# fetty31/fast_LIMO

Measured on AMD Instinct MI355X. Metric: scans/sec (64k-pt scan, 1M-pt map) + kNN HBM GB/s vs roofline; ATE vs CPU ref, higher is better.
Workload: dtype f32; 1 GPU; BASELINE.json configs[1]: 65536-pt Velodyne-like scan (64 rings x 1024 azimuths), 1000000-pt box-world map, k=5, MAX_NUM_ITERS=3, GPU deskew + iterated ESKF update per step; parallelism=replicas x1 (independent scan streams, no collective), steps_bit_reproducible=True, chains_run=0, chains_handed_back_early=0, chains_declined=2597

## Files before the change

fast_limo_amd/_lib.py:

```python
from __future__ import annotations

import ctypes as C
import os
import numpy as np

_PKG = os.path.dirname(os.path.abspath(__file__))
ROOT = os.path.dirname(_PKG)

f32p = np.ctypeslib.ndpointer(dtype=np.float32, flags="C_CONTIGUOUS")
f64p = np.ctypeslib.ndpointer(dtype=np.float64, flags="C_CONTIGUOUS")
i32p = np.ctypeslib.ndpointer(dtype=np.int32, flags="C_CONTIGUOUS")


class FlimoError(RuntimeError):
    pass


class MapCfg(C.Structure):
    _fields_ = [("min_extent", C.c_float), ("bucket_size", C.c_int), ("downsample", C.c_int),
                ("cell_size", C.c_float)]


class MatchCfg(C.Structure):
    _fields_ = [("NUM_MATCH_POINTS", C.c_int), ("MAX_NUM_MATCHES", C.c_int), ("MAX_NUM_PC2MATCH", C.c_int),
                ("MAX_DIST_PLANE", C.c_double), ("PLANE_THRESHOLD", C.c_double), ("estimate_extrinsics", C.c_int)]


class Frame(C.Structure):
    _fields_ = [("p", C.c_float * 3), ("q", C.c_float * 4), ("v", C.c_float * 3), ("g", C.c_float * 3),
                ("w", C.c_float * 3), ("a", C.c_float * 3), ("bg", C.c_float * 3), ("ba", C.c_float * 3),
                ("time", C.c_double)]


CHAIN_MAX_PASSES = 12


class FilterCfg(C.Structure):
    _fields_ = [("crop_active", C.c_int), ("crop_min", C.c_float * 3), ("crop_max", C.c_float * 3), ("dist_active", C.c_int),
                ("min_dist", C.c_float), ("rate_active", C.c_int), ("rate_value", C.c_int), ("time_kind", C.c_int),
                ("end_of_sweep", C.c_int), ("sweep_ref_time", C.c_double), ("fov_active", C.c_int), ("fov_angle", C.c_float)]


class ChainPass(C.Structure):
    _fields_ = [("M", C.c_int), ("stragglers", C.c_int), ("ties", C.c_int), ("HTH", C.c_double * 144), ("HTh", C.c_double * 12),
                ("dx", C.c_double * 23), ("x_after", C.c_double * 26)]


class ChainIO(C.Structure):
    _fields_ = [("x26", C.c_double * 26), ("P", C.c_double * 529), ("limits", C.c_double * 23), ("R", C.c_double), ("D", C.c_double),
                ("max_iter", C.c_int), ("want_log", C.c_int),
                ("status", C.c_int), ("reason", C.c_int), ("passes", C.c_int), ("it_next", C.c_int), ("t", C.c_int),
                ("x26_out", C.c_double * 26), ("meas_valid", C.c_int), ("meas_M", C.c_int), ("meas_HTH", C.c_double * 144),
                ("meas_HTh", C.c_double * 12), ("log", ChainPass * CHAIN_MAX_PASSES)]


MATCH_REC_DTYPE = np.dtype([
    ("H", np.float32, 12), ("h", np.float32), ("valid", np.float32), ("n", np.float32, 4),
    ("p_global", np.float32, 3), ("sqd", np.float32, 5), ("nbr", np.int32, 5), ("n_nbr", np.int32)])

FRAME_DTYPE = np.dtype([
    ("p", np.float32, 3), ("q", np.float32, 4), ("v", np.float32, 3), ("g", np.float32, 3), ("w", np.float32, 3),
    ("a", np.float32, 3), ("bg", np.float32, 3), ("ba", np.float32, 3), ("_pad", np.float32), ("time", np.float64)])

HIP_SYMBOLS = [
    "flimo_ctx_create", "flimo_ctx_destroy", "flimo_last_error", "flimo_version",
    "flimo_map_config", "flimo_map_add", "flimo_map_clear", "flimo_map_crop_box", "flimo_map_crop_stats", "flimo_map_size", "flimo_map_last_time",
    "flimo_map_points", "flimo_knn", "flimo_scan_set", "flimo_scan_size", "flimo_scan_get",
    "flimo_scan_voxel_filter", "flimo_raw_scan_set", "flimo_raw_scan_filter_set", "flimo_raw_scan_filter_order_set", "flimo_raw_scan_order", "flimo_deskew_resident", "flimo_deskew_resident_offset", "flimo_deskew",
    "flimo_match_reduce", "flimo_match_fetch", "flimo_match_fetch_H",
    "flimo_scan_to_world", "flimo_scan_clouds", "flimo_scan_debug_clouds", "flimo_upload_stage", "flimo_match_reduce_overlap", "flimo_map_add_scan",
    "flimo_set_timing", "flimo_set_timing_stride", "flimo_set_timing_deferred", "flimo_pass_count", "flimo_fused_pass_count", "flimo_tie_stats", "flimo_map_index_bytes", "flimo_fine_stats", "flimo_map_grid_selfcheck", "flimo_set_debug_records", "flimo_last_kernel_ms",
    "flimo_last_candidates_per_query", "flimo_last_widen_count", "flimo_last_stragglers", "flimo_stragglers_by_pass", "flimo_timing_totals", "flimo_timing_split", "flimo_set_path_switches", "flimo_set_wait_timeout_ms", "flimo_insert_rule_replay", "flimo_plane_fit5_host", "flimo_plane_eval5_host", "flimo_calculate_H_host",
    "flimo_update_chain", "flimo_chain_stats", "flimo_set_update_mode", "flimo_update_mode", "flimo_scan_adopt", "flimo_set_pass_pipeline", "flimo_pass_pipeline_end", "flimo_pass_pipeline_last", "flimo_pass_pipeline_stats",
]

_hip = None


def hip_lib_path() -> str:
    return os.environ.get("FLIMO_HIP_LIB") or os.path.join(_PKG, "libflimo_hip.so")


def load_hip():
    global _hip
    if _hip is not None:
        return _hip
    path = hip_lib_path()
    if not os.path.exists(path):
        raise FlimoError(f"{path} not found: run `python -c 'import __graft_entry__ as g; g.build()'` first")
    L = C.CDLL(path)
    vp = C.c_void_p
    L.flimo_ctx_create.restype = C.c_int
    L.flimo_ctx_create.argtypes = [C.c_int, C.POINTER(vp)]
    L.flimo_ctx_destroy.restype = None
    L.flimo_ctx_destroy.argtypes = [vp]
    L.flimo_last_error.restype = C.c_char_p
    L.flimo_last_error.argtypes = [vp]
    L.flimo_version.restype = C.c_char_p
    L.flimo_map_config.argtypes = [vp, C.POINTER(MapCfg)]
    L.flimo_map_add.argtypes = [vp, f32p, C.c_size_t, C.c_size_t, C.c_double]
    L.flimo_map_clear.argtypes = [vp]
    L.flimo_map_crop_box.argtypes = [vp, C.c_void_p, C.c_void_p, C.POINTER(C.c_size_t)]
    L.flimo_map_crop_stats.argtypes = [vp, C.POINTER(C.c_uint64)]
    L.flimo_map_size.restype = C.c_size_t
    L.flimo_map_size.argtypes = [vp]
    L.flimo_map_last_time.restype = C.c_double
    L.flimo_map_last_time.argtypes = [vp]
    L.flimo_map_points.argtypes = [vp, C.c_void_p, C.c_size_t, C.POINTER(C.c_size_t)]
    L.flimo_knn.argtypes = [vp, f32p, C.c_size_t, C.c_int, i32p, f32p, i32p]
    L.flimo_scan_set.argtypes = [vp, f32p, C.c_size_t, C.c_size_t]
    L.flimo_scan_size.restype = C.c_size_t
    L.flimo_scan_size.argtypes = [vp]
    L.flimo_scan_get.argtypes = [vp, C.c_void_p, C.c_size_t, C.POINTER(C.c_size_t)]
    L.flimo_scan_voxel_filter.argtypes = [vp, C.c_float, C.POINTER(C.c_size_t)]
    L.flimo_raw_scan_set.argtypes = [vp, f32p, C.c_size_t, C.c_size_t, f64p]
    L.flimo_deskew_resident.argtypes = [vp, C.c_void_p, C.c_size_t, f32p, f64p]
    L.flimo_deskew.argtypes = [vp, f32p, C.c_size_t, C.c_size_t, f64p, C.c_void_p, C.c_size_t, f32p, f64p]
    L.flimo_match_reduce.argtypes = [vp, f64p, C.POINTER(MatchCfg), f64p, f64p, C.POINTER(C.c_int)]
    L.flimo_match_fetch.argtypes = [vp, C.c_void_p, C.c_size_t, C.POINTER(C.c_size_t)]
    L.flimo_match_fetch_H.argtypes = [vp, C.c_void_p, C.c_void_p, C.c_size_t, C.POINTER(C.c_size_t)]
    L.flimo_scan_to_world.argtypes = [vp, f64p, C.c_void_p, C.c_size_t]
    L.flimo_scan_clouds.argtypes = [vp, f64p, C.POINTER(C.c_void_p), C.POINTER(C.c_void_p), C.POINTER(C.c_size_t)]
    L.flimo_scan_debug_clouds.argtypes = [vp, f64p, C.POINTER(C.c_void_p), C.POINTER(C.c_void_p), C.POINTER(C.c_size_t)]
    L.flimo_upload_stage.argtypes = [vp, C.c_size_t, C.POINTER(C.c_void_p)]
    L.flimo_map_add_scan.argtypes = [vp, f64p, C.c_double]
    L.flimo_set_timing.argtypes = [vp, C.c_int]
    L.flimo_set_wait_timeout_ms.argtypes = [vp, C.c_int]
    L.flimo_set_timing_stride.argtypes = [vp, C.c_int]
    L.flimo_set_timing_deferred.argtypes = [vp, C.c_int]
    L.flimo_pass_count.restype = C.c_ulonglong
    L.flimo_pass_count.argtypes = [vp]
    L.flimo_tie_stats.argtypes = [vp, C.POINTER(C.c_ulonglong)]
    L.flimo_fine_stats.argtypes = [vp, C.POINTER(C.c_ulonglong)]
    L.flimo_map_index_bytes.argtypes = [vp, C.POINTER(C.c_uint64)]
    L.flimo_fused_pass_count.restype = C.c_ulonglong
    L.flimo_fused_pass_count.argtypes = [vp]
    L.flimo_map_grid_selfcheck.restype = C.c_int
    L.flimo_map_grid_selfcheck.argtypes = [vp, C.POINTER(C.c_uint64), C.POINTER(C.c_uint64)]
    L.flimo_set_debug_records.argtypes = [vp, C.c_int]
    L.flimo_last_kernel_ms.argtypes = [vp, C.POINTER(C.c_float), C.POINTER(C.c_float), C.POINTER(C.c_float)]
    L.flimo_timing_totals.argtypes = [vp, C.POINTER(C.c_double), C.POINTER(C.c_double), C.POINTER(C.c_double),
                                      C.POINTER(C.c_longlong), C.POINTER(C.c_longlong), C.c_int]
    L.flimo_timing_split.argtypes = [vp, f64p, C.c_int]
    L.flimo_set_path_switches.argtypes = [vp, C.c_int, C.c_int]
    L.flimo_insert_rule_replay.argtypes = [C.c_float, C.c_int, f32p, C.c_void_p, C.c_size_t, C.c_void_p, C.POINTER(C.c_size_t)]
    L.flimo_calculate_H_host.argtypes = [f64p, f32p, f32p, f32p, C.c_size_t, C.c_int, f64p, f64p]
    L.flimo_update_chain.argtypes = [vp, C.POINTER(MatchCfg), C.POINTER(ChainIO)]
    L.flimo_chain_stats.argtypes = [vp, f64p, C.c_int]
    L.flimo_set_update_mode.argtypes = [vp, C.c_int]
    L.flimo_scan_adopt.argtypes = [vp, vp]
    L.flimo_raw_scan_filter_order_set.argtypes = [vp, C.c_void_p, C.c_size_t, C.POINTER(FilterCfg), C.c_int, C.POINTER(C.c_size_t),
                                                  C.POINTER(C.c_double), C.POINTER(C.c_int), C.POINTER(C.c_int)]
    L.flimo_raw_scan_order.argtypes = [vp, C.c_void_p, C.c_size_t, C.POINTER(C.c_size_t)]
    L.flimo_deskew_resident_offset.argtypes = [vp, C.c_void_p, C.c_size_t, np.ctypeslib.ndpointer(np.float32, flags="C_CONTIGUOUS"),
                                               np.ctypeslib.ndpointer(np.float64, flags="C_CONTIGUOUS"), C.c_double]
    L.flimo_set_pass_pipeline.argtypes = [vp, C.c_int]
# ... 245 lines not shown
    def set_debug_records(self, on=True):
        self._chk(self._L.flimo_set_debug_records(self._h, int(on)))

    def last_kernel_ms(self):
        a = C.c_float(0)
        b = C.c_float(0)
        d = C.c_float(0)
        self._chk(self._L.flimo_last_kernel_ms(self._h, C.byref(a), C.byref(b), C.byref(d)))
        return a.value, b.value, d.value

    def timing_totals(self, reset=False):
        a = C.c_double(0); b = C.c_double(0); d = C.c_double(0); n = C.c_longlong(0); q = C.c_longlong(0)
        self._chk(self._L.flimo_timing_totals(self._h, C.byref(a), C.byref(b), C.byref(d), C.byref(n), C.byref(q), int(reset)))
        return dict(knn_ms=a.value, widen_ms=b.value, fit_ms=d.value, passes=n.value, queries=q.value)

    def set_path_switches(self, tail=-1, fuse=-1):
        self._chk(self._L.flimo_set_path_switches(self._h, int(tail), int(fuse)))

    def timing_split(self, reset=False):
        o = np.zeros(6)
        self._chk(self._L.flimo_timing_split(self._h, o, int(reset)))
        return dict(fused_ms=o[0], fused_n=int(o[1]), knn_ms=o[2], widen_ms=o[3], fit_ms=o[4], separate_n=int(o[5]))

    def update_chain(self, cfg: "MatchCfg", x26, P, limits, R=0.001, D=5.0, max_iter=3, want_log=True):
        io = ChainIO()
        io.x26[:] = list(np.asarray(x26, dtype=np.float64))
        io.P[:] = list(np.asarray(P, dtype=np.float64).reshape(-1))
        io.limits[:] = list(np.asarray(limits, dtype=np.float64))
        io.R, io.D, io.max_iter, io.want_log = float(R), float(D), int(max_iter), int(bool(want_log))
        self._chk(self._L.flimo_update_chain(self._h, C.byref(cfg), C.byref(io)))
        n_log = min(CHAIN_MAX_PASSES, io.passes + (1 if io.status == 2 else 0))
        log = [dict(M=io.log[i].M, stragglers=io.log[i].stragglers, ties=io.log[i].ties,
                    HTH=np.array(io.log[i].HTH).reshape(12, 12), HTh=np.array(io.log[i].HTh), dx=np.array(io.log[i].dx),
                    x_after=np.array(io.log[i].x_after)) for i in range(n_log)]
        meas = dict(M=io.meas_M, HTH=np.array(io.meas_HTH).reshape(12, 12), HTh=np.array(io.meas_HTh)) if io.meas_valid else None
        return dict(status=io.status, reason=io.reason, passes=io.passes, it_next=io.it_next, t=io.t, x=np.array(io.x26_out),
                    meas=meas, log=log)

    def set_update_mode(self, mode: int):
        self._chk(self._L.flimo_set_update_mode(self._h, int(mode)))

    def update_mode(self):
        ch = C.c_int(0); rtt = C.c_double(0)
        self._chk(self._L.flimo_update_mode(self._h, C.byref(ch), C.byref(rtt)))
        return dict(chained=bool(ch.value), launch_rtt_us=rtt.value)

    def set_pass_pipeline(self, on: bool):
        self._chk(self._L.flimo_set_pass_pipeline(self._h, int(on)))

    def pass_pipeline_end(self):
        self._chk(self._L.flimo_pass_pipeline_end(self._h))

    def pass_pipeline_last(self):
        self._chk(self._L.flimo_pass_pipeline_last(self._h))

    def pass_pipeline_stats(self):
        o = (C.c_ulonglong * 4)()
        self._chk(self._L.flimo_pass_pipeline_stats(self._h, o))
        return dict(published=int(o[0]), cancelled=int(o[1]), aged=int(o[2]), left=int(o[3]))

    def chain_stats(self, reset=False):
        o = np.zeros(5)
        self._chk(self._L.flimo_chain_stats(self._h, o, int(reset)))
        return dict(algebra_ms=o[0], algebra_n=int(o[1]), chains=int(o[2]), handed_back=int(o[3]), declined=int(o[4]))

    def last_widen_count(self) -> int:
        return int(self._L.flimo_last_widen_count(self._h))

    def set_wait_timeout_ms(self, ms: int):
        self._chk(self._L.flimo_set_wait_timeout_ms(self._h, int(ms)))

    def last_stragglers(self) -> int:
        return int(self._L.flimo_last_stragglers(self._h))

    def stragglers_by_pass(self):
        o = (C.c_int * 4)()
        self._chk(self._L.flimo_stragglers_by_pass(self._h, o))
        return [int(v) for v in o]

    def last_candidates_per_query(self) -> float:
        return float(self._L.flimo_last_candidates_per_query(self._h))


def default_match_cfg(**kw) -> MatchCfg:
    c = MatchCfg(5, 2000, 10000, 2.0, 5.0e-2, 1)
    for k, v in kw.items():
        if not hasattr(c, k):
            raise AttributeError(k)
        setattr(c, k, v)
    return c


def insert_rule_replay(batches, min_extent=0.2, downsample=True):
    L = load_hip()
    sizes = np.array([b.shape[0] for b in batches], dtype=np.uint64)
    xyz = np.ascontiguousarray(np.concatenate([np.asarray(b, dtype=np.float32).reshape(-1, 3) for b in batches]))
    keep = np.zeros(xyz.shape[0], dtype=np.uint8)
    stored = C.c_size_t(0)
    rc = L.flimo_insert_rule_replay(float(min_extent), int(downsample), xyz.reshape(-1), sizes.ctypes.data, len(batches),
                                    keep.ctypes.data, C.byref(stored))
    if rc != 0:
        raise FlimoError(f"flimo_insert_rule_replay failed ({rc})")
    out, off = [], 0
    for b in batches:
        out.append(keep[off:off + b.shape[0]].astype(bool))
        off += b.shape[0]
    return out, int(stored.value)
```

fast_limo_amd/csrc/hip/flimo_capi.hip:

```cpp
#include <hip/hip_runtime.h>
#include <stdarg.h>
#include <stdio.h>
#include <string.h>
#include <math.h>
#include <string>
#include <chrono>
#include <thread>
#include <array>
#include <vector>
#include <algorithm>
#include <immintrin.h>
#include "../../../include/flimo_c.h"
#include "../../../include/flimo_dev.h"
#include "flimo_types.h"
#include "flimo_kernels.h"
#include "flimo_math.h"
#include "flimo_pose.h"
#include "flimo_chain.h"
#include "flimo_ieskf.h"
#include "flimo_insert.h"
#include "flimo_gbook.h"

#pragma clang fp contract(off)

// ... 93 lines not shown
  float4* d_dbg_clouds = nullptr;
  size_t dbg_clouds_cap = 0, dbg_clouds_dcap = 0;
  void (*overlap_fn)(void*) = nullptr;
  void* overlap_arg = nullptr;
  size_t clouds_cap = 0;
  size_t stage_cap = 0;
  hipEvent_t ev[6] = {nullptr, nullptr, nullptr, nullptr, nullptr, nullptr};
  static constexpr int EV_RING = 64;
  hipEvent_t ev_ring[EV_RING][6];
  unsigned char ev_kind[EV_RING];
  int ev_pending = 0;
  bool ev_ring_made = false, timing_deferred = false;
  float last_knn_ms = 0.f, last_widen_ms = 0.f, last_fit_ms = 0.f;
  int* h_wl_count = nullptr;
  int last_widen_count = 0;
  double tot_knn_ms = 0, tot_widen_ms = 0, tot_fit_ms = 0;
  long long tot_passes = 0, tot_queries = 0;
  double split_fused_ms = 0, split_knn_ms = 0, split_widen_ms = 0, split_fit_ms = 0;
  long long split_fused_n = 0, split_sep_n = 0;
  flimo_match_cfg last_cfg{};
  PoseMats last_P{};
  MatchParams last_mp{};
  int last_n_all = 0;
  bool recs_valid = false, dbg_valid = false;
  PrevPass prev{};
  bool prune = true;
  unsigned probe_min = 96;
  int stragglers_hist[4] = {1 << 30, 0, 0, 0};
  int pass_in_scan = 0;
  int last_stragglers = -1;
  bool fine_on = true;
  unsigned fine_threshold = 64;
  int fine_div = 4;
  unsigned fine_min_points = 32768;
  bool fine_valid = false;
  bool crowd_box_valid = false;
  GridView fine{};
  int fine_qlo[3] = {0, 0, 0}, fine_qhi[3] = {-1, -1, -1};
  float4 *d_fine_tmp = nullptr, *d_fine_pts = nullptr;
  size_t fine_pts_cap = 0;
  IndexTables fine_idx;
  uint32_t* d_fine_count = nullptr;
  void* d_crowd_list = nullptr;
  uint32_t* d_crowd_count = nullptr;
  uint32_t* d_crowd_bits = nullptr;
  size_t crowd_bits_cap = 0;
  uint32_t crowd_listed = 0;
  std::vector<std::array<int, 3>> crowd_cells;
  float fine_center[3] = {0.f, 0.f, 0.f};
  bool have_fine_center = false;
  float fine_radius = 24.f;
  uint64_t fine_builds = 0, fine_passes = 0;
  int xslabs = 2;
  int* d_tie_list = nullptr;
  unsigned int* d_tie_count = nullptr;
  size_t tie_cap = 0;
  bool ties = true;
  unsigned long long tie_redos = 0, tie_queries = 0;
  unsigned long long* d_tie_settled = nullptr;
  void* d_nbrk = nullptr;
  size_t nbrk_cap = 0;
  int wait_timeout_ms = 2000;
  hipEvent_t adopt_ev = nullptr;
  hipEvent_t timeout_ev = nullptr;
  bool timeout_pending = false;
  ChainState* d_chain = nullptr;
  void* d_chain_gran = nullptr;
  ChainPrior* h_chain_prior = nullptr;
  ChainPrior* d_chain_prior = nullptr;
  double* h_chain_res = nullptr;
  void* d_chain_res = nullptr;
  double* h_chain_log = nullptr;
  void* d_chain_log = nullptr;
  unsigned long long chain_tag = 0x4000000000000000ull;
  struct Prelaunch {
    bool active = false;
    unsigned long long seq = 0;
    size_t nq = 0;
    int n_all = 0, pos = 0;
    flimo_match_cfg cfg{};
    uint64_t grid_version = 0;
    unsigned int end_code = 0;
    double t_launch = 0.0;
  } pre;
  bool pipeline = false;
  bool pipeline_env = false;
  ChainHead* d_pipe_head = nullptr;
  unsigned int pipe_tag = 0;
  bool pipe_last_hint = false;
  unsigned long long pipe_published = 0, pipe_cancelled = 0;
  unsigned long long pipe_aged = 0, pipe_left = 0;
  bool row_slack = true;
  bool test_tight_array = false;
  int test_publish_delay_ms = 0;
  PrevPass prev_before{};
  int update_mode = 0;
  double launch_rtt_us = 0.0;
  bool host_update = false;
  hipEvent_t chain_ev[CH_MAX_PASSES][8];
  bool chain_ev_made = false;
  double chain_alg_ms = 0;
  long long chain_alg_n = 0, chains_run = 0, chains_back = 0, chains_declined = 0;
  int fov_check = 0, fov_check_bad = 0;
  bool tail = true;
};

constexpr size_t FRAMES_FG_SLOT = 8192;
static int timing_drain(flimo_ctx* c);
static inline void ctx_enter(flimo_ctx* c);
static int fail(flimo_ctx* c, int code, const char* fmt, ...) {
  char buf[512];
  va_list ap;
  va_start(ap, fmt);
  vsnprintf(buf, sizeof(buf), fmt, ap);
  va_end(ap);
  if (c) c->err = buf;
  return code;
}
#define HIPCHK(c, call)                                                                          \
  do {                                                                                           \
    hipError_t e_ = (call);                                                                      \
    if (e_ != hipSuccess) return fail(c, FLIMO_ERR_HIP, "%s failed: %s", #call, hipGetErrorString(e_)); \
  } while (0)

static int ensure_pinned(flimo_ctx* c, void*& buf, size_t& cap, size_t bytes) {
  if (bytes <= cap) return FLIMO_OK;
  if (buf) (void)hipHostFree(buf);
  buf = nullptr;
  cap = 0;
  const size_t ncap = bytes + bytes / 4 + 4096;
  HIPCHK(c, hipHostMalloc(&buf, ncap, hipHostMallocDefault));
  cap = ncap;
  return FLIMO_OK;
}
static int ensure_stage(flimo_ctx* c, size_t bytes) { return ensure_pinned(c, c->h_stage, c->stage_cap, bytes); }

template <typename T>
static int ensure_dev(flimo_ctx* c, T*& p, size_t& cap, size_t need, bool keep, size_t keep_n) {
  if (need <= cap) return FLIMO_OK;
  size_t ncap = need + need / 4 + 1024;
  T* np = nullptr;
  HIPCHK(c, hipMalloc(&np, ncap * sizeof(T)));
  if (keep && p && keep_n) {
    HIPCHK(c, hipMemcpyAsync(np, p, keep_n * sizeof(T), hipMemcpyDeviceToDevice, c->stream));
    HIPCHK(c, hipStreamSynchronize(c->stream));
  }
  if (p) (void)hipFree(p);
  p = np;
  cap = ncap;
  return FLIMO_OK;
}


static void load_dev_switches(flimo_ctx* c) {
  auto env_int = [](const char* name, int& out) { const char* e = getenv(name); if (!e) return false; out = atoi(e); return true; };
  int v = 0;
  if (env_int("FLIMO_FUSE", v)) c->fuse = v != 0;
  if (env_int("FLIMO_TAIL", v)) c->tail = v != 0;
  if (env_int("FLIMO_PRUNE", v)) c->prune = v != 0;
  if (env_int("FLIMO_PROBE", v) && v >= 0) c->probe_min = (unsigned)v;
  if (env_int("FLIMO_TIES", v)) c->ties = v != 0;
  if (env_int("FLIMO_FINE", v)) c->fine_on = v != 0;
  if (env_int("FLIMO_FINE_THRESHOLD", v) && v > 0) c->fine_threshold = (unsigned)v;
  if (env_int("FLIMO_FINE_MIN_POINTS", v) && v >= 0) c->fine_min_points = (unsigned)v;
  if (env_int("FLIMO_FULL_REBUILD", v)) c->full_rebuild = v != 0;
  if (env_int("FLIMO_HOST_UPDATE", v)) c->update_mode = v != 0 ? 1 : 2;
  if (env_int("FLIMO_PIPELINE", v)) { c->pipeline = v != 0; c->pipeline_env = true; }
  if (env_int("FLIMO_TEST_PUBLISH_DELAY_MS", v) && v > 0) c->test_publish_delay_ms = v;
  if (env_int("FLIMO_TEST_TIGHT_ARRAY", v)) c->test_tight_array = v != 0;
  if (env_int("FLIMO_ROW_SLACK", v)) c->row_slack = v != 0;
  if (env_int("FLIMO_TAIL_MAX", v) && v > 0) c->tail_max_env = v;
}

static bool host_store_probe(flimo_ctx* c, ChainHead* head) {
  volatile unsigned long long* tagp = reinterpret_cast<volatile unsigned long long*>(c->h_chain_res) + 1;
  for (unsigned int round = 0; round < 2; round++) {
    const unsigned int pattern = 0x5a17c0deu ^ (round * 0x01010101u);
    __atomic_store_n(&head->epoch, pattern, __ATOMIC_RELEASE);
    _mm_sfence();
    const unsigned long long tag = 0x7200000000000000ull + round;
    launch_word_probe(c->stream, &head->epoch, c->d_chain_res, tag);
    if (hipStreamSynchronize(c->stream) != hipSuccess) { (void)hipGetLastError(); return false; }
    if (*tagp != tag) return false;
    const double seen = c->h_chain_res[0];
    if ((unsigned int)llround(seen) != pattern) return false;
  }
  __atomic_store_n(&head->epoch, 0u, __ATOMIC_RELEASE);
  _mm_sfence();
  memset(c->h_chain_res, 0, 2 * sizeof(double));
  return true;
}

extern "C" const char* flimo_version(void) { return "fast_limo_amd 0.1.0 (gfx950)"; }

extern "C" const char* flimo_last_error(const flimo_ctx* ctx) { return ctx ? ctx->err.c_str() : "null context"; }

extern "C" int flimo_ctx_create(int device, flimo_ctx** out) {
  if (!out) return FLIMO_ERR_INVALID;
  *out = nullptr;
  int ndev = 0;
  if (hipGetDeviceCount(&ndev) != hipSuccess || ndev <= 0) return FLIMO_ERR_NO_DEVICE;
  if (device < 0 || device >= ndev) return FLIMO_ERR_INVALID;
  if (hipSetDevice(device) != hipSuccess) return FLIMO_ERR_NO_DEVICE;
  hipDeviceProp_t prop;
  if (hipGetDeviceProperties(&prop, device) != hipSuccess) return FLIMO_ERR_NO_DEVICE;
  if (strncmp(prop.gcnArchName, "gfx950", 6) != 0) return FLIMO_ERR_NO_DEVICE;
  flimo_ctx* c = new flimo_ctx();
  c->device = device;
  if (hipStreamCreateWithFlags(&c->stream, hipStreamNonBlocking) != hipSuccess) { delete c; return FLIMO_ERR_HIP; }
  for (int i = 0; i < 6; i++) (void)hipEventCreate(&c->ev[i]);
  bool ok = hipMalloc(&c->d_partials, (size_t)c->reduce_waves * 256 * sizeof(double)) == hipSuccess &&
            hipMalloc(&c->d_out256, FIT_GROUPS * FIT_SLOT * sizeof(double)) == hipSuccess &&
            hipHostMalloc((void**)&c->h_out256, FIT_GROUPS * FIT_SLOT * sizeof(double), hipHostMallocMapped) == hipSuccess &&
            hipHostGetDevicePointer((void**)&c->d_out256_host, c->h_out256, 0) == hipSuccess &&
            hipHostMalloc((void**)&c->h_granules, FIT_GROUPS * FIT_LIVE_PAD * 2 * sizeof(double), hipHostMallocMapped) == hipSuccess &&
            hipHostGetDevicePointer((void**)&c->d_granules_host, c->h_granules, 0) == hipSuccess &&
            hipMalloc(&c->d_ticket, (FIT_GROUPS + 2) * sizeof(unsigned int)) == hipSuccess &&
            hipMemset(c->d_ticket, 0, (FIT_GROUPS + 2) * sizeof(unsigned int)) == hipSuccess &&
            hipMalloc(&c->d_cand, sizeof(unsigned long long)) == hipSuccess &&
            hipMalloc(&c->d_tie_count, 2 * sizeof(unsigned int)) == hipSuccess &&
            hipMemset(c->d_tie_count, 0, 2 * sizeof(unsigned int)) == hipSuccess &&
            hipMalloc((void**)&c->d_chain, chain_state_size()) == hipSuccess &&
            hipMemset(c->d_chain, 0, chain_state_size()) == hipSuccess &&
            hipMalloc(&c->d_chain_gran, FIT_GROUPS * FIT_LIVE_PAD * 2 * sizeof(double)) == hipSuccess &&
            hipMemset(c->d_chain_gran, 0, FIT_GROUPS * FIT_LIVE_PAD * 2 * sizeof(double)) == hipSuccess &&
            hipHostMalloc((void**)&c->h_chain_prior, sizeof(ChainPrior), hipHostMallocMapped) == hipSuccess &&
            hipHostGetDevicePointer((void**)&c->d_chain_prior, c->h_chain_prior, 0) == hipSuccess &&
            hipHostMalloc((void**)&c->h_chain_res, (size_t)CH_RES * 2 * sizeof(double), hipHostMallocMapped) == hipSuccess &&
            hipHostGetDevicePointer(&c->d_chain_res, c->h_chain_res, 0) == hipSuccess &&
            hipHostMalloc((void**)&c->h_chain_log, (size_t)CH_MAX_PASSES * CH_LOGN * 2 * sizeof(double), hipHostMallocMapped) == hipSuccess &&
            hipHostGetDevicePointer(&c->d_chain_log, c->h_chain_log, 0) == hipSuccess &&
            hipMalloc((void**)&c->d_tie_settled, sizeof(unsigned long long)) == hipSuccess &&
            hipMemset(c->d_tie_settled, 0, sizeof(unsigned long long)) == hipSuccess &&
            hipMalloc(&c->d_wl_count, sizeof(int)) == hipSuccess &&
            hipMemset(c->d_wl_count, 0, sizeof(int)) == hipSuccess &&
            hipHostMalloc((void**)&c->h_wl_count, sizeof(int), hipHostMallocDefault) == hipSuccess &&
            hipHostMalloc((void**)&c->h_cand, sizeof(unsigned long long), hipHostMallocDefault) == hipSuccess;
  if (!ok) { flimo_ctx_destroy(c); return FLIMO_ERR_HIP; }
  memset(c->h_chain_res, 0, (size_t)CH_RES * 2 * sizeof(double));
  memset(c->h_chain_log, 0, (size_t)CH_MAX_PASSES * CH_LOGN * 2 * sizeof(double));
  memset(c->h_out256, 0, FIT_GROUPS * FIT_SLOT * sizeof(double));
  memset(c->h_granules, 0, FIT_GROUPS * FIT_LIVE_PAD * 2 * sizeof(double));
  launch_mfma_layout(c->stream, c->d_out256);
  if (hipMemcpyAsync(c->h_out256, c->d_out256, 256 * sizeof(double), hipMemcpyDeviceToHost, c->stream) != hipSuccess ||
      hipStreamSynchronize(c->stream) != hipSuccess) { flimo_ctx_destroy(c); return FLIMO_ERR_HIP; }
  bool seen[256] = {false};
  for (int r = 0; r < 256; r++) {
    const double v = c->h_out256[r];
    const int code = (int)llround(v);
    if (code < 0 || code > 255 || fabs(v - code) > 1e-9 || seen[code]) { flimo_ctx_destroy(c); return FLIMO_ERR_HIP; }
    seen[code] = true;
    c->mfma_idx[code / 16][code % 16] = r;
  }
  {
    int k = 0;
    for (int i = 0; i < 12; i++) for (int j = i; j < 12; j++) c->live_idx[k++] = (unsigned char)c->mfma_idx[i][j];
    for (int i = 0; i < 12; i++) c->live_idx[k++] = (unsigned char)c->mfma_idx[i][12];
    c->live_idx[k++] = (unsigned char)c->mfma_idx[13][13];
    for (; k < FIT_LIVE_PAD; k++) c->live_idx[k] = 0;
  }
  c->book = insert_book_create();
  load_dev_switches(c);
  {
    void* p = nullptr;
    int large_bar = 0;
    (void)hipDeviceGetAttribute(&large_bar, hipDeviceAttributeIsLargeBar, device);
    if (getenv("FLIMO_NO_BAR") != nullptr) large_bar = 0;
    if (large_bar && hipExtMallocWithFlags(&p, sizeof(ChainHead), hipDeviceMallocFinegrained) == hipSuccess && p &&
        hipMemset(p, 0, sizeof(ChainHead)) == hipSuccess && hipDeviceSynchronize() == hipSuccess && host_store_probe(c, static_cast<ChainHead*>(p))) {
      c->d_pipe_head = static_cast<ChainHead*>(p);
      void* q = nullptr;
      if (hipExtMallocWithFlags(&q, 2 * FRAMES_FG_SLOT, hipDeviceMallocFinegrained) == hipSuccess && q)
        c->d_frames_fg = static_cast<char*>(q);
      else (void)hipGetLastError();
    } else {
      if (p) (void)hipFree(p);
      (void)hipGetLastError();
      c->d_pipe_head = nullptr;
    }
  }
  {
    std::vector<double> rt;
    volatile unsigned long long* tagp = reinterpret_cast<volatile unsigned long long*>(c->h_chain_res) + 1;
    for (int i = 0; i < 40; i++) {
      const unsigned long long tag = 0x7100000000000000ull + (unsigned long long)i;
      const auto t0 = std::chrono::steady_clock::now();
      launch_rtt_probe(c->stream, c->d_chain_res, tag);
      unsigned long long spins = 0;
      while (*tagp != tag && ++spins < 200000000ull) _mm_pause();
      const double us = std::chrono::duration<double, std::micro>(std::chrono::steady_clock::now() - t0).count();
      if (i >= 8) rt.push_back(us);
    }
    (void)hipStreamSynchronize(c->stream);
    std::sort(rt.begin(), rt.end());
    c->launch_rtt_us = rt[rt.size() / 4];
    memset(c->h_chain_res, 0, 2 * sizeof(double));
    c->host_update = c->update_mode != 2;
  }
  *out = c;
  return FLIMO_OK;
}

extern "C" void flimo_ctx_destroy(flimo_ctx* c) {
  if (!c) return;
  ctx_enter(c);
  if (c->stream) (void)hipStreamSynchronize(c->stream);
  (void)hipFree(c->d_map_raw); (void)hipFree(c->d_map_sorted); index_free(c->idx); index_free(c->fine_idx);
  (void)hipFree(c->d_scan_sorted); (void)hipFree(c->d_nbr); (void)hipFree(c->d_wl); (void)hipFree(c->d_wl_count);
  (void)hipFree(c->d_fit_partials); (void)hipFree(c->d_raw_sorted); (void)hipFree(c->d_t_sorted);
  (void)hipFree(c->d_scan); (void)hipFree(c->d_scan_raw); (void)hipFree(c->d_scan_world); (void)hipFree(c->d_scan_t);
  (void)hipFree(c->d_frames); (void)hipFree(c->d_recs); (void)hipFree(c->d_dbg); (void)hipFree(c->d_dbg_clouds);
  (void)hipFree(c->d_fine_tmp); (void)hipFree(c->d_fine_pts); 
  (void)hipFree(c->d_fine_count); (void)hipFree(c->d_crowd_list); (void)hipFree(c->d_crowd_count); (void)hipFree(c->d_crowd_bits);
  (void)hipFree(c->d_tkey[0]); (void)hipFree(c->d_tkey[1]); (void)hipFree(c->d_tperm); (void)hipFree(c->d_t_tmp);
  (void)hipFree(c->d_raw32); (void)hipFree(c->d_filt_ext); (void)hipFree(c->d_nbrk); (void)hipFree(c->d_tie_list); (void)hipFree(c->d_tie_count);
  if (c->h_filt_ext) (void)hipHostFree(c->h_filt_ext);
  (void)hipFree(c->d_partials); (void)hipFree(c->d_out256); (void)hipFree(c->d_cand); (void)hipFree(c->d_ticket);
  if (c->h_out256) (void)hipHostFree(c->h_out256);
  if (c->h_granules) (void)hipHostFree(c->h_granules);
  (void)hipFree(c->d_fit2_partials);
  if (c->h_cand) (void)hipHostFree(c->h_cand);
  (void)hipFree(c->d_chain); (void)hipFree(c->d_chain_gran); (void)hipFree(c->d_tie_settled);
  if (c->h_chain_prior) (void)hipHostFree(c->h_chain_prior);
  if (c->h_chain_res) (void)hipHostFree(c->h_chain_res);
  if (c->h_chain_log) (void)hipHostFree(c->h_chain_log);
  if (c->chain_ev_made) for (int i = 0; i < CH_MAX_PASSES; i++) for (int k = 0; k < 8; k++) (void)hipEventDestroy(c->chain_ev[i][k]);
  if (c->h_stage) (void)hipHostFree(c->h_stage);
  if (c->h_dbg_clouds) (void)hipHostFree(c->h_dbg_clouds);
  if (c->h_clouds) (void)hipHostFree(c->h_clouds);
  for (int k = 0; k < 2; k++) if (c->h_frames[k]) (void)hipHostFree(c->h_frames[k]);
  map_scratch_free(c->scratch);
  for (int i = 0; i < 6; i++) if (c->ev[i]) (void)hipEventDestroy(c->ev[i]);
  if (c->ev_ring_made) for (int r = 0; r < flimo_ctx::EV_RING; r++) for (int i = 0; i < 6; i++) (void)hipEventDestroy(c->ev_ring[r][i]);
  if (c->timeout_ev) (void)hipEventDestroy(c->timeout_ev);
  if (c->adopt_ev) (void)hipEventDestroy(c->adopt_ev);
  if (c->h_wl_count) (void)hipHostFree(c->h_wl_count);
  if (c->d_pipe_head) (void)hipFree(c->d_pipe_head);
  if (c->d_frames_fg) (void)hipFree(c->d_frames_fg);
  if (c->stream) (void)hipStreamDestroy(c->stream);
  if (c->book) insert_book_destroy(c->book);
  c->gbook.release();
  (void)hipFree(c->d_batch);
  delete c;
}

extern "C" int flimo_map_config(flimo_ctx* c, const flimo_map_cfg* cfg) {
  if (!c || !cfg) return FLIMO_ERR_INVALID;
  if (!(cfg->min_extent > 0.f)) return fail(c, FLIMO_ERR_INVALID, "min_extent must be > 0");
  const float cell_before = c->map_cfg.cell_size;
  c->map_cfg = *cfg;
  if (!(c->map_cfg.cell_size > 0.f)) c->map_cfg.cell_size = 0.5f;
  if (c->map_cfg.cell_size != cell_before) { c->force_full = true; c->have_gbox = false; c->have_origin = false; }
  insert_book_config(c->book, cfg->min_extent, cfg->downsample != 0);
// ... 1007 lines not shown
  out[5] = c->d_map_sorted ? (uint64_t)c->sorted_cap * sizeof(float4) : 0ull;
  out[1] = c->grid_valid ? tables(c->grid, c->idx) : 0ull;
  out[2] = c->fine_valid ? (uint64_t)c->fine.n_pts * sizeof(float4) + tables(c->fine, c->fine_idx) : 0ull;
  out[3] = c->grid_valid ? c->idx.tiles_used : 0ull;
  out[4] = c->index_overflows;
  return FLIMO_OK;
}
extern "C" int flimo_tie_stats(flimo_ctx* c, unsigned long long out[2]) {
  if (!c || !out) return FLIMO_ERR_INVALID;
  out[0] = c->tie_redos; out[1] = c->tie_queries;
  unsigned long long dev = 0;
  ctx_enter(c);
  if (c->d_tie_settled && hipMemcpy(&dev, c->d_tie_settled, sizeof(dev), hipMemcpyDeviceToHost) == hipSuccess) out[1] += dev;
  return FLIMO_OK;
}
extern "C" int flimo_set_timing_stride(flimo_ctx* c, int every) { if (!c || every < 1) return FLIMO_ERR_INVALID; c->timing_stride = every; return FLIMO_OK; }
extern "C" int flimo_set_debug_records(flimo_ctx* c, int on) { if (!c) return FLIMO_ERR_INVALID; c->debug_recs = on != 0; return FLIMO_OK; }
extern "C" int flimo_last_kernel_ms(const flimo_ctx* c, float* knn_ms, float* widen_ms, float* fit_ms) {
  if (!c) return FLIMO_ERR_INVALID;
  if (knn_ms) *knn_ms = c->last_knn_ms;
  if (widen_ms) *widen_ms = c->last_widen_ms;
  if (fit_ms) *fit_ms = c->last_fit_ms;
  return FLIMO_OK;
}
extern "C" int flimo_last_widen_count(const flimo_ctx* c) { return c ? c->last_widen_count : 0; }
extern "C" int flimo_last_stragglers(const flimo_ctx* c) { return c ? c->last_stragglers : -1; }
extern "C" int flimo_stragglers_by_pass(const flimo_ctx* c, int out[4]) {
  if (!c || !out) return FLIMO_ERR_INVALID;
  for (int i = 0; i < 4; i++) out[i] = c->stragglers_hist[i];
  return FLIMO_OK;
}
extern "C" int flimo_timing_totals(flimo_ctx* c, double* knn_ms, double* widen_ms, double* fit_ms, long long* passes,
                                   long long* queries, int reset) {
  if (!c) return FLIMO_ERR_INVALID;
  if (c->ev_pending) { ctx_enter(c); const int rc = timing_drain(c); if (rc) return rc; }
  if (knn_ms) *knn_ms = c->tot_knn_ms;
  if (widen_ms) *widen_ms = c->tot_widen_ms;
  if (fit_ms) *fit_ms = c->tot_fit_ms;
  if (passes) *passes = c->tot_passes;
  if (queries) *queries = c->tot_queries;
  if (reset) { c->tot_knn_ms = c->tot_widen_ms = c->tot_fit_ms = 0.0; c->tot_passes = 0; c->tot_queries = 0; }
  return FLIMO_OK;
}
extern "C" int flimo_set_path_switches(flimo_ctx* c, int tail, int fuse) {
  if (!c) return FLIMO_ERR_INVALID;
  if (tail >= 0) c->tail = tail != 0;
  if (fuse >= 0) c->fuse = fuse != 0;
  return FLIMO_OK;
}
extern "C" int flimo_timing_split(flimo_ctx* c, double out[6], int reset) {
  if (!c || !out) return FLIMO_ERR_INVALID;
  if (c->ev_pending) { ctx_enter(c); const int rc = timing_drain(c); if (rc) return rc; }
  out[0] = c->split_fused_ms; out[1] = (double)c->split_fused_n;
  out[2] = c->split_knn_ms; out[3] = c->split_widen_ms; out[4] = c->split_fit_ms; out[5] = (double)c->split_sep_n;
  if (reset) { c->split_fused_ms = c->split_knn_ms = c->split_widen_ms = c->split_fit_ms = 0.0; c->split_fused_n = c->split_sep_n = 0; }
  return FLIMO_OK;
}
extern "C" double flimo_last_candidates_per_query(const flimo_ctx* c) { return c ? c->last_cand_per_query : 0.0; }

static int gate_rings(const flimo_ctx* c, double max_dist_plane) {
  const double cell = c->grid.cell;
  const int maxdim = std::max(c->grid.nx, std::max(c->grid.ny, c->grid.nz));
  const double margin = 1.0e-3 + 4.0e-7 * maxdim;
  const double need = sqrt(std::max(max_dist_plane, 0.0)) * (1.0 + 1e-5) / cell + margin;
  int r = (int)ceil(need);
  return std::max(r, 1);
}

static int abandon_wait(flimo_ctx* c, const char* what, unsigned long long id) {
  if (!c->timeout_ev) (void)hipEventCreateWithFlags(&c->timeout_ev, hipEventDisableTiming);
  if (c->timeout_ev && hipEventRecord(c->timeout_ev, c->stream) == hipSuccess) c->timeout_pending = true;
  c->prev.valid = 0;
  return fail(c, FLIMO_ERR_TIMEOUT, "%s %llu did not publish its result within %d ms (kernels still running)", what, id, c->wait_timeout_ms);
}
static inline bool same_match_cfg(const flimo_match_cfg& a, const flimo_match_cfg& b) {
  return a.NUM_MATCH_POINTS == b.NUM_MATCH_POINTS && a.MAX_NUM_MATCHES == b.MAX_NUM_MATCHES && a.MAX_NUM_PC2MATCH == b.MAX_NUM_PC2MATCH &&
         a.MAX_DIST_PLANE == b.MAX_DIST_PLANE && a.PLANE_THRESHOLD == b.PLANE_THRESHOLD && a.estimate_extrinsics == b.estimate_extrinsics;
}
static inline double wall_s() { return std::chrono::duration<double>(std::chrono::steady_clock::now().time_since_epoch()).count(); }
static inline void cancel_prelaunch(flimo_ctx* c) {
  if (!c->pre.active) return;
  c->pre.active = false;
  c->pipe_cancelled++;
  __atomic_store_n(&c->d_pipe_head->epoch, c->pre.end_code, __ATOMIC_RELEASE);
  _mm_sfence();
}
static inline void ctx_enter(flimo_ctx* c) {
  (void)hipSetDevice(c->device);
  cancel_prelaunch(c);
}
static inline void publish_prelaunch(flimo_ctx* c, const PoseMats& P, const float prev_RT[16], unsigned long long seq) {
  ChainHead h;
  memset(&h, 0, sizeof(h));
  h.pose = P;
  memcpy(h.prev_RT, prev_RT, sizeof(h.prev_RT));
  h.status = 0;
  const size_t words8 = offsetof(ChainHead, status) / 8;
  static_assert(offsetof(ChainHead, status) % 8 == 0 && offsetof(ChainHead, epoch) == offsetof(ChainHead, status) + 4, "ChainHead layout");
  volatile unsigned long long* dst = reinterpret_cast<volatile unsigned long long*>(c->d_pipe_head);
  const unsigned long long* src = reinterpret_cast<const unsigned long long*>(&h);
  for (size_t i = 0; i < words8; i++) dst[i] = src[i];
  __atomic_store_n(&c->d_pipe_head->status, 0, __ATOMIC_RELAXED);
  _mm_sfence();
  __atomic_store_n(&c->d_pipe_head->epoch, ch_epoch_of(seq), __ATOMIC_RELEASE);
  _mm_sfence();
  c->pre.active = false;
  c->pipe_published++;
}

static inline bool auto_host_update(const flimo_ctx*) { return true; }

static int check_abandoned(flimo_ctx* c) {
  if (!c->timeout_pending) return FLIMO_OK;
  hipError_t q = hipEventQuery(c->timeout_ev);
  if (q == hipErrorNotReady) return fail(c, FLIMO_ERR_TIMEOUT, "the launches of an earlier pass whose wait ran out are still running");
  c->timeout_pending = false;
  if (q != hipSuccess) return fail(c, FLIMO_ERR_HIP, "an abandoned pass failed: %s", hipGetErrorString(q));
  return FLIMO_OK;
}
static bool tags_complete(const flimo_ctx* c, unsigned long long want) {
  const volatile unsigned long long* t0 = reinterpret_cast<const volatile unsigned long long*>(c->h_granules);
  if (t0[2 * FIT_LIVE + 1] != want || t0[2 * (FIT_LIVE + 1) + 1] != want) return false;
  for (int g = 0; g < FIT_GROUPS; g++) {
    const volatile unsigned long long* tags = reinterpret_cast<const volatile unsigned long long*>(c->h_granules + (size_t)g * FIT_LIVE_PAD * 2);
    for (int k = 0; k < FIT_LIVE; k++)
      if (tags[2 * k + 1] != want) return false;
  }
  return true;
}
constexpr int FLIMO_PASS_LEFT = 1000;
static int wait_tags(flimo_ctx* c, unsigned long long want, int left_ms = -1) {
  const volatile unsigned long long* t0 = reinterpret_cast<const volatile unsigned long long*>(c->h_granules);
  unsigned long long spins = 0;
  double deadline = 0.0;
  auto now_s = [] { return std::chrono::duration<double>(std::chrono::steady_clock::now().time_since_epoch()).count(); };
  if (c->wait_timeout_ms == 0) return abandon_wait(c, "pass", want);
  const int bound_ms = left_ms >= 0 ? std::min(left_ms, c->wait_timeout_ms) : c->wait_timeout_ms;
  for (;;) {
    if (t0[2 * (FIT_LIVE + 1) + 1] == want && tags_complete(c, want)) return FLIMO_OK;
    _mm_pause();
    if ((++spins & 0x3fffull) != 0) continue;
    if (left_ms >= 0 && c->d_pipe_head &&
        __atomic_load_n(&c->d_pipe_head->decision, __ATOMIC_ACQUIRE) == ((ch_epoch_of(want) & 0x3fffffffu) | 0x80000000u)) return FLIMO_PASS_LEFT;
    const double t = now_s();
    if (deadline == 0.0) { deadline = t + 1e-3 * (double)bound_ms; continue; }
    if (t < deadline) continue;
    const hipError_t q = hipStreamQuery(c->stream);
    if (q == hipErrorNotReady && left_ms >= 0 && bound_ms < c->wait_timeout_ms) { left_ms = -1; deadline = t + 1e-3 * (double)(c->wait_timeout_ms - bound_ms); continue; }
    if (q == hipErrorNotReady) return abandon_wait(c, "pass", want);
    if (q != hipSuccess) return fail(c, FLIMO_ERR_HIP, "pass %llu failed: %s", want, hipGetErrorString(q));
    if (tags_complete(c, want)) return FLIMO_OK;
    if (left_ms >= 0) return FLIMO_PASS_LEFT;
    (void)hipMemsetAsync(c->d_ticket, 0, (FIT_GROUPS + 2) * sizeof(unsigned int), c->stream);
    (void)hipMemsetAsync(c->d_wl_count, 0, sizeof(int), c->stream);
    (void)hipMemsetAsync(c->d_tie_count, 0, 2 * sizeof(unsigned int), c->stream);
    (void)hipStreamSynchronize(c->stream);
    c->prev.valid = 0;
    return fail(c, FLIMO_ERR_HIP, "pass %llu completed without publishing its result (reduction tickets re-armed)", want);
  }
}

extern "C" int flimo_set_wait_timeout_ms(flimo_ctx* c, int ms) {
  if (!c || ms < 0) return FLIMO_ERR_INVALID;
  c->wait_timeout_ms = ms;
  return FLIMO_OK;
}

extern "C" int flimo_match_reduce(flimo_ctx* c, const double x26[26], const flimo_match_cfg* cfg, double HTH[144], double HTh[12], int* M);
extern "C" int flimo_match_reduce_overlap(flimo_ctx* c, const double x26[26], const flimo_match_cfg* cfg, double HTH[144], double HTh[12],
                                          int* M, void (*while_in_flight)(void*), void* arg) {
  if (!c) return FLIMO_ERR_INVALID;
  c->overlap_fn = while_in_flight;
  c->overlap_arg = arg;
  const int rc = flimo_match_reduce(c, x26, cfg, HTH, HTh, M);
  c->overlap_fn = nullptr;
  return rc;
}

static inline void run_overlap(flimo_ctx* c) {
  if (!c->overlap_fn) return;
  void (*fn)(void*) = c->overlap_fn;
  c->overlap_fn = nullptr;
  fn(c->overlap_arg);
}

struct PassPlan {
  const flimo_match_cfg* cfg = nullptr;
  PoseMats P;
  MatchParams mp;
  size_t nq = 0;
  int n_all = 0;
  bool general_k = false;
  bool use_pre = false, was_pre = false;
  bool last_of_update = false;
  uint64_t grid_version = 0;
  const DeskewArgs* dkp = nullptr;
  bool cap_binds = false, want_recs = false, want_count = false, fused_cap = false, use_fit2 = false;
  int tlev = 0;
  hipEvent_t* ev = nullptr;
  int tail_max = 0;
  bool tail = false, fused = false, after_fine = false, widen_timed = false;
  unsigned long long seq = 0;
  bool ties_on = false, inline_ties = false;
  TieList tl{};
  BookView book{};
  const BookView* bookp = nullptr;
  double tp0 = 0, tpa = 0, tpb = 0, tpc = 0, tp1 = 0;
};
static const bool g_prof_pass = getenv("FLIMO_PROF_PASS") != nullptr;
static inline double now_us() { return std::chrono::duration<double, std::micro>(std::chrono::steady_clock::now().time_since_epoch()).count(); }

constexpr int PASS_NOTHING = 2000;
static int pass_plan(flimo_ctx* c, const double x26[26], const flimo_match_cfg* cfg, PassPlan& pl) {
  pl.cfg = cfg;
  pl.general_k = cfg->NUM_MATCH_POINTS != 5;
  pl.last_of_update = c->pipe_last_hint;
  c->pipe_last_hint = false;
  struct PreGuard { flimo_ctx* c; bool decided = false; ~PreGuard() { if (!decided) cancel_prelaunch(c); } } pre_guard{c};
  { const int rca = check_abandoned(c); if (rca) return rca; }
  c->last_nq = 0;
  c->last_cfg = *cfg;
  c->recs_valid = c->dbg_valid = false;
  if (!c->grid_valid && c->map_n > 0) { int rc0 = rebuild_grid(c); if (rc0) return rc0; }
  if (!c->grid_valid || c->map_n == 0) return PASS_NOTHING;
  size_t nq = c->scan_n;
  if (cfg->MAX_NUM_PC2MATCH >= 0 && nq > (size_t)cfg->MAX_NUM_PC2MATCH) nq = (size_t)cfg->MAX_NUM_PC2MATCH;
  if (nq == 0) return PASS_NOTHING;
  pl.nq = nq;
  (void)hipSetDevice(c->device);
  pl.grid_version = c->grid_builds * 0x100000000ull + c->grid_merges;
  bool use_pre = c->pre.active && !pl.general_k && c->prev.valid && c->pre.nq == nq && c->pre.seq == c->pass_seq + 1 &&
                 same_match_cfg(c->pre.cfg, *cfg) && c->pre.grid_version == pl.grid_version && !c->deskew_pending &&
                 !(nq < c->sorted_n || (c->sorted_n < c->scan_n && nq > c->sorted_n)) && c->pre.n_all == (int)c->sorted_n &&
                 !c->debug_recs && !(cfg->MAX_NUM_MATCHES >= 0 && (size_t)cfg->MAX_NUM_MATCHES < nq);
  if (use_pre && !(wall_s() - c->pre.t_launch < 0.25e-3 * (double)CH_POLL_MS)) { use_pre = false; c->pipe_aged++; }
  if (!use_pre) cancel_prelaunch(c);
  pre_guard.decided = true;
  int rc = ensure_recs(c, nq);
  if (rc) { cancel_prelaunch(c); return rc; }

  pl.tp0 = g_prof_pass ? now_us() : 0.0;
  pose_from_x26(x26, pl.P);
  MatchParams& mp = pl.mp;
  mp.max_dist_plane_d = cfg->MAX_DIST_PLANE;
  mp.plane_threshold = (float)cfg->PLANE_THRESHOLD;
  mp.estimate_extrinsics = cfg->estimate_extrinsics ? 1 : 0;
  mp.n_queries = (int)nq;
  mp.max_ring = gate_rings(c, cfg->MAX_DIST_PLANE);

  if (nq < c->sorted_n || (c->sorted_n < c->scan_n && nq > c->sorted_n)) {
    const size_t want = nq;
    { const int rcf = flush_deskew(c); if (rcf) return rcf; }
    HIPCHK(c, sort_scan(c->stream, c->d_scan, want, c->d_scan_sorted, c->scratch));
    c->sorted_n = want;
    c->prev.valid = 0;
  }
  pl.n_all = (int)c->sorted_n;
  const bool ride = c->deskew_pending && !pl.general_k && c->deskew_n == (size_t)pl.n_all &&
                    !(c->fine_valid && mp.max_ring >= 1);
  if (!ride) { const int rcf = flush_deskew(c); if (rcf) return rcf; }
  pl.dkp = ride ? &c->deskew_args : nullptr;
  c->deskew_pending = false;
  pl.cap_binds = cfg->MAX_NUM_MATCHES >= 0 && (size_t)cfg->MAX_NUM_MATCHES < nq;
  if (pl.general_k) return FLIMO_OK;
  pl.want_recs = c->debug_recs || pl.cap_binds;
  if (c->debug_recs) HIPCHK(c, hipMemsetAsync(c->d_cand, 0, sizeof(unsigned long long), c->stream));
  pl.want_count = c->debug_recs;
  pl.tpa = g_prof_pass ? now_us() : 0.0;
  pl.tlev = (c->timing == 1 && c->timing_stride > 1 && ((c->pass_seq + 1) % (unsigned long long)c->timing_stride) != 0) ? 0 : c->timing;
  pl.ev = (c->timing_deferred && c->ev_ring_made) ? c->ev_ring[c->ev_pending] : c->ev;
  const bool first_pass = !c->prev.valid;
  c->pass_in_scan = first_pass ? 0 : std::min(c->pass_in_scan + 1, 3);
  pl.tail_max = c->tail_max_env > 0 ? c->tail_max_env : std::max(1024, pl.n_all / 64);
  const bool tail_here = first_pass ? (c->stragglers_hist[0] <= pl.tail_max)
                                    : (c->stragglers_hist[c->pass_in_scan] <= pl.tail_max);
  pl.tail = c->tail && tail_here && mp.max_ring >= 2 && mp.max_ring <= 3;
  c->prev.probe_min = c->probe_min;
  pl.fused = pl.tail && c->fuse && !pl.want_recs;
  pl.seq = ++c->pass_seq;
  pl.ties_on = c->ties && c->gbook.active;
  pl.tl = TieList{};
  pl.tl.count_next = c->d_tie_count + ((pl.seq + 1) & 1);
  pl.inline_ties = pl.ties_on && !pl.want_recs;
  if (pl.ties_on && !pl.inline_ties) { pl.tl.list = c->d_tie_list; pl.tl.count = c->d_tie_count + (pl.seq & 1); pl.tl.cap = (unsigned)c->tie_cap; }
  pl.book = BookView{c->gbook.node_c, c->gbook.node_child, c->gbook.node_cnt, c->gbook.root, c->d_tie_settled};
  pl.bookp = pl.inline_ties ? &pl.book : nullptr;
  pl.after_fine = c->fine_valid && mp.max_ring >= 1;
  if (use_pre && !(pl.fused && !pl.after_fine && pl.tlev == 0)) {
    cancel_prelaunch(c);
    use_pre = false;
  }
  if (use_pre) {
    const int test_delay_ms = c->test_publish_delay_ms;
    if (wall_s() - c->pre.t_launch >= 0.25e-3 * (double)CH_POLL_MS) { cancel_prelaunch(c); use_pre = false; c->pipe_aged++; }
    else if (test_delay_ms > 0) std::this_thread::sleep_for(std::chrono::milliseconds(test_delay_ms));
  }
  pl.use_pre = pl.was_pre = use_pre;
  pl.widen_timed = !pl.tail && pl.tlev == 1 && mp.max_ring >= 2;
  pl.fused_cap = pl.cap_binds && !c->debug_recs;
  pl.use_fit2 = !pl.want_recs;
  return FLIMO_OK;
}

static int pass_general_k(flimo_ctx* c, const PassPlan& pl, double HTH[144], double HTh[12], int* M) {
  const flimo_match_cfg* cfg = pl.cfg;
  const int n_all = pl.n_all;
  const size_t nq = pl.nq;
  if ((size_t)n_all > c->nbrk_cap) {
    (void)hipFree(c->d_nbrk);
    c->d_nbrk = nullptr; c->nbrk_cap = 0;
    const size_t cap = (size_t)n_all + (size_t)n_all / 4 + 1024;
    HIPCHK(c, hipMalloc(&c->d_nbrk, cap * nbrk_rec_size()));
    c->nbrk_cap = cap;
  }
  c->prev.valid = 0;
  const BookView bookk{c->gbook.node_c, c->gbook.node_child, c->gbook.node_cnt, c->gbook.root, nullptr};
  if (!launch_match_k(c->stream, cfg->NUM_MATCH_POINTS, c->grid, c->d_scan_sorted, n_all, pl.P, pl.mp, c->d_nbrk, c->d_recs, c->d_dbg,
                      (c->ties && c->gbook.active) ? &bookk : nullptr))
    return fail(c, FLIMO_ERR_UNSUPPORTED, "NUM_MATCH_POINTS out of range");
  if (pl.cap_binds) launch_cap(c->stream, c->d_recs, (int)nq, cfg->MAX_NUM_MATCHES);
  launch_reduce(c->stream, c->d_recs, (int)nq, c->reduce_waves, c->d_partials, c->d_out256_host);
  HIPCHK(c, hipMemsetAsync(c->d_tie_count, 0, 2 * sizeof(unsigned int), c->stream));
  HIPCHK(c, hipGetLastError());
  run_overlap(c);
  HIPCHK(c, hipStreamSynchronize(c->stream));
  ++c->pass_seq;
  for (int i = 0; i < 12; i++) {
    for (int j = 0; j < 12; j++) HTH[i * 12 + j] = c->h_out256[c->mfma_idx[i][j]];
    HTh[i] = c->h_out256[c->mfma_idx[i][12]];
  }
  *M = (int)llround(c->h_out256[c->mfma_idx[13][13]]);
  c->last_nq = (int)nq;
  c->last_P = pl.P; c->last_mp = pl.mp; c->last_n_all = n_all;
  c->recs_valid = true; c->dbg_valid = true;
  c->last_stragglers = -1;
  c->async_deskews = 0;
  return FLIMO_OK;
}

static int pass_launch(flimo_ctx* c, PassPlan& pl) {
  const flimo_match_cfg* cfg = pl.cfg;
  const PoseMats& P = pl.P;
  const MatchParams& mp = pl.mp;
  const int n_all = pl.n_all;
  const size_t nq = pl.nq;
  const unsigned long long seq = pl.seq;
  const int tlev = pl.tlev;
  if (pl.use_pre) {
    publish_prelaunch(c, P, c->prev.RT, seq);
    c->fused_passes++;
  } else if (pl.after_fine) {
    launch_knn5_fine(c->stream, c->fine, c->d_scan_sorted, n_all, P, c->d_nbr, c->prev, c->fine_qlo, c->fine_qhi, &pl.tl, seq);
    c->fine_passes++;
  }
  if (pl.use_pre) {
  } else if (pl.fused) {
    launch_match_fused(c->stream, c->grid, c->d_scan_sorted, n_all, P, mp, c->d_nbr, c->d_wl, c->d_wl_count, nullptr, c->prev,
                       c->live_idx, c->d_fit2_partials, c->d_granules_host, c->d_ticket, seq, tlev == 1 ? pl.ev[0] : nullptr,
                       tlev == 1 ? pl.ev[1] : nullptr, &pl.tl, pl.after_fine ? 1 : 0, pl.dkp, nullptr, nullptr, pl.bookp);
    c->fused_passes++;
  } else
  launch_knn5(c->stream, 2, c->grid, c->d_scan_sorted, n_all, P, mp.max_ring, c->d_nbr, c->d_wl,
              c->d_wl_count, c->debug_recs ? c->d_cand : nullptr, c->prev, pl.tail ? 1 : 0, tlev == 1 ? pl.ev[0] : nullptr,
              tlev == 1 ? pl.ev[1] : nullptr, nullptr, &pl.tl, pl.after_fine ? 1 : 0, seq, pl.dkp);
  c->prev_before = c->prev;
  if (c->prune) { memcpy(c->prev.RT, P.RT, sizeof(c->prev.RT)); c->prev.valid = 1; }
  pl.tpb = g_prof_pass ? now_us() : 0.0;
  if (!pl.tail)
    launch_widen(c->stream, c->grid, c->d_scan_sorted, P, mp.max_ring, c->d_nbr, c->d_wl, c->d_wl_count,
                 c->debug_recs ? c->d_cand : nullptr, pl.widen_timed ? pl.ev[4] : nullptr, pl.widen_timed ? pl.ev[5] : nullptr, &pl.tl);
  pl.tpc = g_prof_pass ? now_us() : 0.0;
  if (pl.want_count) HIPCHK(c, hipMemcpyAsync(c->h_wl_count, c->d_wl_count, sizeof(int), hipMemcpyDeviceToHost, c->stream));
  if (pl.fused) {
  } else if (pl.use_fit2)
    launch_fit2(c->stream, c->grid, c->d_scan_sorted, n_all, c->d_nbr, P, mp, c->live_idx, c->d_fit2_partials, c->d_granules_host,
                c->d_ticket, c->d_wl_count, seq, tlev == 1 ? pl.ev[2] : nullptr, tlev == 1 ? pl.ev[3] : nullptr, &pl.tl, nullptr, nullptr, pl.bookp);
  else {
    HIPCHK(c, hipGetLastError());
    if (pl.ties_on) { launch_tie(c->stream, c->grid, pl.book, c->d_scan_sorted, P, c->d_nbr, pl.tl); HIPCHK(c, hipGetLastError()); }
    launch_fit(c->stream, c->grid, c->d_scan_sorted, n_all, c->d_nbr, P, mp, pl.fused_cap ? nullptr : c->d_fit_partials,
               pl.want_recs ? c->d_recs : nullptr, c->debug_recs ? c->d_dbg : nullptr, pl.cap_binds ? c->d_out256 : c->d_out256_host,
               c->d_ticket, c->d_wl_count, seq);
    HIPCHK(c, hipGetLastError());
    HIPCHK(c, hipMemsetAsync(c->d_tie_count, 0, 2 * sizeof(unsigned int), c->stream));
  }
  if (pl.fused_cap) {
    launch_capreduce(c->stream, c->d_recs, (int)nq, cfg->MAX_NUM_MATCHES, c->d_out256_host, c->d_wl_count, seq);
  } else if (pl.cap_binds) {
    launch_cap(c->stream, c->d_recs, (int)nq, cfg->MAX_NUM_MATCHES);
    launch_reduce(c->stream, c->d_recs, (int)nq, c->reduce_waves, c->d_partials, c->d_out256_host);
  }
  HIPCHK(c, hipGetLastError());
  pl.tp1 = g_prof_pass ? now_us() : 0.0;
  if (c->debug_recs) HIPCHK(c, hipMemcpyAsync(c->h_cand, c->d_cand, sizeof(unsigned long long), hipMemcpyDeviceToHost, c->stream));
  if (c->pipeline && !pl.last_of_update && c->d_pipe_head && c->prune && pl.use_fit2 && !pl.want_count && c->tail && c->fuse &&
      mp.max_ring >= 2 && mp.max_ring <= 3 && !c->fine_valid && pl.inline_ties == pl.ties_on) {
    const unsigned long long nseq = seq + 1;
    const int ntlev = (c->timing == 1 && c->timing_stride > 1 && (nseq % (unsigned long long)c->timing_stride) != 0) ? 0 : c->timing;
    const int npos = std::min(c->pass_in_scan + 1, 3);
    if (ntlev == 0 && c->stragglers_hist[npos] <= pl.tail_max) {
      TieList tln{};
      tln.count_next = c->d_tie_count + ((nseq + 1) & 1);
      ChainCtl pc{};
      pc.end_code = 0x80000000u | (++c->pipe_tag & 0x7fffffffu);
      PrevPass pv = c->prev;
      pv.valid = 1;
      launch_match_fused(c->stream, c->grid, c->d_scan_sorted, n_all, P, mp, c->d_nbr, c->d_wl, c->d_wl_count, nullptr, pv,
                         c->live_idx, c->d_fit2_partials, c->d_granules_host, c->d_ticket, nseq, nullptr, nullptr, &tln, 0, nullptr,
                         c->d_pipe_head, &pc, pl.bookp, ch_epoch_of(nseq));
      HIPCHK(c, hipGetLastError());
      c->pre.active = true; c->pre.seq = nseq; c->pre.nq = nq; c->pre.n_all = n_all; c->pre.pos = npos; c->pre.cfg = *cfg;
      c->pre.grid_version = pl.grid_version; c->pre.end_code = pc.end_code; c->pre.t_launch = wall_s();
    }
  }
  return FLIMO_OK;
}

static int timing_read(flimo_ctx* c, hipEvent_t* ev, int kind) {
  const bool fused = kind & 1, use_fit2 = kind & 2, widen_timed = kind & 4;
  if (hipEventElapsedTime(&c->last_knn_ms, ev[0], ev[1]) != hipSuccess) {
    HIPCHK(c, hipEventSynchronize(ev[1]));
    (void)hipEventElapsedTime(&c->last_knn_ms, ev[0], ev[1]);
  }
  c->tot_knn_ms += c->last_knn_ms;
  if (fused) {
    c->last_fit_ms = 0.f; c->last_widen_ms = 0.f;
    c->split_fused_ms += c->last_knn_ms; c->split_fused_n++;
  } else if (use_fit2) {
    c->last_widen_ms = 0.f;
    if (widen_timed) {
      if (hipEventElapsedTime(&c->last_widen_ms, ev[4], ev[5]) != hipSuccess) c->last_widen_ms = 0.f;
      c->tot_widen_ms += c->last_widen_ms;
    }
    if (hipEventElapsedTime(&c->last_fit_ms, ev[2], ev[3]) != hipSuccess) {
      HIPCHK(c, hipEventSynchronize(ev[3]));
      (void)hipEventElapsedTime(&c->last_fit_ms, ev[2], ev[3]);
    }
    c->tot_fit_ms += c->last_fit_ms;
    c->split_knn_ms += c->last_knn_ms; c->split_widen_ms += c->last_widen_ms; c->split_fit_ms += c->last_fit_ms; c->split_sep_n++;
  }
  return FLIMO_OK;
}
static int timing_drain(flimo_ctx* c) {
  const int n = c->ev_pending;
  c->ev_pending = 0;
  for (int i = 0; i < n; i++) { const int rc = timing_read(c, c->ev_ring[i], c->ev_kind[i]); if (rc) return rc; }
  return FLIMO_OK;
}

static int pass_collect(flimo_ctx* c, PassPlan& pl, double HTH[144], double HTh[12], int* M) {
  const PoseMats& P = pl.P;
  const MatchParams& mp = pl.mp;
  const int n_all = pl.n_all;
  const size_t nq = pl.nq;
  const unsigned long long seq = pl.seq;
  const int tlev = pl.tlev;
  double acc[256];
  if (pl.use_fit2) {
    auto wait_granules = [&](unsigned long long want, int left_ms = -1) -> int {
      const int rcw = wait_tags(c, want, left_ms);
      if (rcw) return rcw;
      __atomic_thread_fence(__ATOMIC_ACQUIRE);
      return FLIMO_OK;
    };
    run_overlap(c);
    {
      int rcw = wait_granules(seq, pl.was_pre ? CH_POLL_MS + 25 : -1);
      if (rcw == FLIMO_PASS_LEFT) {
        cancel_prelaunch(c);
        c->pipe_left++;
        launch_match_fused(c->stream, c->grid, c->d_scan_sorted, n_all, P, mp, c->d_nbr, c->d_wl, c->d_wl_count, nullptr, c->prev_before,
                           c->live_idx, c->d_fit2_partials, c->d_granules_host, c->d_ticket, seq, nullptr, nullptr, &pl.tl, 0, nullptr, nullptr,
                           nullptr, pl.bookp);
        HIPCHK(c, hipGetLastError());
        rcw = wait_granules(seq);
      }
      if (rcw) return rcw;
    }
    c->last_stragglers = (int)llround(c->h_granules[2 * FIT_LIVE]);
    c->stragglers_hist[c->pass_in_scan] = c->last_stragglers;
    const long n_ties = (long)llround(c->h_granules[2 * (FIT_LIVE + 1)]);
    if (n_ties > 0 && pl.ties_on) {
      c->tie_redos++; c->tie_queries += (unsigned long long)n_ties;
      launch_tie(c->stream, c->grid, pl.book, c->d_scan_sorted, P, c->d_nbr, pl.tl);
      const unsigned long long seq2 = ++c->pass_seq;
      TieList tl2{};
      tl2.count_next = c->d_tie_count + ((seq2 + 1) & 1);
      launch_fit2(c->stream, c->grid, c->d_scan_sorted, n_all, c->d_nbr, P, mp, c->live_idx, c->d_fit2_partials, c->d_granules_host,
                  c->d_ticket, c->d_wl_count, seq2, nullptr, nullptr, &tl2);
      HIPCHK(c, hipGetLastError());
      const int rcw = wait_granules(seq2);
      if (rcw) return rcw;
    }
    double live[FIT_LIVE];
    for (int k = 0; k < FIT_LIVE; k++) {
// ... 34 lines not shown
      const int rc = timing_read(c, c->ev, kind);
      if (rc) return rc;
    }
    c->tot_passes++; c->tot_queries += n_all;
  }
  if (g_prof_pass) {
    static double acc_launch = 0, acc_wait = 0, a0 = 0, a1 = 0, a2 = 0, a3 = 0; static long cnt = 0;
    const double tp2 = now_us();
    acc_launch += pl.tp1 - pl.tp0; acc_wait += tp2 - pl.tp1;
    a0 += pl.tpa - pl.tp0; a1 += pl.tpb - pl.tpa; a2 += pl.tpc - pl.tpb; a3 += pl.tp1 - pl.tpc;
    if (++cnt % 200 == 0) {
      fprintf(stderr, "[flimo pass] host: pose+launches %.2f us (prep %.2f, knn launch %.2f, widen launch %.2f, fit launch %.2f), wait for result %.2f us (mean of 200)\n",
              acc_launch / 200, a0 / 200, a1 / 200, a2 / 200, a3 / 200, acc_wait / 200);
      acc_launch = acc_wait = a0 = a1 = a2 = a3 = 0;
    }
  }
  c->async_deskews = 0;
  if (pl.want_count) c->last_widen_count = *c->h_wl_count;
  if (c->debug_recs) c->last_cand_per_query = (double)(*c->h_cand) / (double)nq;
  if (!pl.use_fit2) {
    c->last_stragglers = -1;
    const int slots = pl.cap_binds ? 1 : FIT_GROUPS;
    for (int t = 0; t < 256; t++) {
      double r = c->h_out256[t];
      for (int g = 1; g < slots; g++) r += c->h_out256[(size_t)g * FIT_SLOT + t];
      acc[t] = r;
    }
  }
  for (int i = 0; i < 12; i++) {
    for (int j = 0; j < 12; j++) HTH[i * 12 + j] = acc[c->mfma_idx[i][j]];
    HTh[i] = acc[c->mfma_idx[i][12]];
  }
  *M = (int)llround(acc[c->mfma_idx[13][13]]);
  c->last_nq = (int)nq;
  c->last_P = P; c->last_mp = mp; c->last_n_all = n_all;
  c->recs_valid = pl.want_recs && !pl.fused_cap;
  c->dbg_valid = c->debug_recs;
  return FLIMO_OK;
}

extern "C" int flimo_match_reduce(flimo_ctx* c, const double x26[26], const flimo_match_cfg* cfg, double HTH[144],
                                  double HTh[12], int* M) {
  if (!c || !x26 || !cfg || !HTH || !HTh || !M) return FLIMO_ERR_INVALID;
  if (cfg->NUM_MATCH_POINTS < 3 || cfg->NUM_MATCH_POINTS > 8)
    return fail(c, FLIMO_ERR_UNSUPPORTED, "NUM_MATCH_POINTS must be in 3..8 (a plane needs 3 points; the neighbour records hold 8)");
  for (int i = 0; i < 144; i++) HTH[i] = 0.0;
  for (int i = 0; i < 12; i++) HTh[i] = 0.0;
  *M = 0;
  PassPlan pl;
  int rc = pass_plan(c, x26, cfg, pl);
  if (rc == PASS_NOTHING) return FLIMO_OK;
  if (rc) return rc;
  if (pl.general_k) return pass_general_k(c, pl, HTH, HTh, M);
  if ((rc = pass_launch(c, pl)) != FLIMO_OK) return rc;
  return pass_collect(c, pl, HTH, HTh, M);
}

extern "C" int flimo_set_update_mode(flimo_ctx* c, int mode) {
  if (!c || mode < 0 || mode > 2) return FLIMO_ERR_INVALID;
  c->update_mode = mode;
  c->host_update = mode == 1 || (mode == 0 && auto_host_update(c));
  return FLIMO_OK;
}
extern "C" int flimo_set_pass_pipeline(flimo_ctx* c, int on) {
  if (!c) return FLIMO_ERR_INVALID;
  cancel_prelaunch(c);
  if (!c->pipeline_env) c->pipeline = on != 0;
  if (c->update_mode == 0) c->host_update = auto_host_update(c);
  return FLIMO_OK;
}
extern "C" int flimo_pass_pipeline_end(flimo_ctx* c) {
  if (!c) return FLIMO_ERR_INVALID;
  cancel_prelaunch(c);
  return FLIMO_OK;
}
extern "C" int flimo_pass_pipeline_last(flimo_ctx* c) {
  if (!c) return FLIMO_ERR_INVALID;
  c->pipe_last_hint = true;
  return FLIMO_OK;
}
extern "C" int flimo_pass_pipeline_stats(const flimo_ctx* c, unsigned long long out[4]) {
  if (!c || !out) return FLIMO_ERR_INVALID;
  out[0] = c->pipe_published; out[1] = c->pipe_cancelled; out[2] = c->pipe_aged; out[3] = c->pipe_left;
  return FLIMO_OK;
}
extern "C" int flimo_update_mode(const flimo_ctx* c, int* chained, double* launch_rtt_us) {
  if (!c) return FLIMO_ERR_INVALID;
  if (chained) *chained = c->host_update ? 0 : 1;
  if (launch_rtt_us) *launch_rtt_us = c->launch_rtt_us;
  return FLIMO_OK;
}
extern "C" int flimo_chain_stats(flimo_ctx* c, double out[5], int reset) {
  if (!c || !out) return FLIMO_ERR_INVALID;
  out[0] = c->chain_alg_ms; out[1] = (double)c->chain_alg_n; out[2] = (double)c->chains_run; out[3] = (double)c->chains_back;
  out[4] = (double)c->chains_declined;
  if (reset) { c->chain_alg_ms = 0; c->chain_alg_n = 0; c->chains_run = c->chains_back = c->chains_declined = 0; }
  return FLIMO_OK;
}

extern "C" int flimo_update_chain(flimo_ctx* c, const flimo_match_cfg* cfg, flimo_chain_io* io) {
  if (!c || !cfg || !io) return FLIMO_ERR_INVALID;
  io->status = FLIMO_CHAIN_DECLINED; io->reason = 0; io->passes = 0; io->it_next = -1; io->t = 0; io->meas_valid = 0; io->meas_M = 0;
  auto decline = [&]() { c->chains_declined++; return FLIMO_OK; };
  { const int rca = check_abandoned(c); if (rca) return rca; }
  if (c->host_update) return decline();
  if (cfg->NUM_MATCH_POINTS != 5) return decline();
  const int n_pass = io->max_iter + 1;
  if (io->max_iter < 0 || n_pass > CH_MAX_PASSES) return decline();
  if (c->debug_recs || !c->tail || !c->fuse) return decline();
  if (!c->grid_valid && c->map_n > 0) { int rc0 = rebuild_grid(c); if (rc0) return rc0; }
  if (!c->grid_valid || c->map_n == 0) return decline();
  size_t nq = c->scan_n;
  if (cfg->MAX_NUM_PC2MATCH >= 0 && nq > (size_t)cfg->MAX_NUM_PC2MATCH) nq = (size_t)cfg->MAX_NUM_PC2MATCH;
  if (nq == 0) return decline();
  if (cfg->MAX_NUM_MATCHES >= 0 && (size_t)cfg->MAX_NUM_MATCHES < nq) return decline();
  ctx_enter(c);
  { int rc = ensure_recs(c, nq); if (rc) return rc; }
  MatchParams mp;
  mp.max_dist_plane_d = cfg->MAX_DIST_PLANE;
  mp.plane_threshold = (float)cfg->PLANE_THRESHOLD;
  mp.estimate_extrinsics = cfg->estimate_extrinsics ? 1 : 0;
  mp.n_queries = (int)nq;
  mp.max_ring = gate_rings(c, cfg->MAX_DIST_PLANE);
  if (mp.max_ring < 2 || mp.max_ring > 3) return decline();
  c->last_nq = 0;
  c->last_cfg = *cfg;
  c->recs_valid = c->dbg_valid = false;
  if (nq < c->sorted_n || (c->sorted_n < c->scan_n && nq > c->sorted_n)) {
    { const int rcf = flush_deskew(c); if (rcf) return rcf; }
    HIPCHK(c, sort_scan(c->stream, c->d_scan, nq, c->d_scan_sorted, c->scratch));
    c->sorted_n = nq;
    c->prev.valid = 0;
  }
  const int n_all = (int)c->sorted_n;
  const bool after_fine = c->fine_valid && mp.max_ring >= 1;
  const bool ride = c->deskew_pending && c->deskew_n == (size_t)n_all && !after_fine;
  if (!ride) { const int rcf = flush_deskew(c); if (rcf) return rcf; }
  const DeskewArgs* dkp = ride ? &c->deskew_args : nullptr;
  c->deskew_pending = false;

  PoseMats P0;
  pose_from_x26(io->x26, P0);
  ChainPrior& pr = *c->h_chain_prior;
  memcpy(pr.x, io->x26, sizeof(pr.x));
  memcpy(pr.P, io->P, sizeof(pr.P));
  memcpy(pr.limit, io->limits, sizeof(pr.limit));
  pr.R = io->R; pr.D = io->D; pr.max_iter = io->max_iter; pr.pad = 0;
  ik_pre_serial(io->x26, io->x26, io->P, io->R, pr.dxn, pr.AG, pr.AG + 144);
  __atomic_thread_fence(__ATOMIC_RELEASE);

  const unsigned long long tag = ++c->chain_tag;
  const unsigned long long seq0 = c->pass_seq;
  const bool ties_on = c->ties && c->gbook.active;
  const BookView book{c->gbook.node_c, c->gbook.node_child, c->gbook.node_cnt, c->gbook.root, c->d_tie_settled};
  const BookView* bookp = ties_on ? &book : nullptr;
  const ChainHead* head = reinterpret_cast<const ChainHead*>(c->d_chain);
  const int tail_max = std::max(1024, n_all / 64);
  struct Plan { int pos; bool fused, combined, timed; };
  Plan plan[CH_MAX_PASSES];
  int pos = c->pass_in_scan;
  bool prev_valid = c->prev.valid != 0;
  c->prev.probe_min = c->probe_min;
  ChainCtl ctl{};
  ctl.S = c->d_chain;
  ctl.gran = reinterpret_cast<double2*>(c->d_chain_gran);
  ctl.res = reinterpret_cast<double2*>(c->d_chain_res);
  ctl.log = io->want_log ? reinterpret_cast<double2*>(c->d_chain_log) : nullptr;
  ctl.tag = tag;
  ctl.end_code = 0x80000000u | (unsigned int)(tag & 0x7fffffffull);
  for (int i = 0; i < n_pass; i++) {
    const unsigned long long seq = seq0 + 1 + (unsigned long long)i;
    const bool first_pass = !prev_valid;
    pos = first_pass ? 0 : std::min(pos + 1, 3);
    const bool tail_here = first_pass ? (c->stragglers_hist[0] <= tail_max)
                                      : (c->stragglers_hist[pos] <= tail_max);
    const bool fused = tail_here;
    const bool combined = false;
    const bool timed = c->timing == 1 && (c->timing_stride <= 1 || (seq % (unsigned long long)c->timing_stride) == 0);
    plan[i] = Plan{pos, fused, combined, timed};
    hipEvent_t* ev = timed ? c->chain_ev[i] : nullptr;
    const ChainHead* ch = i == 0 ? nullptr : head;
    ctl.prior = i == 0 ? c->d_chain_prior : nullptr;
    PrevPass pv = c->prev;
    pv.valid = prev_valid ? 1 : 0;
    TieList tl{};
    tl.count_next = c->d_tie_count + ((seq + 1) & 1);
    unsigned int wait_epoch = 0u;
    if (after_fine) {
      launch_knn5_fine(c->stream, c->fine, c->d_scan_sorted, n_all, P0, c->d_nbr, pv, c->fine_qlo, c->fine_qhi, &tl, seq, ch, wait_epoch, ctl.end_code);
      wait_epoch = 0u;
      c->fine_passes++;
    }
    const DeskewArgs* dk = i == 0 ? dkp : nullptr;
    if (fused) {
      launch_match_fused(c->stream, c->grid, c->d_scan_sorted, n_all, P0, mp, c->d_nbr, c->d_wl, c->d_wl_count, nullptr, pv, c->live_idx,
                         c->d_fit2_partials, c->d_chain_gran, c->d_ticket, seq, ev ? ev[0] : nullptr, ev ? ev[1] : nullptr, &tl,
                         after_fine ? 1 : 0, dk, ch, &ctl, bookp, wait_epoch);
    } else {
      launch_knn5(c->stream, 2, c->grid, c->d_scan_sorted, n_all, P0, mp.max_ring, c->d_nbr, c->d_wl, c->d_wl_count, nullptr, pv, 0,
                  ev ? ev[0] : nullptr, ev ? ev[1] : nullptr, nullptr, &tl, after_fine ? 1 : 0, seq, dk, ch, wait_epoch, ctl.end_code);
      {
        launch_widen(c->stream, c->grid, c->d_scan_sorted, P0, mp.max_ring, c->d_nbr, c->d_wl, c->d_wl_count, nullptr, ev ? ev[6] : nullptr, ev ? ev[7] : nullptr, &tl, ch);
        launch_fit2(c->stream, c->grid, c->d_scan_sorted, n_all, c->d_nbr, P0, mp, c->live_idx, c->d_fit2_partials, c->d_chain_gran,
                    c->d_ticket, c->d_wl_count, seq, ev ? ev[2] : nullptr, ev ? ev[3] : nullptr, &tl, ch, &ctl, bookp);
      }
    }
    launch_ieskf(c->stream, ctl, seq, i == 0 ? P0.RT : nullptr, ev ? ev[4] : nullptr, ev ? ev[5] : nullptr);
    prev_valid = c->prune;
  }
  HIPCHK(c, hipGetLastError());
  c->chains_run++;

  const volatile unsigned long long* rt = reinterpret_cast<const volatile unsigned long long*>(c->h_chain_res);
  auto tag_at = [&](int slot) { return rt[2 * slot + 1] == tag; };
  auto val_at = [&](int slot) { return c->h_chain_res[2 * slot]; };
  auto complete = [&]() {
    for (int k = 0; k < CH_RES; k++) if (!tag_at(k)) return false;
    return true;
  };
  {
    if (c->wait_timeout_ms == 0) { c->pass_seq = seq0 + (unsigned long long)n_pass; return abandon_wait(c, "update chain", tag - 0x4000000000000000ull); }
    unsigned long long spins = 0;
    double deadline = 0.0;
    auto now_s = [] { return std::chrono::duration<double>(std::chrono::steady_clock::now().time_since_epoch()).count(); };
    for (;;) {
      if (tag_at(CH_STATUS) && complete()) break;
      _mm_pause();
      if ((++spins & 0x3fffull) != 0) continue;
      const double t = now_s();
      if (deadline == 0.0) { deadline = t + 1e-3 * (double)c->wait_timeout_ms; continue; }
      if (t < deadline) continue;
      const hipError_t q = hipStreamQuery(c->stream);
      c->prev.valid = 0;
      if (q == hipErrorNotReady) { c->pass_seq = seq0 + (unsigned long long)n_pass; return abandon_wait(c, "update chain", tag - 0x4000000000000000ull); }
      if (q != hipSuccess) return fail(c, FLIMO_ERR_HIP, "the update chain failed: %s", hipGetErrorString(q));
      if (complete()) break;
      (void)hipMemsetAsync(c->d_ticket, 0, (FIT_GROUPS + 2) * sizeof(unsigned int), c->stream);
      (void)hipMemsetAsync(c->d_wl_count, 0, sizeof(int), c->stream);
      (void)hipMemsetAsync(c->d_tie_count, 0, 2 * sizeof(unsigned int), c->stream);
      (void)hipStreamSynchronize(c->stream);
      return fail(c, FLIMO_ERR_HIP, "the update chain completed without publishing its result (reduction tickets re-armed)");
    }
    __atomic_thread_fence(__ATOMIC_ACQUIRE);
  }
  io->status = (int)llround(val_at(CH_STATUS));
  io->reason = (int)llround(val_at(CH_BAIL));
  io->passes = (int)llround(val_at(CH_PASSES));
  io->it_next = (int)llround(val_at(CH_IT));
  io->t = (int)llround(val_at(CH_T));
  for (int k = 0; k < 26; k++) io->x26_out[k] = val_at(CH_X + k);
  if (io->reason == CH_R_FINAL || io->reason == CH_R_DEGENERATE) {
    io->meas_valid = 1;
    int k = 0;
    for (int i = 0; i < 12; i++) for (int j = i; j < 12; j++) { const double v = val_at(CH_SUMS + k++); io->meas_HTH[i * 12 + j] = v; io->meas_HTH[j * 12 + i] = v; }
    for (int i = 0; i < 12; i++) io->meas_HTh[i] = val_at(CH_SUMS + k++);
    io->meas_M = (int)llround(val_at(CH_SUMS + k));
  }
  const int executed = std::min(n_pass, io->passes + 1);
  for (int i = 0; i < executed; i++) {
    flimo_chain_pass& L = io->log[i];
    L.M = (int)llround(val_at(CH_PASSINFO + 3 * i)); L.stragglers = (int)llround(val_at(CH_PASSINFO + 3 * i + 1));
    L.ties = (int)llround(val_at(CH_PASSINFO + 3 * i + 2));
    c->stragglers_hist[plan[i].pos] = L.stragglers;
    c->last_stragglers = L.stragglers;
    c->pass_in_scan = plan[i].pos;
    if (plan[i].fused) c->fused_passes++;
    if (io->want_log && i < io->passes) {
      const volatile unsigned long long* lt = reinterpret_cast<const volatile unsigned long long*>(c->h_chain_log) + (size_t)i * CH_LOGN * 2;
      const double* lv = c->h_chain_log + (size_t)i * CH_LOGN * 2;
      unsigned long long spins = 0;
      for (int k = 0; k < CH_LOGN; k++) {
        while (lt[2 * k + 1] != tag) { _mm_pause(); if (++spins > 400000000ull) return fail(c, FLIMO_ERR_HIP, "the update chain's log did not arrive"); }
      }
      __atomic_thread_fence(__ATOMIC_ACQUIRE);
      for (int k = 0; k < 144; k++) L.HTH[k] = lv[2 * k];
      for (int k = 0; k < 12; k++) L.HTh[k] = lv[2 * (144 + k)];
      for (int k = 0; k < 23; k++) L.dx[k] = lv[2 * (156 + k)];
      for (int k = 0; k < 26; k++) L.x_after[k] = lv[2 * (179 + k)];
    }
  }
  if (io->reason != CH_R_FINAL) c->chains_back++;
  c->pass_seq = seq0 + (unsigned long long)executed;
  if (io->reason == CH_R_FAILED) {
// ... 216 lines not shown
```

fast_limo_amd/csrc/hip/flimo_chain.h:

```cpp
#pragma once
#include <hip/hip_runtime.h>
#include "flimo_types.h"

namespace flimo {

constexpr int CH_MAX_PASSES = 12;

struct ChainHead {
  PoseMats pose;
  float prev_RT[16];
  int status;
  unsigned int epoch;
  unsigned int decision;
  int pad;
};
static_assert(sizeof(ChainHead) % 4 == 0 && sizeof(ChainHead) / 4 <= 128, "a pass workgroup reads the head with one load per thread");

struct ChainPrior {
  double x[26];
  double P[529];
  double limit[23];
  double R, D;
  int max_iter;
  int pad;
  double dxn[23];
  double AG[276];
};

struct ChainState {
  ChainHead head;
  double x[26];
  double x_prop[26];
  double P_prop[529];
  double limit[23];
  double R, D;
  int max_iter;
  int it;
  int t;
  int passes;
  double info[3 * CH_MAX_PASSES];
  double pre_dxn[23];
  double pre_AG[276];
};

struct ChainCtl {
  ChainState* S;
  const ChainPrior* prior;
  double2* gran;
  double2* res;
  double2* log;
  unsigned long long tag;
  unsigned int end_code;
};

constexpr int CH_STATUS = 0, CH_BAIL = 1, CH_PASSES = 2, CH_IT = 3, CH_T = 4;
constexpr int CH_X = 5;
constexpr int CH_PASSINFO = CH_X + 26;
constexpr int CH_SUMS = CH_PASSINFO + 3 * CH_MAX_PASSES;
constexpr int CH_RES = CH_SUMS + 91;
constexpr int CH_R_FEW = 1, CH_R_TIES = 2, CH_R_DEGENERATE = 3, CH_R_FAILED = 4, CH_R_FINAL = 5;
constexpr int CH_LOGN = 144 + 12 + 23 + 26;

size_t chain_state_size();
void launch_ieskf(hipStream_t st, const ChainCtl& ch, unsigned long long seq, const float* used_RT_host_or_null,
                  hipEvent_t e0 = nullptr, hipEvent_t e1 = nullptr);
void launch_ieskf_extra(hipStream_t st, const ChainCtl& ch, hipEvent_t e0 = nullptr, hipEvent_t e1 = nullptr);
__host__ __device__ inline unsigned int ch_epoch_of(unsigned long long seq) { return (unsigned int)(seq & 0x3fffffffull) | 0x40000000u; }
constexpr int CH_POLL_MS = 50;

}
```

fast_limo_amd/csrc/hip/flimo_kernels.h:

```cpp
#pragma once
#include <hip/hip_runtime.h>
#include "flimo_types.h"

namespace flimo {
struct FuseArgs;
struct TieList;
struct BookView;
struct ChainCtl;
struct ChainHead;
struct DeskewArgs {
  const float4* raw; const double* t; const void* frames; int nf; const float* mats; double t_offset;
  float4* out_sorted; float4* out_orig; int on;
  int stage_words;
};

void launch_knn5(hipStream_t st, int lanes_per_query, const GridView& G, const float4* scan_sorted, int n,
                 const PoseMats& P, int max_ring, void* nbr, int* wl, int* wl_count, unsigned long long* cand,
                 const PrevPass& prev, int tail, hipEvent_t e0 = nullptr, hipEvent_t e1 = nullptr, const struct FuseArgs* fuse = nullptr,
                 const TieList* ties = nullptr, int after_fine = 0, unsigned long long seq = 0ull, const DeskewArgs* deskew = nullptr,
                 const ChainHead* chain = nullptr, unsigned int wait_epoch = 0u, unsigned int end_code = 0u);
void launch_knn5_fine(hipStream_t st, const GridView& Gf, const float4* scan_sorted, int n, const PoseMats& P, void* nbr,
                      const PrevPass& prev, const int qlo[3], const int qhi[3], const TieList* ties, unsigned long long seq,
                      const ChainHead* chain = nullptr, unsigned int wait_epoch = 0u, unsigned int end_code = 0u);
void launch_widen(hipStream_t st, const GridView& G, const float4* scan_sorted, const PoseMats& P, int max_ring, void* nbr,
                  int* wl, int* wl_count, unsigned long long* cand, hipEvent_t e0 = nullptr, hipEvent_t e1 = nullptr,
                  const TieList* ties = nullptr, const ChainHead* chain = nullptr);
int fit_blocks(int n);
void set_xcd_stripe(int stripe);
constexpr int FIT_GROUPS = 8;
constexpr int FIT_SLOT = 264;
void launch_fit(hipStream_t st, const GridView& G, const float4* scan_sorted, int n, const void* nbr, const PoseMats& P,
                const MatchParams& mp, double* partials, Rec16* recs, RecDbg* dbg, double* out256, unsigned int* ticket,
                int* wl_count, unsigned long long seq);
constexpr int FIT_LIVE = 91;
constexpr int FIT_LIVE_PAD = 96;
int fit2_blocks(int n);
void launch_fit2(hipStream_t st, const GridView& G, const float4* scan_sorted, int n, const void* nbr, const PoseMats& P,
                 const MatchParams& mp, const unsigned char* live_idx, double* partials, void* out_granules, unsigned int* ticket,
                 int* wl_count, unsigned long long seq, hipEvent_t e0 = nullptr, hipEvent_t e1 = nullptr, const TieList* ties = nullptr,
                 const ChainHead* chain = nullptr, const ChainCtl* ctl = nullptr, const BookView* book = nullptr);
constexpr int FUSED_SPREAD_SLOTS = 32768;
int fused_spread(int n);
int fused_blocks(int n);
void launch_match_fused(hipStream_t st, const GridView& G, const float4* scan_sorted, int n, const PoseMats& P, const MatchParams& mp,
                        void* nbr, int* wl, int* wl_count, unsigned long long* cand, const PrevPass& prev,
                        const unsigned char* live_idx, double* partials, void* out_granules, unsigned int* ticket,
                        unsigned long long seq, hipEvent_t e0 = nullptr, hipEvent_t e1 = nullptr, const TieList* ties = nullptr,
                        int after_fine = 0, const DeskewArgs* deskew = nullptr, const ChainHead* chain = nullptr,
                        const ChainCtl* ctl = nullptr, const BookView* book = nullptr, unsigned int wait_epoch = 0u);
struct BookView { const float4* node_c; const int* node_child; const int* node_cnt; int root; unsigned long long* settled; };
struct TieList { int* list; unsigned int* count; unsigned int cap; unsigned int* count_next; };
void launch_tie(hipStream_t st, const GridView& G, const BookView& B, const float4* scan_sorted, const PoseMats& P, void* nbr,
                const TieList& tl);
void launch_knn_tie(hipStream_t st, const GridView& G, const BookView& B, const float* qxyz, int nq, int k, int32_t* idx, float* sqd,
                    const int32_t* cnt);
size_t nbrk_rec_size();
bool launch_match_k(hipStream_t st, int k, const GridView& G, const float4* scan_sorted, int n, const PoseMats& P,
                    const MatchParams& mp, void* nbrk, Rec16* recs, RecDbg* dbg, const BookView* book = nullptr);
size_t nbr_rec_size();
size_t wl_entry_size();
void launch_knn(hipStream_t st, const GridView& G, const float* qxyz, int nq, int k, int max_ring, int32_t* idx,
                float* sqd, int32_t* cnt);
void launch_cap(hipStream_t st, Rec16* recs, int n, int cap);
void launch_capreduce(hipStream_t st, const Rec16* recs, int n, int cap, double* out256, int* wl_count, unsigned long long seq);
void launch_reduce(hipStream_t st, const Rec16* recs, int n, int nwaves, double* partials, double* out256);
void launch_mfma_layout(hipStream_t st, double* raw256);
void launch_word_probe(hipStream_t st, const unsigned int* src, void* out_granule, unsigned long long tag);
void launch_rtt_probe(hipStream_t st, void* out_granule, unsigned long long tag);
void launch_deskew(hipStream_t st, const float4* in, const double* t, int n, const void* frames, int nf,
                   const float* mats32, float4* out_sorted, float4* out_orig, double t_offset = 0.0);
void launch_transform(hipStream_t st, const float4* in, int n, const PoseMats& P, float4* out);
bool launch_deskew_debug(hipStream_t st, const DeskewArgs& dk, int n, const PoseMats& P, float4* out_world, float4* out_final);
size_t dev_frame_size();

struct MapBuildScratch {
  void* cub_tmp = nullptr;
  size_t cub_tmp_bytes = 0;
  uint32_t* keys_in = nullptr;
  uint32_t* keys_out = nullptr;
  uint32_t* vals_in = nullptr;
  uint32_t* vals_out = nullptr;
  size_t cap_pts = 0;
  unsigned long long *ck_in = nullptr, *ck_out = nullptr;
  size_t ck_cap = 0;
  float* bbox = nullptr;
  uint32_t* mail_host = nullptr;
  uint32_t* mail_dev = nullptr;
  uint32_t mail_seq = 0;
  unsigned long long* filt_desc = nullptr;
  size_t filt_tiles_cap = 0;
  unsigned int filt_epoch = 0, filt_ticket_base = 0;
  unsigned long long* filt_mail_host = nullptr;
  unsigned long long* filt_mail_dev = nullptr;
  unsigned long long* crop_desc = nullptr;
  size_t crop_tiles_cap = 0;
};
enum MailSlot { MAIL_BOOK = 0 , MAIL_BOOK_END = 8 , MAIL_CROWD = 12, MAIL_BOXCOUNT = 13, MAIL_BBOX = 16 , MAIL_VOXEL = 24 , MAIL_TILES = 28 , MAIL_ROWS = 32 , MAIL_CROP = 36 ,
                MAIL_TAG = 62 , MAIL_WORDS = 64 };
struct MailPart { const void* src; int n; int dst; };
hipError_t mail_words(hipStream_t st, MapBuildScratch& S, const MailPart* parts, int nparts, bool rearm_bbox = false, void* zero = nullptr,
                      int zero_n = 0);
hipError_t ensure_mail(MapBuildScratch& S);
hipError_t mail_wait(hipStream_t st, MapBuildScratch& S);
hipError_t map_crop_compact(hipStream_t st, const float4* in, size_t n, const float lo[3], const float hi[3], float4* out, int blocks,
                            MapBuildScratch& S, size_t* kept, float bb[6]);

hipError_t map_bbox(hipStream_t st, const float4* pts, size_t n, MapBuildScratch& S, float bbox_host[6]);
hipError_t sort_scan(hipStream_t st, const float4* in, size_t n, float4* out, MapBuildScratch& S,
                     const double* t_in = nullptr, double* t_out = nullptr);
hipError_t index_scan(hipStream_t st, const float4* in, size_t n, float4* out, const double* t_in, double* t_out);
struct IndexTables {
  uint2* tiles = nullptr; size_t tiles_cap_entries = 0;
  uint32_t cap_tiles = 0, tiles_used = 0;
  TileShape shape{5, 5, 3, 0, 0, 0};
  uint16_t* dir = nullptr;
  uint32_t* need = nullptr;
  uint32_t* counters = nullptr;
  uint32_t* ovf = nullptr; size_t ovf_cap = 0;
  uint32_t* xstart = nullptr; size_t xstart_cap = 0;
  uint32_t* rowcap = nullptr; size_t rowcap_cap = 0;
  uint32_t* rowoff = nullptr; size_t rowoff_cap = 0;
  uint32_t* xstart_alt = nullptr; size_t xstart_alt_cap = 0;
  uint32_t* rowcap_alt = nullptr; size_t rowcap_alt_cap = 0;
  uint16_t* dir_alt = nullptr;
  uint32_t* tail = nullptr;
};
void index_free(IndexTables& T);
hipError_t map_build_grid(hipStream_t st, const float4* pts_in, size_t n, float4* pts_out, size_t out_cap, bool slack, IndexTables& T, size_t pts_cap,
                          const GridView& geo, MapBuildScratch& S);
hipError_t index_regrid(hipStream_t st, IndexTables& T, const GridView& O, GridView& N);
hipError_t index_grow_pool(hipStream_t st, IndexTables& T, uint32_t cap_tiles_new);
void index_view(const IndexTables& T, GridView& G);
// ... 26 lines not shown
```

fast_limo_amd/csrc/hip/flimo_kernels.hip:

```cpp
#include <hip/hip_runtime.h>
#include <hip/hip_ext.h>
#include <float.h>
#include <limits.h>
#include <stdlib.h>
#include <algorithm>
#include "flimo_types.h"
#include "flimo_math.h"
#include "flimo_kernels.h"
#include "flimo_chain.h"
#include "flimo_ieskf.h"

#pragma clang fp contract(off)

namespace flimo {

FLIMO_DEV bool pair_less(float d0, int i0, float d1, int i1) { return (d0 < d1) || (d0 == d1 && i0 < i1); }

template <int K>
FLIMO_DEV void topk_insert(float (&bd)[K], int (&bi)[K], float d, int id) {
  if (!pair_less(d, id, bd[K - 1], bi[K - 1])) return;
  bd[K - 1] = d;
  bi[K - 1] = id;
#pragma unroll
  for (int s = K - 1; s > 0; s--) {
// ... 110 lines not shown
  const float rx = fminf(fmaxf(fx - flx, 0.f), 1.f), ry = fminf(fmaxf(fy - fly, 0.f), 1.f),
              rz = fminf(fmaxf(fz - flz, 0.f), 1.f);

  const int maxdim = grid_maxdim(G);
  const float margin = 1.0e-3f + 4.0e-7f * (float)maxdim;
  const float cell2 = G.cell * G.cell;
  const float edge = fminf(fminf(fminf(rx, 1.f - rx), fminf(ry, 1.f - ry)), fminf(rz, 1.f - rz));

  int r0;
  {
    const int ox_ = cx < 0 ? -cx : (cx >= G.nx ? cx - G.nx + 1 : 0);
    const int oy_ = cy < 0 ? -cy : (cy >= G.ny ? cy - G.ny + 1 : 0);
    const int oz_ = cz < 0 ? -cz : (cz >= G.nz ? cz - G.nz + 1 : 0);
    r0 = max(1, max(ox_, max(oy_, oz_)));
  }
  if (r0 > max_ring) return;

  int r_prev = -1;
  int r = r0;
  float bound = FLT_MAX;
  for (;;) {
    if (r == 1) {
      uint32_t lo[9], hi[9];
      const int x0 = max(cx - 1, 0), x1 = min(cx + 1, G.nx - 1);
#pragma unroll
      for (int t = 0; t < 9; t++) {
        const int dy = (t % 3 == 0) ? 0 : ((t % 3 == 1) ? -1 : 1);
        const int dz = (t / 3 == 0) ? 0 : ((t / 3 == 1) ? -1 : 1);
        const int yy = cy + dy, zz = cz + dz;
        const bool in = (yy >= 0) && (yy < G.ny) && (zz >= 0) && (zz < G.nz) && (x0 <= x1);
        lo[t] = 0u; hi[t] = 0u;
        if (in) grid_row_range(G, G.dir, yy, zz, x0 * G.xs, (x1 + 1) * G.xs, lo[t], hi[t]);
      }
#pragma unroll
      for (int t = 0; t < 9; t++) {
        const int dy = (t % 3 == 0) ? 0 : ((t % 3 == 1) ? -1 : 1);
        const int dz = (t / 3 == 0) ? 0 : ((t / 3 == 1) ? -1 : 1);
        const float a = fmaxf(slab_dist(dy, ry) - margin, 0.f), b = fmaxf(slab_dist(dz, rz) - margin, 0.f);
        if ((a * a + b * b) * cell2 >= R.bd[K - 1]) continue;
        scan_range<L, K>(G.pts, lo[t], hi[t], sub, gx, gy, gz, R.bd, R.bi, R.cand);
      }
    } else {
      const int dz0 = max(-r, -cz), dz1 = min(r, G.nz - 1 - cz);
      const int dy0 = max(-r, -cy), dy1 = min(r, G.ny - 1 - cy);
      for (int dz = dz0; dz <= dz1; dz++)
        for (int dy = dy0; dy <= dy1; dy++)
          visit_row<L, K>(G, cx, cy, cz, dy, dz, r_prev, r, rx, ry, rz, margin, cell2, bound, sub, gx, gy, gz, R);
    }
    if (L > 1) merge_group<L, K>(R.bd, R.bi);
    const float rg = ((float)r + edge - margin) * G.cell;
    const bool have5 = R.bi[K - 1] != INT_MAX;
    const bool covers = (cx - r <= 0) && (cx + r >= G.nx - 1) && (cy - r <= 0) && (cy + r >= G.ny - 1) &&
                        (cz - r <= 0) && (cz + r >= G.nz - 1);
    if (covers || (have5 && R.bd[K - 1] <= rg * rg * (1.f - 1.0e-6f))) { R.exact = true; break; }
    if (r >= max_ring) break;
    int rn = 2 * r;
    if (have5) {
      bound = R.bd[K - 1];
      const float need = fl_sqrt(R.bd[K - 1]) * G.inv_cell * (1.f + 4.0e-6f) - edge + margin;
      rn = max(r + 1, (int)ceilf(fminf(need, 1.0e9f)));
    }
    rn = min(rn, max_ring);
    if (L > 1 && sub != 0) {
#pragma unroll
      for (int s = 0; s < K; s++) { R.bd[s] = FLT_MAX; R.bi[s] = INT_MAX; }
    }
    r_prev = r;
    r = rn;
  }
}

typedef unsigned long long u64;
#define KEY_EMPTY 0xffffffffffffffffull

#ifdef FLIMO_TRACE
__device__ unsigned long long g_trace[2][16384 * 8];
#if FLIMO_TRACE == 2
__shared__ unsigned long long s_trace_lds[2][8];
#define TRACE(k, slot)                                                                                  \
  do {                                                                                                  \
    asm volatile("s_waitcnt vmcnt(0) lgkmcnt(0)" ::: "memory");                                         \
    if (threadIdx.x == 0) s_trace_lds[k][slot] = wall_clock64();                                        \
  } while (0)
#define TRACE_FLUSH()                                                                                   \
  do {                                                                                                  \
    if (threadIdx.x == 0 && blockIdx.x < 16384)                                                         \
      for (int k_ = 0; k_ < 2; k_++) for (int s_ = 0; s_ < 8; s_++) g_trace[k_][blockIdx.x * 8 + s_] = s_trace_lds[k_][s_]; \
  } while (0)
#else
#define TRACE(k, slot)                                                                                  \
  do {                                                                                                  \
    asm volatile("s_waitcnt vmcnt(0) lgkmcnt(0)" ::: "memory");                                         \
    if (threadIdx.x == 0 && blockIdx.x < 16384) g_trace[k][blockIdx.x * 8 + (slot)] = wall_clock64();  \
  } while (0)
#define TRACE_FLUSH() do {} while (0)
#endif
extern "C" int flimo_trace_read(int k, unsigned long long* out, size_t n) {
  return (int)hipMemcpyFromSymbol(out, HIP_SYMBOL(g_trace), n * sizeof(unsigned long long), (size_t)k * 16384 * 8 * sizeof(unsigned long long),
                                  hipMemcpyDeviceToHost);
}
#else
#define TRACE(k, slot) do {} while (0)
#define TRACE_FLUSH() do {} while (0)
#endif

FLIMO_DEV u64 make_key(float d, uint32_t idx) { return ((u64)__float_as_uint(d) << 32) | (u64)idx; }

FLIMO_DEV void key5_insert(u64 (&k)[5], u64 key) {
  if (key >= k[4]) return;
  k[4] = key;
#pragma unroll
  for (int s = 4; s > 0; s--) {
    const u64 a = k[s - 1], b = k[s];
    const bool sw = b < a;
    k[s - 1] = sw ? b : a;
    k[s] = sw ? a : b;
  }
}

__constant__ int c_stripe = 8;
void set_xcd_stripe(int stripe) { (void)hipMemcpyToSymbol(HIP_SYMBOL(c_stripe), &stripe, sizeof(int)); }

__device__ __forceinline__ int xcd_chunk(int b, int nb) {
  const int x = b & 7, k = b >> 3, per = nb >> 3;
  const int S = c_stripe;
  if (S <= 0 || S >= per) return x * per + k;
  const int full = (per / S) * S;
  if (k >= full) return 8 * full + x * (per - full) + (k - full);
  return ((k / S) * 8 + x) * S + (k % S);
}

struct NbrRec {
  int32_t idx[5];
  int32_t flag;
  int32_t d5_bits;
  int32_t d5_valid;
};

struct U3 { uint32_t a, b, c; };
struct __attribute__((aligned(8))) Seg2 { uint32_t x0, y0, x1, y1; };
__device__ __forceinline__ double key_min(double a, double b) { double r; asm("v_min_f64 %0, %1, %2" : "=v"(r) : "v"(a), "v"(b)); return r; }
__device__ __forceinline__ double key_max(double a, double b) { double r; asm("v_max_f64 %0, %1, %2" : "=v"(r) : "v"(a), "v"(b)); return r; }
__device__ __forceinline__ double key_make(float d, uint32_t id) { return __hiloint2double((int)__float_as_uint(d), (int)id); }
__device__ __forceinline__ void best5_insert(double (&k)[5], double x) {
  double t = x;
#pragma unroll
  for (int i = 0; i < 4; i++) {
    const double lo = key_min(k[i], t);
    t = key_max(k[i], t);
    k[i] = lo;
  }
  k[4] = key_min(k[4], t);
}
__device__ __forceinline__ void best6_insert(double (&k)[6], double x) {
  double t = x;
#pragma unroll
  for (int i = 0; i < 5; i++) {
    const double lo = key_min(k[i], t);
    t = key_max(k[i], t);
    k[i] = lo;
  }
  k[5] = key_min(k[5], t);
}
#define KEY_NONE 0x7f800000ffffffffull

template <int CTRL>
__device__ __forceinline__ double key_dpp(double x) {
  const int lo = __double2loint(x), hi = __double2hiint(x);
  const int l2 = __builtin_amdgcn_update_dpp(lo, lo, CTRL, 0xf, 0xf, false);
  const int h2 = __builtin_amdgcn_update_dpp(hi, hi, CTRL, 0xf, 0xf, false);
  return __hiloint2double(h2, l2);
}
__device__ __forceinline__ double key_group_min(double md, int Gl, int lane) {
  md = key_min(md, key_dpp<0xB1>(md));
  if (Gl >= 4) md = key_min(md, key_dpp<0x4E>(md));
  if (Gl >= 8) md = key_min(md, key_dpp<0x141>(md));
  if (Gl >= 16) md = key_min(md, key_dpp<0x140>(md));
  if (Gl >= 32) {
    const int lo = __double2loint(md), hi = __double2hiint(md);
    const double r0 = __hiloint2double(__builtin_amdgcn_readlane(hi, 0), __builtin_amdgcn_readlane(lo, 0));
    const double r1 = __hiloint2double(__builtin_amdgcn_readlane(hi, 16), __builtin_amdgcn_readlane(lo, 16));
    const double r2 = __hiloint2double(__builtin_amdgcn_readlane(hi, 32), __builtin_amdgcn_readlane(lo, 32));
    const double r3 = __hiloint2double(__builtin_amdgcn_readlane(hi, 48), __builtin_amdgcn_readlane(lo, 48));
    const double a = key_min(r0, r1), b = key_min(r2, r3);
    md = (Gl >= 64) ? key_min(a, b) : (lane < 32 ? a : b);
  }
// ... 823 lines not shown
    for (int o = 1; o < L; o <<= 1) c += __shfl_xor(c, o, 64);
    if (sub == 0 && in_range) atomicAdd(cand_total, (unsigned long long)c);
  }
  if constexpr (FINE) {
    const bool inside = qcx >= fa.qlo[0] && qcx <= fa.qhi[0] && qcy >= fa.qlo[1] && qcy <= fa.qhi[1] && qcz >= fa.qlo[2] && qcz <= fa.qhi[2];
    if (in_range && sub == 0 && flag == 1 && inside) {
      int4 a, b;
      a.x = (int)(uint32_t)best[0]; a.y = (int)(uint32_t)best[1]; a.z = (int)(uint32_t)best[2]; a.w = (int)(uint32_t)best[3];
      b.x = (int)(uint32_t)best[4]; b.y = 4; b.z = (int)(uint32_t)(best[4] >> 32);
      b.w = (int)(1u | (tie ? 2u : 0u) | ((uint32_t)(fa.seq & 0xffffffull) << 8));
      int4* o = reinterpret_cast<int4*>(&nbr[p]);
      o[0] = a;
      o[1] = b;
      if (tie && tl.list) { const unsigned slot = atomicAdd(tl.count, 1u); if (slot < tl.cap) tl.list[slot] = p; }
    }
    return;
  }
  TRACE(0, 4);
  const bool pend_tail = tail && in_range && flag == 2;
  if (in_range && sub == 0 && !pend_tail) {
    int4 a, b;
    a.x = (int)(uint32_t)best[0]; a.y = (int)(uint32_t)best[1]; a.z = (int)(uint32_t)best[2]; a.w = (int)(uint32_t)best[3];
    b.x = (int)(uint32_t)best[4]; b.y = min(flag, 2); b.z = (int)(uint32_t)(best[4] >> 32); b.w = ((flag == 1) ? 1 : 0) | (tie ? 2 : 0);
    if (tie && !tie_listed && tl.list) { const unsigned slot = atomicAdd(tl.count, 1u); if (slot < tl.cap) tl.list[slot] = p; }
    int4* o = reinterpret_cast<int4*>(&nbr[p]);
    o[0] = a;
    o[1] = b;
    if (flag >= 2) {
      const int slot = atomicAdd(wl_count, 1);
      int4* e = reinterpret_cast<int4*>(wl) + 2 * (size_t)slot;
      e[0] = make_int4(p, __float_as_int(gx), __float_as_int(gy), __float_as_int(gz));
      e[1] = make_int4((int)(uint32_t)(best[4] >> 32), 2, __float_as_int(b2), 0);
    }
  }
  WaveLds& W = s_w[threadIdx.x >> 6];
  if (tail) knn5_tail(G, dir, max_ring, nbr, pend_tail && sub == 0, p, gx, gy, gz, (uint32_t)(best[4] >> 32), b2, W, wl_count, cand_total, FUSE, tl);
  TRACE(0, 5);
  if constexpr (FUSE) {
    const int lane = threadIdx.x & 63;
    float v[16];
#pragma unroll
    for (int i = 0; i < 16; i++) v[i] = 0.f;
    wave_lds_sync();
    int ids[5] = {(int)(uint32_t)best[0], (int)(uint32_t)best[1], (int)(uint32_t)best[2], (int)(uint32_t)best[3], (int)(uint32_t)best[4]};
    int fl = flag;
    bool tied = tie;
    uint32_t d5b = (uint32_t)(best[4] >> 32);
    if (sub == 0 && in_range && pend_tail) {
      const int4* rr = reinterpret_cast<const int4*>(W.res[lane]);
      const int4 a = rr[0], b = rr[1];
      ids[0] = a.x; ids[1] = a.y; ids[2] = a.z; ids[3] = a.w; ids[4] = b.x;
      fl = b.y;
      tied = (b.w & 2) != 0;
      d5b = (uint32_t)b.z;
    }
    if (fa.book.node_c)
      tie_repair_wave(G, fa.book, nbr, sub == 0 && in_range && fl == 1 && tied, p, gx, gy, gz, d5b, ids, *reinterpret_cast<TieLds*>(W.tile));
    TRACE(1, 1);
    if (sub == 0 && in_range) {
      if (fl == 1 && __float_as_uint(sp.w) < (uint32_t)fa.mp.n_queries) fit_row(G, P, fa.mp, ids, gx, gy, gz, v);
    }
    TRACE(1, 3);
    wave_lds_sync();
    fit_reduce_publish<64 / L>(v, sub == 0, lane / L, W.tile, s_w[0].acc, s_w[1].acc, s_w[2].acc, s_w[3].acc, &s_last, fa.idx,
                               fa.partials, fa.granules, fa.ticket, wl_count, fa.seq, tl, (int)blockIdx.x, nb);
  }
  TRACE_FLUSH();
}

template <int L, int SLOTS, bool FUSE, bool FINE = false>
__global__ __launch_bounds__(256) KNN_WPE void knn5_kernel(GridView G, const float4* __restrict__ scan_sorted, int n,
                                                   PoseMats P, int max_ring, NbrRec* __restrict__ nbr,
                                                   int* __restrict__ wl, int* __restrict__ wl_count,
                                                   unsigned long long* __restrict__ cand_total, PrevPass prev, int tail,
                                                   FuseArgs fa) {
  __shared__ __align__(16) uint16_t s_dir[GRID_DIR_MAX];
  const DirRegs dr = grid_dir_fetch(G);
  __shared__ PoseMats s_pose;
  static_assert(sizeof(PoseMats) % 4 == 0 && sizeof(PoseMats) / 4 <= 256, "one word per thread");
  if (threadIdx.x < sizeof(PoseMats) / 4)
    reinterpret_cast<uint32_t*>(&s_pose)[threadIdx.x] = reinterpret_cast<const uint32_t*>(&P)[threadIdx.x];
  knn5_pass<L, SLOTS, FUSE, FINE>(G, s_dir, &dr, scan_sorted, n, s_pose, max_ring, nbr, wl, wl_count, cand_total, prev.RT, prev.valid, prev.probe_min, tail, fa);
}
__device__ __forceinline__ const ChainHead* chain_enter(const ChainHead* __restrict__ H, unsigned int wait_epoch, unsigned int end_code) {
  constexpr int NW = (int)(sizeof(ChainHead) / 4);
  __shared__ unsigned int s_head[NW];
  __shared__ int s_go;
  if (wait_epoch != 0u) {
    if (threadIdx.x == 0) {
      const unsigned long long t0 = wall_clock64();
      int go = 0;
      unsigned int* dec = const_cast<unsigned int*>(&H->decision);
      const unsigned int v_go = wait_epoch, v_pend = wait_epoch | 0x80000000u, v_no = (wait_epoch & 0x3fffffffu) | 0x80000000u;
      for (int look = 0;; look++) {
        const unsigned int d = __hip_atomic_load(dec, __ATOMIC_RELAXED, __HIP_MEMORY_SCOPE_SYSTEM);
        const unsigned int e = __hip_atomic_load(&H->epoch, __ATOMIC_RELAXED, __HIP_MEMORY_SCOPE_SYSTEM);
        if (d == v_no) break;
        if (d == v_pend) { __builtin_amdgcn_s_sleep(8); continue; }
        if (e == wait_epoch || d == v_go) { go = 1; break; }
        if (e == end_code) break;
        const unsigned long long waited = wall_clock64() - t0;
        if (blockIdx.x == 0 && waited > (unsigned long long)CH_POLL_MS * 100000ull) {
          __hip_atomic_store(dec, v_pend, __ATOMIC_RELAXED, __HIP_MEMORY_SCOPE_SYSTEM);
          asm volatile("s_waitcnt vmcnt(0)" ::: "memory");
          for (int nap = 0; nap < 4; nap++) __builtin_amdgcn_s_sleep(127);
          const unsigned int e2 = __hip_atomic_load(&H->epoch, __ATOMIC_RELAXED, __HIP_MEMORY_SCOPE_SYSTEM);
          go = e2 == wait_epoch ? 1 : 0;
          __hip_atomic_store(dec, go ? v_go : v_no, __ATOMIC_RELAXED, __HIP_MEMORY_SCOPE_SYSTEM);
          break;
        }
        if (waited > 4ull * (unsigned long long)CH_POLL_MS * 100000ull) break;
        if (look == 0) __builtin_amdgcn_s_sleep(48);
        else __builtin_amdgcn_s_sleep(8);
      }
      s_go = go;
    }
    __syncthreads();
    if (!s_go) return nullptr;
    if ((int)threadIdx.x < NW)
      s_head[threadIdx.x] = __hip_atomic_load(reinterpret_cast<const unsigned int*>(H) + threadIdx.x, __ATOMIC_RELAXED, __HIP_MEMORY_SCOPE_SYSTEM);
  } else {
    if ((int)threadIdx.x < NW) s_head[threadIdx.x] = reinterpret_cast<const unsigned int*>(H)[threadIdx.x];
  }
  __syncthreads();
  const ChainHead* Lh = reinterpret_cast<const ChainHead*>(s_head);
  return Lh->status != 0 ? nullptr : Lh;
}
template <int L, int SLOTS, bool FUSE, bool FINE = false>
__global__ __launch_bounds__(256) KNN_WPE void knn5_chain_kernel(GridView G, const float4* __restrict__ scan_sorted, int n,
                                                   const ChainHead* __restrict__ H, int max_ring, NbrRec* __restrict__ nbr,
                                                   int* __restrict__ wl, int* __restrict__ wl_count,
                                                   unsigned long long* __restrict__ cand_total, int prev_valid, unsigned probe_min, int tail,
                                                   FuseArgs fa, unsigned int wait_epoch) {
  __shared__ __align__(16) uint16_t s_dir[GRID_DIR_MAX];
  {
    const DirRegs dr = grid_dir_fetch(G);
    grid_dir_store(s_dir, dr);
  }
  const ChainHead* Lh = chain_enter(H, wait_epoch, fa.ch.end_code);
  if (!Lh) return;
  knn5_pass<L, SLOTS, FUSE, FINE>(G, s_dir, nullptr, scan_sorted, n, Lh->pose, max_ring, nbr, wl, wl_count, cand_total, Lh->prev_RT, prev_valid, probe_min, tail, fa);
}

__device__ __forceinline__ void widen_body(const GridView& G, int max_ring, NbrRec* __restrict__ nbr,
                                           const int* __restrict__ wl, const int* __restrict__ wl_count,
                                           unsigned long long* __restrict__ cand_total, int first_ring, const TieList& tl,
                                           int blk, int nblk, uint32_t (*s_off)[65], uint32_t (*s_lo)[64]) {
  const int lane = threadIdx.x & 63, wave = threadIdx.x >> 6;
  const int maxdim = grid_maxdim(G);
  const float margin = 1.0e-3f + 4.0e-7f * (float)maxdim;
  int w = blk * 4 + wave;
  const int4* entries = reinterpret_cast<const int4*>(wl);
  int4 e0 = entries[2 * (size_t)w], e1 = entries[2 * (size_t)w + 1];
  const int count = *wl_count;
  for (; w < count; w += nblk * 4) {
    if (w != blk * 4 + wave) { e0 = entries[2 * (size_t)w]; e1 = entries[2 * (size_t)w + 1]; }
    const int p = e0.x;
    const float gx = __int_as_float(e0.y), gy = __int_as_float(e0.z), gz = __int_as_float(e0.w);
    const int hint_bits = e1.x;
    const float fx = (gx - G.ox) * G.inv_cell, fy = (gy - G.oy) * G.inv_cell, fz = (gz - G.oz) * G.inv_cell;
    const float flx = floorf(fminf(fmaxf(fx, -1.0e9f), 1.0e9f)), fly = floorf(fminf(fmaxf(fy, -1.0e9f), 1.0e9f)),
                flz = floorf(fminf(fmaxf(fz, -1.0e9f), 1.0e9f));
    const int cx = (int)flx - G.six, cy = (int)fly - G.siy, cz = (int)flz - G.siz;
    const float rx = fminf(fmaxf(fx - flx, 0.f), 1.f), ry = fminf(fmaxf(fy - fly, 0.f), 1.f),
                rz = fminf(fmaxf(fz - flz, 0.f), 1.f);
    const float edge = fminf(fminf(fminf(rx, 1.f - rx), fminf(ry, 1.f - ry)), fminf(rz, 1.f - rz));
    u64 best[5] = {KEY_NONE, KEY_NONE, KEY_NONE, KEY_NONE, KEY_NONE};
    u64 sixth = KEY_NONE;
    int flag = 0;
    int cand = 0;
    int r = first_ring;
    float bnd2 = __int_as_float(e1.z);
    if (!(bnd2 >= 0.f)) bnd2 = INFINITY;
    {
      const float hint = __int_as_float(hint_bits);
      if (hint >= 0.f && hint < INFINITY) {
        const float need = fl_sqrt(hint) * G.inv_cell * (1.f + 4.0e-6f) - edge + margin;
        r = max(2, (int)ceilf(fminf(need, 1.0e9f)));
        const float rc = (fl_sqrt(hint) * (1.f + 1.0e-5f) + 1.0e-6f) * G.inv_cell;
        bnd2 = fminf(bnd2, rc * rc * (1.f + 1.0e-5f));
      }
      r = min(r, max_ring);
    }
    for (;;) {
      const int side = 2 * r + 1;
      uint32_t lo = 0, len = 0;
      if (lane < side * side) {
        const int dy = (lane % side) - r, dz = (lane / side) - r;
        const int yy = cy + dy, zz = cz + dz;
        const float a_ = fmaxf(slab_dist(dy, ry) - margin, 0.f), b_ = fmaxf(slab_dist(dz, rz) - margin, 0.f);
        const float dyz2 = a_ * a_ + b_ * b_;
        int x0 = max(cx - r, 0), x1 = min(cx + r, G.nx - 1);
        if (bnd2 < 1.0e18f) {
          const float xr = fl_sqrt(fmaxf(bnd2 - dyz2, 0.f)) * (1.f + 1.0e-6f) + margin + 1.0e-4f;
          const int dr = (int)fminf(floorf(fminf(xr + rx, 1.0e6f)), (float)r);
          const int dl = (int)fminf(floorf(fminf(xr + (1.f - rx), 1.0e6f)), (float)r);
          x0 = max(cx - dl, 0); x1 = min(cx + dr, G.nx - 1);
        }
        if (dyz2 <= bnd2 && yy >= 0 && yy < G.ny && zz >= 0 && zz < G.nz && x0 <= x1) {
          uint32_t hi_;
          grid_row_range(G, G.dir, yy, zz, x0 * G.xs, (x1 + 1) * G.xs, lo, hi_);
          len = hi_ - lo;
        }
      }
      uint32_t inc = len;
#pragma unroll
      for (int o = 1; o < 64; o <<= 1) {
        const uint32_t v = __shfl_up(inc, o, 64);
        if (lane >= o) inc += v;
      }
      const uint32_t total = __shfl(inc, 63, 64);
      s_off[wave][lane + 1] = inc;
      if (lane == 0) s_off[wave][0] = 0;
      s_lo[wave][lane] = lo;
      __builtin_amdgcn_wave_barrier();
      const double none = __longlong_as_double((long long)KEY_NONE);
      double k5[6] = {none, none, none, none, none, none};
      const uint32_t last = total - 1u;
      for (uint32_t s0 = (uint32_t)lane; s0 < total; s0 += 4 * 64) {
        float4 q[4];
        uint32_t id[4];
#pragma unroll
// ... 208 lines not shown
    double r = 0.0;
#pragma unroll
    for (int w = 0; w < FIT_WAVES; w++) r += s_acc[w][t];
    __hip_atomic_store(&partials[(size_t)blockIdx.x * 256 + t], r, __ATOMIC_RELAXED, __HIP_MEMORY_SCOPE_AGENT);
  }
  asm volatile("s_waitcnt vmcnt(0)" ::: "memory");
  __syncthreads();
  TRACE(1, 4);
  const int group = blockIdx.x & (FIT_GROUPS - 1);
  const int nb_g = (int)(gridDim.x / FIT_GROUPS);
  if (threadIdx.x == 0) {
    const unsigned int old = __hip_atomic_fetch_add(ticket + group, 1u, __ATOMIC_RELAXED, __HIP_MEMORY_SCOPE_AGENT);
    s_last = (old == (unsigned int)nb_g - 1u) ? 1u : 0u;
  }
  __syncthreads();
  TRACE(1, 5);
  if (s_last) {
    constexpr int PARTS = FIT_THREADS / 256;
    const int t = threadIdx.x & 255, part = threadIdx.x >> 8;
    const int per = (nb_g + PARTS - 1) / PARTS;
    const int k0 = part * per, k1 = min(nb_g, k0 + per);
    const double* base = partials + (size_t)group * 256 + t;
    const size_t stride = (size_t)FIT_GROUPS * 256;
    double s0 = 0, s1 = 0, s2 = 0, s3 = 0;
    int k = k0;
    for (; k + 31 < k1; k += 32) {
      double v[32];
#pragma unroll
      for (int u = 0; u < 32; u++) v[u] = __hip_atomic_load(base + (size_t)(k + u) * stride, __ATOMIC_RELAXED, __HIP_MEMORY_SCOPE_AGENT);
#pragma unroll
      for (int u = 0; u < 32; u += 4) { s0 += v[u]; s1 += v[u + 1]; s2 += v[u + 2]; s3 += v[u + 3]; }
    }
    for (; k + 3 < k1; k += 4) {
      double v[4];
#pragma unroll
      for (int u = 0; u < 4; u++) v[u] = __hip_atomic_load(base + (size_t)(k + u) * stride, __ATOMIC_RELAXED, __HIP_MEMORY_SCOPE_AGENT);
      s0 += v[0]; s1 += v[1]; s2 += v[2]; s3 += v[3];
    }
    for (; k < k1; k++) s0 += __hip_atomic_load(base + (size_t)k * stride, __ATOMIC_RELAXED, __HIP_MEMORY_SCOPE_AGENT);
    s_acc[part][t] = (s0 + s1) + (s2 + s3);
    __syncthreads();
    TRACE(1, 6);
    double* out = out256 + (size_t)group * FIT_SLOT;
    if (part == 0) {
      double r = 0.0;
#pragma unroll
      for (int q = 0; q < PARTS; q++) r += s_acc[q][t];
      __hip_atomic_store(&out[t], r, __ATOMIC_RELAXED, __HIP_MEMORY_SCOPE_SYSTEM);
    }
    asm volatile("s_waitcnt vmcnt(0)" ::: "memory");
    __syncthreads();
    if (threadIdx.x == 0) {
      __hip_atomic_store(reinterpret_cast<unsigned long long*>(out + 256), seq, __ATOMIC_RELAXED, __HIP_MEMORY_SCOPE_SYSTEM);
      ticket[group] = 0u;
      if (group == 0) *wl_count = 0;
    }
    TRACE(1, 7);
  }
}


FLIMO_DEV void fit_row(const GridView& G, const PoseMats& P, const MatchParams& mp, const int (&ids)[5], float gx, float gy, float gz,
                       float (&v)[16]) {
  float px[5], py[5], pz[5], sq4 = 0.f;
#pragma unroll
  for (int s = 0; s < 5; s++) {
    const float4 q = G.pts[ids[s]];
    px[s] = q.x; py[s] = q.y; pz[s] = q.z;
    if (s == 4) sq4 = sqdist3(gx, gy, gz, q.x, q.y, q.z);
  }
  if (!((double)sq4 < mp.max_dist_plane_d)) return;
  float n4[4];
  plane_fit5(px, py, pz, n4);
  if (!plane_eval5(n4, px, py, pz, mp.plane_threshold)) return;
  const float dist = n4[0] * gx + n4[1] * gy + n4[2] * gz + n4[3];
  float row[12];
  h_row(P, gx, gy, gz, n4, mp.estimate_extrinsics, row);
#pragma unroll
  for (int i = 0; i < 12; i++) v[i] = row[i];
  v[12] = -dist;
  v[13] = 1.f;
}

template <int ROWS>
__device__ __forceinline__ void fit_reduce_publish(const float (&v)[16], bool owns_row, int row, float* sr, double* sa0, double* sa1,
                                                   double* sa2, double* sa3, unsigned int* s_last, const FitIdx& idx,
                                                   double* __restrict__ partials, double2* __restrict__ out_granules,
                                                   unsigned int* __restrict__ ticket, int* __restrict__ wl_count,
                                                   unsigned long long seq, const TieList& tl, int blk, int nblk) {
  typedef double v2d_t __attribute__((ext_vector_type(2)));
  const int fb = blk < 0 ? (int)blockIdx.x : blk, fnb = nblk < 0 ? (int)gridDim.x : nblk;
  const int lane = threadIdx.x & 63, wave = threadIdx.x >> 6;
  if (owns_row) {
#pragma unroll
    for (int c = 0; c < 16; c++) sr[c * 65 + row] = v[c];
  }
  wave_lds_sync();
  double4_t acc = {0.0, 0.0, 0.0, 0.0};
  const int col = lane & 15, sub4 = lane >> 4;
#pragma unroll
  for (int s = 0; s < ROWS / 4; s++) {
    const double a = (double)sr[col * 65 + 4 * s + sub4];
    acc = __builtin_amdgcn_mfma_f64_16x16x4f64(a, a, acc, 0, 0, 0);
  }
  double* sa = wave == 0 ? sa0 : (wave == 1 ? sa1 : (wave == 2 ? sa2 : sa3));
  sa[lane * 4 + 0] = acc[0]; sa[lane * 4 + 1] = acc[1]; sa[lane * 4 + 2] = acc[2]; sa[lane * 4 + 3] = acc[3];
  __syncthreads();
  if (threadIdx.x < FIT_LIVE) {
    const int t = idx.raw[threadIdx.x];
    const double r = ((sa0[t] + sa1[t]) + sa2[t]) + sa3[t];
    __hip_atomic_store(&partials[(size_t)fb * FIT_LIVE_PAD + threadIdx.x], r, __ATOMIC_RELAXED, __HIP_MEMORY_SCOPE_AGENT);
  }
  asm volatile("s_waitcnt vmcnt(0)" ::: "memory");
  __syncthreads();
  TRACE(1, 4);
  const int group = fb & (FIT_GROUPS - 1);
  const int nb_g = fnb / FIT_GROUPS;
  if (threadIdx.x == 0) {
    const unsigned int old = __hip_atomic_fetch_add(ticket + group, 1u, __ATOMIC_RELAXED, __HIP_MEMORY_SCOPE_AGENT);
    *s_last = (old == (unsigned int)nb_g - 1u) ? 1u : 0u;
  }
  __syncthreads();
  TRACE(1, 5);
  if (*s_last) {
    bool launch_last = false;
    if (threadIdx.x == 0)
      launch_last = __hip_atomic_fetch_add(ticket + FIT_GROUPS, 1u, __ATOMIC_RELAXED, __HIP_MEMORY_SCOPE_AGENT) == (unsigned int)FIT_GROUPS - 1u;
    const int c2 = (int)threadIdx.x % (FIT_LIVE_PAD / 2), sl = (int)threadIdx.x / (FIT_LIVE_PAD / 2);
    const int per = (nb_g + 4) / 5;
    const int k0 = sl * per, k1 = sl < 5 ? min(nb_g, k0 + per) : 0;
    v2d_t a0 = {0.0, 0.0}, a1 = {0.0, 0.0};
    {
      const double* base = partials + (size_t)group * FIT_LIVE_PAD + 2 * c2;
      const size_t stride = (size_t)FIT_GROUPS * FIT_LIVE_PAD;
      for (int k = k0; k < k1; k += 16) {
        v2d_t w[16];
#pragma unroll
        for (int u = 0; u < 16; u++) {
          const double* q = base + (size_t)min(k + u, k1 - 1) * stride;
          asm volatile("global_load_dwordx4 %0, %1, off sc1" : "=v"(w[u]) : "v"(q));
        }
        asm volatile("s_waitcnt vmcnt(0)"
                     : "+v"(w[0]), "+v"(w[1]), "+v"(w[2]), "+v"(w[3]), "+v"(w[4]), "+v"(w[5]), "+v"(w[6]), "+v"(w[7]), "+v"(w[8]), "+v"(w[9]),
                       "+v"(w[10]), "+v"(w[11]), "+v"(w[12]), "+v"(w[13]), "+v"(w[14]), "+v"(w[15]));
#pragma unroll
        for (int u = 0; u < 16; u += 2) {
          if (k + u < k1) a0 += w[u];
          if (k + u + 1 < k1) a1 += w[u + 1];
        }
      }
    }
    __syncthreads();
    if (sl < 5) {
      double* dstb = sl < 2 ? sa0 + sl * FIT_LIVE_PAD : (sl < 4 ? sa1 + (sl - 2) * FIT_LIVE_PAD : sa2);
      dstb[2 * c2] = a0.x + a1.x;
      dstb[2 * c2 + 1] = a0.y + a1.y;
    }
    __syncthreads();
    TRACE(1, 6);
    if (threadIdx.x < FIT_LIVE) {
      v2d_t g;
      g.x = ((sa0[threadIdx.x] + sa0[FIT_LIVE_PAD + threadIdx.x]) + (sa1[threadIdx.x] + sa1[FIT_LIVE_PAD + threadIdx.x])) + sa2[threadIdx.x];
      g.y = __longlong_as_double((long long)seq);
      double2* o = out_granules + (size_t)group * FIT_LIVE_PAD + threadIdx.x;
      asm volatile("global_store_dwordx4 %0, %1, off sc0 sc1\n\ts_nop 1" :: "v"(o), "v"(g) : "memory");
    }
    if (threadIdx.x == 0) {
      __hip_atomic_store(ticket + group, 0u, __ATOMIC_RELAXED, __HIP_MEMORY_SCOPE_AGENT);
      if (launch_last) {
        v2d_t g;
        g.x = (double)__hip_atomic_load(wl_count, __ATOMIC_RELAXED, __HIP_MEMORY_SCOPE_AGENT);
        g.y = __longlong_as_double((long long)seq);
        double2* o = out_granules + FIT_LIVE;
        asm volatile("global_store_dwordx4 %0, %1, off sc0 sc1\n\ts_nop 1" :: "v"(o), "v"(g) : "memory");
        g.x = tl.count ? (double)__hip_atomic_load(tl.count, __ATOMIC_RELAXED, __HIP_MEMORY_SCOPE_AGENT) : 0.0;
        o = out_granules + FIT_LIVE + 1;
        asm volatile("global_store_dwordx4 %0, %1, off sc0 sc1\n\ts_nop 1" :: "v"(o), "v"(g) : "memory");
        __hip_atomic_store(ticket + FIT_GROUPS, 0u, __ATOMIC_RELAXED, __HIP_MEMORY_SCOPE_AGENT);
        __hip_atomic_store(wl_count, 0, __ATOMIC_RELAXED, __HIP_MEMORY_SCOPE_AGENT);
        if (tl.count_next) __hip_atomic_store(tl.count_next, 0u, __ATOMIC_RELAXED, __HIP_MEMORY_SCOPE_AGENT);
      }
    }
    TRACE(1, 7);
  }
}

template <int PPW>
__device__ __forceinline__ void fit2_pass(const GridView& G, const float4* __restrict__ scan_sorted, int n,
                                          const NbrRec* __restrict__ nbr, const PoseMats& P, const MatchParams& mp, const FitIdx& idx,
                                          double* __restrict__ partials, double2* __restrict__ out_granules,
                                          unsigned int* __restrict__ ticket, int* __restrict__ wl_count,
                                          unsigned long long seq, const TieList& tl, const ChainCtl& ch, const BookView& book) {
  __shared__ __align__(16) float s_rec[4][16 * 65];
  __shared__ double s_acc[4][256];
  __shared__ unsigned int s_last;
  static_assert(sizeof(float) * 4 * 16 * 65 >= (size_t)IESKF_LDS_BYTES, "the filter's algebra runs in this workgroup's shared memory");
  int nb = (int)gridDim.x;
  if (ch.S) {
    nb -= 1;
    if ((int)blockIdx.x == nb) {
      double* big = reinterpret_cast<double*>(&s_rec[0][0]);
      ik_extra_block(ch, big, (int)threadIdx.x);
      return;
    }
  }
  const int lane = threadIdx.x & 63, wave = threadIdx.x >> 6;
  const int chunk = xcd_chunk(blockIdx.x, nb);
  const int p = (chunk * 4 + wave) * PPW + lane;
  float v[16];
#pragma unroll
  for (int i = 0; i < 16; i++) v[i] = 0.f;
  TRACE(1, 0);
  {
    const bool mine = lane < PPW && p < n;
    const float4 sp = scan_sorted[mine ? p : 0];
    const int4* nb = reinterpret_cast<const int4*>(&nbr[mine ? p : 0]);
    const int4 a = nb[0], b = nb[1];
    float gx, gy, gz;
    xform4(P.RT, sp.x, sp.y, sp.z, gx, gy, gz);
    int ids[5] = {a.x, a.y, a.z, a.w, b.x};
    TRACE(1, 1);
    if (book.node_c)
      tie_repair_wave(G, book, const_cast<NbrRec*>(nbr), mine && b.y == 1 && (b.w & 2) != 0, p, gx, gy, gz, (uint32_t)b.z, ids,
                      *reinterpret_cast<TieLds*>(&s_rec[wave][0]));
    if (mine && b.y == 1 && __float_as_uint(sp.w) < (uint32_t)mp.n_queries) fit_row(G, P, mp, ids, gx, gy, gz, v);
  }
  TRACE(1, 3);
  fit_reduce_publish<PPW>(v, lane < PPW, lane, s_rec[wave], s_acc[0], s_acc[1], s_acc[2], s_acc[3], &s_last, idx, partials,
                          out_granules, ticket, wl_count, seq, tl, (int)blockIdx.x, nb);
}

template <int PPW>
__global__ __launch_bounds__(256) void fit2_kernel(GridView G, const float4* __restrict__ scan_sorted, int n,
                                                   const NbrRec* __restrict__ nbr, PoseMats P, MatchParams mp, FitIdx idx,
                                                   double* __restrict__ partials, double2* __restrict__ out_granules,
                                                   unsigned int* __restrict__ ticket, int* __restrict__ wl_count,
                                                   unsigned long long seq, TieList tl, ChainCtl ch, BookView book) {
  fit2_pass<PPW>(G, scan_sorted, n, nbr, P, mp, idx, partials, out_granules, ticket, wl_count, seq, tl, ch, book);
}
template <int PPW>
__global__ __launch_bounds__(256) void fit2_chain_kernel(GridView G, const float4* __restrict__ scan_sorted, int n,
                                                   const NbrRec* __restrict__ nbr, const ChainHead* __restrict__ H, MatchParams mp, FitIdx idx,
                                                   double* __restrict__ partials, double2* __restrict__ out_granules,
                                                   unsigned int* __restrict__ ticket, int* __restrict__ wl_count,
                                                   unsigned long long seq, TieList tl, ChainCtl ch, BookView book) {
  if (H->status != 0) return;
  fit2_pass<PPW>(G, scan_sorted, n, nbr, H->pose, mp, idx, partials, out_granules, ticket, wl_count, seq, tl, ch, book);
}

__constant__ unsigned char c_ordered_indices[8][7] = {
    {1, 2, 4, 3, 5, 6, 7}, {0, 3, 5, 2, 4, 7, 6}, {0, 3, 6, 1, 4, 7, 5}, {1, 2, 7, 0, 5, 6, 4},
    {0, 5, 6, 1, 2, 7, 3}, {1, 4, 7, 0, 3, 6, 2}, {2, 4, 7, 0, 3, 5, 1}, {3, 5, 6, 1, 2, 4, 0}};

__device__ __forceinline__ int book_morton(float x, float y, float z, const float4& c) {
  return (x > c.x ? 1 : 0) | (y > c.y ? 2 : 0) | (z > c.z ? 4 : 0);
}
__device__ __forceinline__ int visit_pos(int m, int c) {
  if (c == m) return 0;
  int pos = 8;
#pragma unroll
  for (int i = 0; i < 7; i++) pos = (c_ordered_indices[m][i] == c) ? 1 + i : pos;
  return pos;
}
__device__ bool visited_before(const BookView& B, float ax, float ay, float az, uint32_t ra, float bx, float by, float bz, uint32_t rb,
                               float qx, float qy, float qz) {
// ... 557 lines not shown
    *wl_count = 0;
  }
}

__global__ void mfma_layout_kernel(double* __restrict__ raw) {
  const int lane = threadIdx.x;
  const int rc = lane & 15, k = lane >> 4;
  const double a = (k == 0) ? 1.0 : (k == 1 ? (double)rc : 0.0);
  const double b = (k == 0) ? (double)rc : (k == 1 ? 16.0 : 0.0);
  double4_t acc = {0.0, 0.0, 0.0, 0.0};
  acc = __builtin_amdgcn_mfma_f64_16x16x4f64(a, b, acc, 0, 0, 0);
  raw[lane * 4 + 0] = acc[0]; raw[lane * 4 + 1] = acc[1]; raw[lane * 4 + 2] = acc[2]; raw[lane * 4 + 3] = acc[3];
}

__global__ void word_probe_kernel(const unsigned int* __restrict__ src, double2* __restrict__ out, unsigned long long tag) {
  const unsigned int w = __hip_atomic_load(src, __ATOMIC_RELAXED, __HIP_MEMORY_SCOPE_SYSTEM);
  typedef double v2d_t __attribute__((ext_vector_type(2)));
  v2d_t g;
  g.x = (double)w;
  g.y = __longlong_as_double((long long)tag);
  asm volatile("global_store_dwordx4 %0, %1, off sc0 sc1\n\ts_nop 1" :: "v"(out), "v"(g) : "memory");
}
__global__ void rtt_probe_kernel(double2* __restrict__ out, unsigned long long tag) {
  typedef double v2d_t __attribute__((ext_vector_type(2)));
  v2d_t g;
  g.x = 1.0;
  g.y = __longlong_as_double((long long)tag);
  asm volatile("global_store_dwordx4 %0, %1, off sc0 sc1\n\ts_nop 1" :: "v"(out), "v"(g) : "memory");
}
void launch_rtt_probe(hipStream_t st, void* out_granule, unsigned long long tag) {
  hipLaunchKernelGGL(rtt_probe_kernel, dim3(1), dim3(1), 0, st, (double2*)out_granule, tag);
}

__global__ __launch_bounds__(256) void transform_kernel(const float4* __restrict__ in, int n, PoseMats P,
                                                        float4* __restrict__ out) {
  const int k = blockIdx.x * blockDim.x + threadIdx.x;
  if (k >= n) return;
  const float4 p = in[k];
  const float* M = P.RT;
  const float x = M[0] * p.x + (M[1] * p.y + (M[2] * p.z + M[3]));
  const float y = M[4] * p.x + (M[5] * p.y + (M[6] * p.z + M[7]));
  const float z = M[8] * p.x + (M[9] * p.y + (M[10] * p.z + M[11]));
  out[k] = make_float4(x, y, z, p.w);
}

constexpr int DEBUG_STAGE_WORDS = 2048;
__global__ __launch_bounds__(256) void deskew_debug_kernel(const DeskewArgs dk, int n, PoseMats P, float4* __restrict__ out_world,
                                                           float4* __restrict__ out_final) {
  __shared__ double s_frames[DEBUG_STAGE_WORDS / 2];
  const DevFrame* frames = static_cast<const DevFrame*>(dk.frames);
  const float* mats = dk.mats;
  if (dk.stage_words > 0) {
    unsigned int* dst = reinterpret_cast<unsigned int*>(s_frames);
    const unsigned int* src = reinterpret_cast<const unsigned int*>(dk.frames);
    for (int i = (int)threadIdx.x; i < dk.stage_words; i += 256)
      dst[i] = __hip_atomic_load(src + i, __ATOMIC_RELAXED, __HIP_MEMORY_SCOPE_SYSTEM);
    __syncthreads();
    frames = reinterpret_cast<const DevFrame*>(dst);
    mats = reinterpret_cast<const float*>(dst) + (dk.mats - static_cast<const float*>(dk.frames));
  }
  const int k = blockIdx.x * blockDim.x + threadIdx.x;
  if (k >= n) return;
  const float4 p = dk.raw[k];
  const unsigned int o = __float_as_uint(p.w);
  if (o >= (unsigned int)n) return;
  const float4 wp = deskew_world(p, dk.t[k] + dk.t_offset, frames, dk.nf, mats);
  const float4 b = deskew_body(wp, mats, 1.0f);
  const float* M = P.RT;
  const float x = M[0] * b.x + (M[1] * b.y + (M[2] * b.z + M[3]));
  const float y = M[4] * b.x + (M[5] * b.y + (M[6] * b.z + M[7]));
  const float z = M[8] * b.x + (M[9] * b.y + (M[10] * b.z + M[11]));
  const float w = M[12] * b.x + (M[13] * b.y + (M[14] * b.z + M[15]));
  out_world[o] = wp;
  out_final[o] = make_float4(x, y, z, w);
}

static inline int round_up8(int x) { return (x + 7) & ~7; }

template <int L>
static void launch_knn5_L(hipStream_t st, const GridView& G, const float4* scan_sorted, int n, const PoseMats& P,
                          int max_ring, void* nbr, int* wl, int* wl_count, unsigned long long* cand, const PrevPass& prev,
                          int tail, hipEvent_t e0, hipEvent_t e1, const FuseArgs* fuse, const TieList* tlp, int after_fine = 0,
                          unsigned long long seq = 0ull, const DeskewArgs* dk = nullptr, const ChainHead* chain = nullptr,
                          unsigned int wait_epoch = 0u, unsigned int end_code = 0u) {
  const int qpb = 256 / L;
  const int blocks = round_up8((n + qpb - 1) / qpb);
  constexpr int slots = 8;
  if constexpr (L == 2) {
    if (fuse) {
      const int grid = fused_blocks(n) + (fuse->ch.S ? 1 : 0);
      if (chain)
        hipExtLaunchKernelGGL((knn5_chain_kernel<2, 8, true>), dim3(grid), dim3(256), 0, st, e0, e1, 0, G, scan_sorted, n, chain, max_ring, (NbrRec*)nbr, wl, wl_count, cand, prev.valid, prev.probe_min, 1, *fuse, wait_epoch);
      else
      hipExtLaunchKernelGGL((knn5_kernel<2, 8, true>), dim3(grid), dim3(256), 0, st, e0, e1, 0, G, scan_sorted, n, P, max_ring, (NbrRec*)nbr, wl, wl_count, cand, prev, 1, *fuse);
      return;
    }
  }
  FuseArgs nofuse{};
  if (tlp) nofuse.tl = *tlp;
  nofuse.fine_mode = after_fine ? 1 : 0;
  nofuse.seq = seq;
  if (dk) nofuse.dk = *dk;
  nofuse.ch.end_code = end_code;
  if constexpr (L == 2) {
    if (chain) {
      hipExtLaunchKernelGGL((knn5_chain_kernel<2, 8, false>), dim3(blocks), dim3(256), 0, st, e0, e1, 0, G, scan_sorted, n, chain, max_ring, (NbrRec*)nbr, wl, wl_count, cand, prev.valid, prev.probe_min, tail, nofuse, wait_epoch);
      return;
    }
  }
  hipExtLaunchKernelGGL((knn5_kernel<L, slots, false>), dim3(blocks), dim3(256), 0, st, e0, e1, 0, G, scan_sorted, n, P, max_ring, (NbrRec*)nbr, wl, wl_count, cand, prev, tail, nofuse);
}

void launch_knn5(hipStream_t st, int lanes_per_query, const GridView& G, const float4* scan_sorted, int n,
                 const PoseMats& P, int max_ring, void* nbr, int* wl, int* wl_count, unsigned long long* cand,
                 const PrevPass& prev, int tail, hipEvent_t e0, hipEvent_t e1, const FuseArgs* fuse, const TieList* tlp, int after_fine,
                 unsigned long long seq, const DeskewArgs* dk, const ChainHead* chain, unsigned int wait_epoch, unsigned int end_code) {
  if (n <= 0) return;
  if (max_ring < 2 || max_ring > TAIL_MAX_RING) tail = 0;
  if (chain) { launch_knn5_L<2>(st, G, scan_sorted, n, P, max_ring, nbr, wl, wl_count, cand, prev, tail, e0, e1, fuse, tlp, after_fine, seq, dk, chain, wait_epoch, end_code); return; }
  (void)lanes_per_query;
  launch_knn5_L<2>(st, G, scan_sorted, n, P, max_ring, nbr, wl, wl_count, cand, prev, tail, e0, e1, fuse, tlp, after_fine, seq, dk);
}

void launch_widen(hipStream_t st, const GridView& G, const float4* scan_sorted, const PoseMats& P, int max_ring, void* nbr,
                  int* wl, int* wl_count, unsigned long long* cand, hipEvent_t e0, hipEvent_t e1, const TieList* tlp, const ChainHead* chain) {
  TieList tl{};
  if (tlp) tl = *tlp;
  if (max_ring <= 1) return;
  if (max_ring <= 3)
    hipExtLaunchKernelGGL(widen_kernel, dim3(2048), dim3(256), 0, st, e0, e1, 0, G, scan_sorted, P, max_ring, (NbrRec*)nbr, wl, wl_count, cand, max_ring, tl, chain);
  else
    hipLaunchKernelGGL(widen_general_kernel, dim3(256), dim3(256), 0, st, G, scan_sorted, P, max_ring, (NbrRec*)nbr, wl, wl_count, tl);
}

int fit_blocks(int n) { const int b = (n + 255) / 256; return (b + FIT_GROUPS - 1) / FIT_GROUPS * FIT_GROUPS; }

void launch_fit(hipStream_t st, const GridView& G, const float4* scan_sorted, int n, const void* nbr, const PoseMats& P,
                const MatchParams& mp, double* partials, Rec16* recs, RecDbg* dbg, double* out256, unsigned int* ticket,
                int* wl_count, unsigned long long seq) {
  if (n <= 0) return;
  const int blocks = fit_blocks(n);
  if (recs && dbg)
    hipLaunchKernelGGL((fit_kernel<true, true, 256>), dim3(blocks), dim3(256), 0, st, G, scan_sorted, n, (const NbrRec*)nbr, P, mp, partials, recs, dbg, out256, ticket, wl_count, seq);
  else if (recs)
    hipLaunchKernelGGL((fit_kernel<true, false, 256>), dim3(blocks), dim3(256), 0, st, G, scan_sorted, n, (const NbrRec*)nbr, P, mp, partials, recs, dbg, out256, ticket, wl_count, seq);
}

int fit2_blocks(int n) { const int b = (n + 255) / 256; return (b + FIT_GROUPS - 1) / FIT_GROUPS * FIT_GROUPS; }

void launch_fit2(hipStream_t st, const GridView& G, const float4* scan_sorted, int n, const void* nbr, const PoseMats& P,
                 const MatchParams& mp, const unsigned char* live_idx, double* partials, void* out_granules, unsigned int* ticket,
                 int* wl_count, unsigned long long seq, hipEvent_t e0, hipEvent_t e1, const TieList* tlp, const ChainHead* chain,
                 const ChainCtl* ctl, const BookView* bookp) {
  if (n <= 0) return;
  BookView book{};
  if (bookp) book = *bookp;
  TieList tl{};
  if (tlp) tl = *tlp;
  FitIdx idx;
  for (int i = 0; i < FIT_LIVE_PAD; i++) idx.raw[i] = i < FIT_LIVE ? live_idx[i] : 0;
  ChainCtl ch{};
  if (ctl) ch = *ctl;
  const int grid = fit2_blocks(n) + (ch.S ? 1 : 0);
  if (chain) {
    hipExtLaunchKernelGGL((fit2_chain_kernel<64>), dim3(grid), dim3(256), 0, st, e0, e1, 0, G, scan_sorted, n, (const NbrRec*)nbr, chain, mp, idx, partials, (double2*)out_granules, ticket, wl_count, seq, tl, ch, book);
    return;
  }
  hipExtLaunchKernelGGL((fit2_kernel<64>), dim3(grid), dim3(256), 0, st, e0, e1, 0, G, scan_sorted, n, (const NbrRec*)nbr, P, mp, idx, partials, (double2*)out_granules, ticket, wl_count, seq, tl, ch, book);
}

int fused_spread(int n) { int sh = 0; while (sh < 3 && ((long long)n << (sh + 1)) <= FUSED_SPREAD_SLOTS) sh++; return sh; }
int fused_blocks(int n) { return round_up8((int)((((long long)n << fused_spread(n)) + 127) / 128)); }
void launch_knn5_fine(hipStream_t st, const GridView& Gf, const float4* scan_sorted, int n, const PoseMats& P, void* nbr,
                      const PrevPass& prev, const int qlo[3], const int qhi[3], const TieList* tlp, unsigned long long seq, const ChainHead* chain,
                      unsigned int wait_epoch, unsigned int end_code) {
  if (n <= 0) return;
  FuseArgs fa{};
  fa.ch.end_code = end_code;
  fa.fine_mode = 2;
  fa.seq = seq;
  for (int a = 0; a < 3; a++) { fa.qlo[a] = qlo[a]; fa.qhi[a] = qhi[a]; }
  if (tlp) fa.tl = *tlp;
  PrevPass pv = prev;
  if (chain) {
    hipLaunchKernelGGL((knn5_chain_kernel<2, 8, false, true>), dim3(round_up8((n + 127) / 128)), dim3(256), 0, st, Gf, scan_sorted, n, chain, 1,
                       (NbrRec*)nbr, (int*)nullptr, (int*)nullptr, (unsigned long long*)nullptr, pv.valid, pv.probe_min, 0, fa, wait_epoch);
    return;
  }
  hipLaunchKernelGGL((knn5_kernel<2, 8, false, true>), dim3(round_up8((n + 127) / 128)), dim3(256), 0, st, Gf, scan_sorted, n, P, 1,
                     (NbrRec*)nbr, (int*)nullptr, (int*)nullptr, (unsigned long long*)nullptr, pv, 0, fa);
}
void launch_match_fused(hipStream_t st, const GridView& G, const float4* scan_sorted, int n, const PoseMats& P, const MatchParams& mp,
                        void* nbr, int* wl, int* wl_count, unsigned long long* cand, const PrevPass& prev,
                        const unsigned char* live_idx, double* partials, void* out_granules, unsigned int* ticket,
                        unsigned long long seq, hipEvent_t e0, hipEvent_t e1, const TieList* tlp, int after_fine, const DeskewArgs* dk,
                        const ChainHead* chain, const ChainCtl* ctl, const BookView* bookp, unsigned int wait_epoch) {
  if (n <= 0) return;
  FuseArgs fa{};
  if (ctl) fa.ch = *ctl;
  if (bookp) fa.book = *bookp;
  if (dk) fa.dk = *dk;
  fa.fine_mode = after_fine ? 1 : 0;
  fa.tl = TieList{};
  if (tlp) fa.tl = *tlp;
  fa.mp = mp;
  for (int i = 0; i < FIT_LIVE_PAD; i++) fa.idx.raw[i] = i < FIT_LIVE ? live_idx[i] : 0;
  fa.partials = partials; fa.granules = (double2*)out_granules; fa.ticket = ticket; fa.seq = seq;
  fa.spread = fused_spread(n);
  launch_knn5_L<2>(st, G, scan_sorted, n, P, mp.max_ring, nbr, wl, wl_count, cand, prev, 1, e0, e1, &fa, nullptr, 0, 0ull, nullptr, chain, wait_epoch, fa.ch.end_code);
}

size_t nbr_rec_size() { return sizeof(NbrRec); }
size_t wl_entry_size() { return 2 * sizeof(int4); }

void launch_knn(hipStream_t st, const GridView& G, const float* qxyz, int nq, int k, int max_ring, int32_t* idx,
                float* sqd, int32_t* cnt) {
  const int L = 4;
  const long long threads = (long long)nq * L;
  const int blocks = (int)((threads + 255) / 256);
  if (blocks == 0) return;
  const bool anywhere = max_ring > KNN_FAR_RING * 1024;
  hipLaunchKernelGGL((knn_kernel<4>), dim3(blocks), dim3(256), 0, st, G, qxyz, nq, k, anywhere ? KNN_FAR_RING : max_ring, idx, sqd, cnt);
  if (anywhere) hipLaunchKernelGGL(knn_far_kernel, dim3(std::min(4096, (nq + 3) / 4)), dim3(256), 0, st, G, qxyz, nq, k, idx, sqd, cnt);
}

void launch_cap(hipStream_t st, Rec16* recs, int n, int cap) {
  hipLaunchKernelGGL(cap_kernel, dim3(1), dim3(1024), 0, st, recs, n, cap);
}

void launch_capreduce(hipStream_t st, const Rec16* recs, int n, int cap, double* out256, int* wl_count, unsigned long long seq) {
  hipLaunchKernelGGL(capreduce_kernel, dim3(1), dim3(1024), 0, st, recs, n, cap, out256, wl_count, seq);
}

void launch_reduce(hipStream_t st, const Rec16* recs, int n, int nwaves, double* partials, double* out256) {
  hipLaunchKernelGGL(reduce_kernel, dim3(nwaves), dim3(64), 0, st, recs, n, partials);
  hipLaunchKernelGGL(reduce_final_kernel, dim3(1), dim3(1024), 0, st, partials, nwaves, out256);
}

void launch_word_probe(hipStream_t st, const unsigned int* src, void* out_granule, unsigned long long tag) {
  hipLaunchKernelGGL(word_probe_kernel, dim3(1), dim3(1), 0, st, src, (double2*)out_granule, tag);
}
void launch_mfma_layout(hipStream_t st, double* raw256) {
  hipLaunchKernelGGL(mfma_layout_kernel, dim3(1), dim3(64), 0, st, raw256);
}

void launch_deskew(hipStream_t st, const float4* in, const double* t, int n, const void* frames, int nf,
                   const float* mats32, float4* out_sorted, float4* out_orig, double t_offset) {
  const int blocks = (n + 255) / 256;
  if (blocks == 0) return;
  hipLaunchKernelGGL(deskew_kernel, dim3(blocks), dim3(256), 0, st, in, t, n, (const DevFrame*)frames, nf, mats32,
                     out_sorted, out_orig, t_offset);
}

bool launch_deskew_debug(hipStream_t st, const DeskewArgs& dk, int n, const PoseMats& P, float4* out_world, float4* out_final) {
  if (dk.stage_words > DEBUG_STAGE_WORDS) return false;
  const int blocks = (n + 255) / 256;
  if (blocks == 0) return true;
  hipLaunchKernelGGL(deskew_debug_kernel, dim3(blocks), dim3(256), 0, st, dk, n, P, out_world, out_final);
  return true;
}

void launch_transform(hipStream_t st, const float4* in, int n, const PoseMats& P, float4* out) {
  const int blocks = (n + 255) / 256;
  if (blocks == 0) return;
  hipLaunchKernelGGL(transform_kernel, dim3(blocks), dim3(256), 0, st, in, n, P, out);
}

size_t dev_frame_size() { return sizeof(DevFrame); }

}
```

include/flimo_dev.h:

```cpp
#ifndef FLIMO_DEV_H
#define FLIMO_DEV_H
#include "flimo_c.h"
#ifdef __cplusplus
extern "C" {
#endif

int flimo_set_timing(flimo_ctx* ctx, int level);
int flimo_set_timing_stride(flimo_ctx* ctx, int every);
int flimo_set_timing_deferred(flimo_ctx* ctx, int on);
unsigned long long flimo_pass_count(const flimo_ctx* ctx);
unsigned long long flimo_fused_pass_count(const flimo_ctx* ctx);
int flimo_tie_stats(flimo_ctx* ctx, unsigned long long out[2]);
int flimo_fine_stats(const flimo_ctx* ctx, unsigned long long out[4]);
int flimo_last_kernel_ms(const flimo_ctx* ctx, float* knn_ms, float* widen_ms, float* fit_ms);
int flimo_timing_totals(flimo_ctx* ctx, double* knn_ms, double* widen_ms, double* fit_ms, long long* passes,
                        long long* queries, int reset);
int flimo_timing_split(flimo_ctx* ctx, double out[6], int reset);
int flimo_set_path_switches(flimo_ctx* ctx, int tail, int fuse);
int flimo_last_widen_count(const flimo_ctx* ctx);
int flimo_last_stragglers(const flimo_ctx* ctx);
int flimo_stragglers_by_pass(const flimo_ctx* ctx, int out[4]);
double flimo_last_candidates_per_query(const flimo_ctx* ctx);

int flimo_map_grid_selfcheck(flimo_ctx* ctx, uint64_t* mismatches, uint64_t stats[2]);
int flimo_map_crop_stats(const flimo_ctx* ctx, uint64_t out[2]);

int flimo_chain_stats(flimo_ctx* ctx, double out[5], int reset);
int flimo_map_index_bytes(const flimo_ctx* ctx, uint64_t out[6]);
int flimo_pass_pipeline_stats(const flimo_ctx* ctx, unsigned long long out[4]);

void flimo_plane_fit5_host(const float xyz[15], float n_out[4]);
int  flimo_plane_eval5_host(const float n[4], const float xyz[15], float threshold);

int flimo_calculate_H_host(const double x26[26], const float* p_global, const float* n, const float* dist, size_t M,
                           int estimate_extrinsics, double* H, double* h);

int flimo_insert_rule_replay(float min_extent, int downsample, const float* xyz, const size_t* batch_sizes,
                             size_t n_batches, unsigned char* keep, size_t* stored);

#ifdef __cplusplus
}
#endif
#endif
```

Before: 7844 scans/s.

## Publish prelaunched pass pose via epoch-tagged 64-bit granules in a dedicated PipeHead

Replaces the shared ChainHead-based prelaunch handoff with a new PipeHead where each live pose word travels in its own 64-bit granule tagged with the epoch. The waiting kernel can then check tags per word instead of relying on one trailing epoch store. prev_RT moves from the published head into a kernel argument, and reuse of a prelaunch now requires that prev_RT matches. The aim is a torn-write-safe host-to-device publish with a single store pass and no separate status/epoch ordering; the cost is a larger head and per-word validation in the kernel. Also adds a large-BAR query API and a test hook that splits the publish with a delay.

```diff
diff --git a/fast_limo_amd/_lib.py b/fast_limo_amd/_lib.py
--- a/fast_limo_amd/_lib.py
+++ b/fast_limo_amd/_lib.py
@@ -71,7 +71,7 @@
     "flimo_scan_to_world", "flimo_scan_clouds", "flimo_scan_debug_clouds", "flimo_upload_stage", "flimo_match_reduce_overlap", "flimo_map_add_scan",
     "flimo_set_timing", "flimo_set_timing_stride", "flimo_set_timing_deferred", "flimo_pass_count", "flimo_fused_pass_count", "flimo_tie_stats", "flimo_map_index_bytes", "flimo_fine_stats", "flimo_map_grid_selfcheck", "flimo_set_debug_records", "flimo_last_kernel_ms",
     "flimo_last_candidates_per_query", "flimo_last_widen_count", "flimo_last_stragglers", "flimo_stragglers_by_pass", "flimo_timing_totals", "flimo_timing_split", "flimo_set_path_switches", "flimo_set_wait_timeout_ms", "flimo_insert_rule_replay", "flimo_plane_fit5_host", "flimo_plane_eval5_host", "flimo_calculate_H_host",
-    "flimo_update_chain", "flimo_chain_stats", "flimo_set_update_mode", "flimo_update_mode", "flimo_scan_adopt", "flimo_set_pass_pipeline", "flimo_pass_pipeline_end", "flimo_pass_pipeline_last", "flimo_pass_pipeline_stats",
+    "flimo_update_chain", "flimo_chain_stats", "flimo_set_update_mode", "flimo_update_mode", "flimo_scan_adopt", "flimo_set_pass_pipeline", "flimo_pass_pipeline_end", "flimo_pass_pipeline_last", "flimo_pass_pipeline_stats", "flimo_device_large_bar",
 ]
 
 _hip = None
@@ -483,6 +483,16 @@
         return float(self._L.flimo_last_candidates_per_query(self._h))
 
 
+def device_large_bar(device: int = 0) -> bool:
+    v = C.c_int(0)
+    fn = load_hip().flimo_device_large_bar
+    fn.argtypes = [C.c_int, C.POINTER(C.c_int)]
+    rc = fn(int(device), C.byref(v))
+    if rc != 0:
+        raise FlimoError(f"flimo_device_large_bar({device}) failed: {_ERRS.get(rc, rc)}")
+    return bool(v.value)
+
+
 def default_match_cfg(**kw) -> MatchCfg:
     c = MatchCfg(5, 2000, 10000, 2.0, 5.0e-2, 1)
     for k, v in kw.items():
diff --git a/fast_limo_amd/csrc/hip/flimo_capi.hip b/fast_limo_amd/csrc/hip/flimo_capi.hip
--- a/fast_limo_amd/csrc/hip/flimo_capi.hip
+++ b/fast_limo_amd/csrc/hip/flimo_capi.hip
@@ -199,10 +199,11 @@
     uint64_t grid_version = 0;
     unsigned int end_code = 0;
     double t_launch = 0.0;
+    float prev_RT[16] = {0};
   } pre;
   bool pipeline = false;
   bool pipeline_env = false;
-  ChainHead* d_pipe_head = nullptr;
+  PipeHead* d_pipe_head = nullptr;
   unsigned int pipe_tag = 0;
   bool pipe_last_hint = false;
   unsigned long long pipe_published = 0, pipe_cancelled = 0;
@@ -210,6 +211,7 @@
   bool row_slack = true;
   bool test_tight_array = false;
   int test_publish_delay_ms = 0;
+  int test_publish_split_ms = 0;
   PrevPass prev_before{};
   int update_mode = 0;
   double launch_rtt_us = 0.0;
@@ -284,25 +286,27 @@
   if (env_int("FLIMO_HOST_UPDATE", v)) c->update_mode = v != 0 ? 1 : 2;
   if (env_int("FLIMO_PIPELINE", v)) { c->pipeline = v != 0; c->pipeline_env = true; }
   if (env_int("FLIMO_TEST_PUBLISH_DELAY_MS", v) && v > 0) c->test_publish_delay_ms = v;
+  if (env_int("FLIMO_TEST_PUBLISH_SPLIT_MS", v) && v > 0) c->test_publish_split_ms = v;
   if (env_int("FLIMO_TEST_TIGHT_ARRAY", v)) c->test_tight_array = v != 0;
   if (env_int("FLIMO_ROW_SLACK", v)) c->row_slack = v != 0;
   if (env_int("FLIMO_TAIL_MAX", v) && v > 0) c->tail_max_env = v;
 }
 
-static bool host_store_probe(flimo_ctx* c, ChainHead* head) {
+static bool host_store_probe(flimo_ctx* c, PipeHead* head) {
   volatile unsigned long long* tagp = reinterpret_cast<volatile unsigned long long*>(c->h_chain_res) + 1;
   for (unsigned int round = 0; round < 2; round++) {
     const unsigned int pattern = 0x5a17c0deu ^ (round * 0x01010101u);
-    __atomic_store_n(&head->epoch, pattern, __ATOMIC_RELEASE);
+    volatile unsigned long long* g = &head->gran[round == 0 ? 0 : PH_GRANULES - 1];
+    *g = ((unsigned long long)pattern << 32) | (unsigned long long)round;
     _mm_sfence();
     const unsigned long long tag = 0x7200000000000000ull + round;
-    launch_word_probe(c->stream, &head->epoch, c->d_chain_res, tag);
+    launch_word_probe(c->stream, reinterpret_cast<unsigned int*>(const_cast<unsigned long long*>(g)) + 1, c->d_chain_res, tag);
     if (hipStreamSynchronize(c->stream) != hipSuccess) { (void)hipGetLastError(); return false; }
     if (*tagp != tag) return false;
     const double seen = c->h_chain_res[0];
     if ((unsigned int)llround(seen) != pattern) return false;
-  }
-  __atomic_store_n(&head->epoch, 0u, __ATOMIC_RELEASE);
+    *g = 0ull;
+  }
   _mm_sfence();
   memset(c->h_chain_res, 0, 2 * sizeof(double));
   return true;
@@ -383,9 +387,9 @@
     int large_bar = 0;
     (void)hipDeviceGetAttribute(&large_bar, hipDeviceAttributeIsLargeBar, device);
     if (getenv("FLIMO_NO_BAR") != nullptr) large_bar = 0;
-    if (large_bar && hipExtMallocWithFlags(&p, sizeof(ChainHead), hipDeviceMallocFinegrained) == hipSuccess && p &&
-        hipMemset(p, 0, sizeof(ChainHead)) == hipSuccess && hipDeviceSynchronize() == hipSuccess && host_store_probe(c, static_cast<ChainHead*>(p))) {
-      c->d_pipe_head = static_cast<ChainHead*>(p);
+    if (large_bar && hipExtMallocWithFlags(&p, sizeof(PipeHead), hipDeviceMallocFinegrained) == hipSuccess && p &&
+        hipMemset(p, 0, sizeof(PipeHead)) == hipSuccess && hipDeviceSynchronize() == hipSuccess && host_store_probe(c, static_cast<PipeHead*>(p))) {
+      c->d_pipe_head = static_cast<PipeHead*>(p);
       void* q = nullptr;
       if (hipExtMallocWithFlags(&q, 2 * FRAMES_FG_SLOT, hipDeviceMallocFinegrained) == hipSuccess && q)
         c->d_frames_fg = static_cast<char*>(q);
@@ -1559,27 +1563,26 @@
   if (!c->pre.active) return;
   c->pre.active = false;
   c->pipe_cancelled++;
-  __atomic_store_n(&c->d_pipe_head->epoch, c->pre.end_code, __ATOMIC_RELEASE);
+  *reinterpret_cast<volatile unsigned long long*>(&c->d_pipe_head->gran[0]) = (unsigned long long)c->pre.end_code << 32;
   _mm_sfence();
 }
 static inline void ctx_enter(flimo_ctx* c) {
   (void)hipSetDevice(c->device);
   cancel_prelaunch(c);
 }
-static inline void publish_prelaunch(flimo_ctx* c, const PoseMats& P, const float prev_RT[16], unsigned long long seq) {
-  ChainHead h;
-  memset(&h, 0, sizeof(h));
-  h.pose = P;
-  memcpy(h.prev_RT, prev_RT, sizeof(h.prev_RT));
-  h.status = 0;
-  const size_t words8 = offsetof(ChainHead, status) / 8;
-  static_assert(offsetof(ChainHead, status) % 8 == 0 && offsetof(ChainHead, epoch) == offsetof(ChainHead, status) + 4, "ChainHead layout");
-  volatile unsigned long long* dst = reinterpret_cast<volatile unsigned long long*>(c->d_pipe_head);
-  const unsigned long long* src = reinterpret_cast<const unsigned long long*>(&h);
-  for (size_t i = 0; i < words8; i++) dst[i] = src[i];
-  __atomic_store_n(&c->d_pipe_head->status, 0, __ATOMIC_RELAXED);
-  _mm_sfence();
-  __atomic_store_n(&c->d_pipe_head->epoch, ch_epoch_of(seq), __ATOMIC_RELEASE);
+static inline void publish_prelaunch(flimo_ctx* c, const PoseMats& P, unsigned long long seq) {
+  unsigned int w[PH_GRANULES] = {0u};
+  const unsigned int* src = reinterpret_cast<const unsigned int*>(&P);
+  for (int i = 0; i < PH_WORDS; i++) w[i] = src[i < 36 ? (i / 12) * 16 + i % 12 : i + 12];
+  const unsigned long long tag = (unsigned long long)ch_epoch_of(seq) << 32;
+  volatile unsigned long long* dst = c->d_pipe_head->gran;
+  for (int i = 0; i < PH_GRANULES; i++) {
+    if (i == PH_GRANULES / 2 && c->test_publish_split_ms > 0) {
+      _mm_sfence();
+      std::this_thread::sleep_for(std::chrono::milliseconds(c->test_publish_split_ms));
+    }
+    dst[i] = tag | (unsigned long long)w[i];
+  }
   _mm_sfence();
   c->pre.active = false;
   c->pipe_published++;
@@ -1709,7 +1712,8 @@
   bool use_pre = c->pre.active && !pl.general_k && c->prev.valid && c->pre.nq == nq && c->pre.seq == c->pass_seq + 1 &&
                  same_match_cfg(c->pre.cfg, *cfg) && c->pre.grid_version == pl.grid_version && !c->deskew_pending &&
                  !(nq < c->sorted_n || (c->sorted_n < c->scan_n && nq > c->sorted_n)) && c->pre.n_all == (int)c->sorted_n &&
-                 !c->debug_recs && !(cfg->MAX_NUM_MATCHES >= 0 && (size_t)cfg->MAX_NUM_MATCHES < nq);
+                 !c->debug_recs && !(cfg->MAX_NUM_MATCHES >= 0 && (size_t)cfg->MAX_NUM_MATCHES < nq) &&
+                 memcmp(c->pre.prev_RT, c->prev.RT, sizeof(c->pre.prev_RT)) == 0;
   if (use_pre && !(wall_s() - c->pre.t_launch < 0.25e-3 * (double)CH_POLL_MS)) { use_pre = false; c->pipe_aged++; }
   if (!use_pre) cancel_prelaunch(c);
   pre_guard.decided = true;
@@ -1824,7 +1828,7 @@
   const unsigned long long seq = pl.seq;
   const int tlev = pl.tlev;
   if (pl.use_pre) {
-    publish_prelaunch(c, P, c->prev.RT, seq);
+    publish_prelaunch(c, P, seq);
     c->fused_passes++;
   } else if (pl.after_fine) {
     launch_knn5_fine(c->stream, c->fine, c->d_scan_sorted, n_all, P, c->d_nbr, c->prev, c->fine_qlo, c->fine_qhi, &pl.tl, seq);
@@ -1884,10 +1888,11 @@
       pv.valid = 1;
       launch_match_fused(c->stream, c->grid, c->d_scan_sorted, n_all, P, mp, c->d_nbr, c->d_wl, c->d_wl_count, nullptr, pv,
                          c->live_idx, c->d_fit2_partials, c->d_granules_host, c->d_ticket, nseq, nullptr, nullptr, &tln, 0, nullptr,
-                         c->d_pipe_head, &pc, pl.bookp, ch_epoch_of(nseq));
+                         nullptr, &pc, pl.bookp, ch_epoch_of(nseq), c->d_pipe_head);
       HIPCHK(c, hipGetLastError());
       c->pre.active = true; c->pre.seq = nseq; c->pre.nq = nq; c->pre.n_all = n_all; c->pre.pos = npos; c->pre.cfg = *cfg;
       c->pre.grid_version = pl.grid_version; c->pre.end_code = pc.end_code; c->pre.t_launch = wall_s();
+      memcpy(c->pre.prev_RT, pv.RT, sizeof(c->pre.prev_RT));
     }
   }
   return FLIMO_OK;
@@ -2088,6 +2093,13 @@
 extern "C" int flimo_pass_pipeline_stats(const flimo_ctx* c, unsigned long long out[4]) {
   if (!c || !out) return FLIMO_ERR_INVALID;
   out[0] = c->pipe_published; out[1] = c->pipe_cancelled; out[2] = c->pipe_aged; out[3] = c->pipe_left;
+  return FLIMO_OK;
+}
+extern "C" int flimo_device_large_bar(int device, int* large_bar) {
+  if (!large_bar) return FLIMO_ERR_INVALID;
+  int v = 0;
+  if (hipDeviceGetAttribute(&v, hipDeviceAttributeIsLargeBar, device) != hipSuccess) { (void)hipGetLastError(); return FLIMO_ERR_HIP; }
+  *large_bar = v;
   return FLIMO_OK;
 }
 extern "C" int flimo_update_mode(const flimo_ctx* c, int* chained, double* launch_rtt_us) {
@@ -2191,20 +2203,18 @@
     pv.valid = prev_valid ? 1 : 0;
     TieList tl{};
     tl.count_next = c->d_tie_count + ((seq + 1) & 1);
-    unsigned int wait_epoch = 0u;
     if (after_fine) {
-      launch_knn5_fine(c->stream, c->fine, c->d_scan_sorted, n_all, P0, c->d_nbr, pv, c->fine_qlo, c->fine_qhi, &tl, seq, ch, wait_epoch, ctl.end_code);
-      wait_epoch = 0u;
+      launch_knn5_fine(c->stream, c->fine, c->d_scan_sorted, n_all, P0, c->d_nbr, pv, c->fine_qlo, c->fine_qhi, &tl, seq, ch);
       c->fine_passes++;
     }
     const DeskewArgs* dk = i == 0 ? dkp : nullptr;
     if (fused) {
       launch_match_fused(c->stream, c->grid, c->d_scan_sorted, n_all, P0, mp, c->d_nbr, c->d_wl, c->d_wl_count, nullptr, pv, c->live_idx,
                          c->d_fit2_partials, c->d_chain_gran, c->d_ticket, seq, ev ? ev[0] : nullptr, ev ? ev[1] : nullptr, &tl,
-                         after_fine ? 1 : 0, dk, ch, &ctl, bookp, wait_epoch);
+                         after_fine ? 1 : 0, dk, ch, &ctl, bookp);
     } else {
       launch_knn5(c->stream, 2, c->grid, c->d_scan_sorted, n_all, P0, mp.max_ring, c->d_nbr, c->d_wl, c->d_wl_count, nullptr, pv, 0,
-                  ev ? ev[0] : nullptr, ev ? ev[1] : nullptr, nullptr, &tl, after_fine ? 1 : 0, seq, dk, ch, wait_epoch, ctl.end_code);
+                  ev ? ev[0] : nullptr, ev ? ev[1] : nullptr, nullptr, &tl, after_fine ? 1 : 0, seq, dk, ch);
       {
         launch_widen(c->stream, c->grid, c->d_scan_sorted, P0, mp.max_ring, c->d_nbr, c->d_wl, c->d_wl_count, nullptr, ev ? ev[6] : nullptr, ev ? ev[7] : nullptr, &tl, ch);
         launch_fit2(c->stream, c->grid, c->d_scan_sorted, n_all, c->d_nbr, P0, mp, c->live_idx, c->d_fit2_partials, c->d_chain_gran,
diff --git a/fast_limo_amd/csrc/hip/flimo_chain.h b/fast_limo_amd/csrc/hip/flimo_chain.h
--- a/fast_limo_amd/csrc/hip/flimo_chain.h
+++ b/fast_limo_amd/csrc/hip/flimo_chain.h
@@ -10,11 +10,19 @@
   PoseMats pose;
   float prev_RT[16];
   int status;
-  unsigned int epoch;
-  unsigned int decision;
   int pad;
 };
 static_assert(sizeof(ChainHead) % 4 == 0 && sizeof(ChainHead) / 4 <= 128, "a pass workgroup reads the head with one load per thread");
+
+constexpr int PH_GRANULES = 64;
+constexpr int PH_WORDS = 3 * 12 + 9 + 9;
+struct PipeHead {
+  unsigned long long gran[PH_GRANULES];
+  unsigned int decision;
+  unsigned int pad[15];
+};
+static_assert(PH_WORDS <= PH_GRANULES && sizeof(PoseMats) == (PH_WORDS + 12) * 4, "every live word of PoseMats has its granule");
+struct PrevRT { float v[16]; };
 
 struct ChainPrior {
   double x[26];
diff --git a/fast_limo_amd/csrc/hip/flimo_kernels.h b/fast_limo_amd/csrc/hip/flimo_kernels.h
--- a/fast_limo_amd/csrc/hip/flimo_kernels.h
+++ b/fast_limo_amd/csrc/hip/flimo_kernels.h
@@ -7,6 +7,7 @@
 struct TieList;
 struct BookView;
 struct ChainCtl;
+struct PipeHead;
 struct ChainHead;
 struct DeskewArgs {
   const float4* raw; const double* t; const void* frames; int nf; const float* mats; double t_offset;
@@ -18,10 +19,10 @@
                  const PoseMats& P, int max_ring, void* nbr, int* wl, int* wl_count, unsigned long long* cand,
                  const PrevPass& prev, int tail, hipEvent_t e0 = nullptr, hipEvent_t e1 = nullptr, const struct FuseArgs* fuse = nullptr,
                  const TieList* ties = nullptr, int after_fine = 0, unsigned long long seq = 0ull, const DeskewArgs* deskew = nullptr,
-                 const ChainHead* chain = nullptr, unsigned int wait_epoch = 0u, unsigned int end_code = 0u);
+                 const ChainHead* chain = nullptr);
 void launch_knn5_fine(hipStream_t st, const GridView& Gf, const float4* scan_sorted, int n, const PoseMats& P, void* nbr,
                       const PrevPass& prev, const int qlo[3], const int qhi[3], const TieList* ties, unsigned long long seq,
-                      const ChainHead* chain = nullptr, unsigned int wait_epoch = 0u, unsigned int end_code = 0u);
+                      const ChainHead* chain = nullptr);
 void launch_widen(hipStream_t st, const GridView& G, const float4* scan_sorted, const PoseMats& P, int max_ring, void* nbr,
                   int* wl, int* wl_count, unsigned long long* cand, hipEvent_t e0 = nullptr, hipEvent_t e1 = nullptr,
                   const TieList* ties = nullptr, const ChainHead* chain = nullptr);
@@ -47,7 +48,8 @@
                         const unsigned char* live_idx, double* partials, void* out_granules, unsigned int* ticket,
                         unsigned long long seq, hipEvent_t e0 = nullptr, hipEvent_t e1 = nullptr, const TieList* ties = nullptr,
                         int after_fine = 0, const DeskewArgs* deskew = nullptr, const ChainHead* chain = nullptr,
-                        const ChainCtl* ctl = nullptr, const BookView* book = nullptr, unsigned int wait_epoch = 0u);
+                        const ChainCtl* ctl = nullptr, const BookView* book = nullptr, unsigned int wait_epoch = 0u,
+                        const PipeHead* pipe = nullptr);
 struct BookView { const float4* node_c; const int* node_child; const int* node_cnt; int root; unsigned long long* settled; };
 struct TieList { int* list; unsigned int* count; unsigned int cap; unsigned int* count_next; };
 void launch_tie(hipStream_t st, const GridView& G, const BookView& B, const float4* scan_sorted, const PoseMats& P, void* nbr,
diff --git a/fast_limo_amd/csrc/hip/flimo_kernels.hip b/fast_limo_amd/csrc/hip/flimo_kernels.hip
--- a/fast_limo_amd/csrc/hip/flimo_kernels.hip
+++ b/fast_limo_amd/csrc/hip/flimo_kernels.hip
@@ -216,8 +216,16 @@
     asm volatile("s_waitcnt vmcnt(0) lgkmcnt(0)" ::: "memory");                                         \
     if (threadIdx.x == 0) s_trace_lds[k][slot] = wall_clock64();                                        \
   } while (0)
+#define TRACE_LANE(k, slot, tid)                                                                        \
+  do {                                                                                                  \
+    if (threadIdx.x == (tid)) {                                                                         \
+      asm volatile("s_waitcnt vmcnt(0) lgkmcnt(0)" ::: "memory");                                       \
+      s_trace_lds[k][slot] = wall_clock64();                                                            \
+    }                                                                                                   \
+  } while (0)
 #define TRACE_FLUSH()                                                                                   \
   do {                                                                                                  \
+    __syncthreads();                                                                                    \
     if (threadIdx.x == 0 && blockIdx.x < 16384)                                                         \
       for (int k_ = 0; k_ < 2; k_++) for (int s_ = 0; s_ < 8; s_++) g_trace[k_][blockIdx.x * 8 + s_] = s_trace_lds[k_][s_]; \
   } while (0)
@@ -228,6 +236,7 @@
     if (threadIdx.x == 0 && blockIdx.x < 16384) g_trace[k][blockIdx.x * 8 + (slot)] = wall_clock64();  \
   } while (0)
 #define TRACE_FLUSH() do {} while (0)
+#define TRACE_LANE(k, slot, tid) do {} while (0)
 #endif
 extern "C" int flimo_trace_read(int k, unsigned long long* out, size_t n) {
   return (int)hipMemcpyFromSymbol(out, HIP_SYMBOL(g_trace), n * sizeof(unsigned long long), (size_t)k * 16384 * 8 * sizeof(unsigned long long),
@@ -236,6 +245,7 @@
 #else
 #define TRACE(k, slot) do {} while (0)
 #define TRACE_FLUSH() do {} while (0)
+#define TRACE_LANE(k, slot, tid) do {} while (0)
 #endif
 
 FLIMO_DEV u64 make_key(float d, uint32_t idx) { return ((u64)__float_as_uint(d) << 32) | (u64)idx; }
@@ -1225,47 +1235,59 @@
     reinterpret_cast<uint32_t*>(&s_pose)[threadIdx.x] = reinterpret_cast<const uint32_t*>(&P)[threadIdx.x];
   knn5_pass<L, SLOTS, FUSE, FINE>(G, s_dir, &dr, scan_sorted, n, s_pose, max_ring, nbr, wl, wl_count, cand_total, prev.RT, prev.valid, prev.probe_min, tail, fa);
 }
-__device__ __forceinline__ const ChainHead* chain_enter(const ChainHead* __restrict__ H, unsigned int wait_epoch, unsigned int end_code) {
+__device__ __forceinline__ const ChainHead* chain_enter(const ChainHead* __restrict__ H, const PipeHead* __restrict__ pipe, const PrevRT& prt,
+                                                        unsigned int wait_epoch, unsigned int end_code) {
   constexpr int NW = (int)(sizeof(ChainHead) / 4);
   __shared__ unsigned int s_head[NW];
   __shared__ int s_go;
-  if (wait_epoch != 0u) {
-    if (threadIdx.x == 0) {
+  if (pipe != nullptr) {
+    const int tid = (int)threadIdx.x;
+    if (tid < 64) {
       const unsigned long long t0 = wall_clock64();
       int go = 0;
-      unsigned int* dec = const_cast<unsigned int*>(&H->decision);
+      unsigned long long gv = 0ull;
+      unsigned int* dec = const_cast<unsigned int*>(&pipe->decision);
       const unsigned int v_go = wait_epoch, v_pend = wait_epoch | 0x80000000u, v_no = (wait_epoch & 0x3fffffffu) | 0x80000000u;
       for (int look = 0;; look++) {
         const unsigned int d = __hip_atomic_load(dec, __ATOMIC_RELAXED, __HIP_MEMORY_SCOPE_SYSTEM);
-        const unsigned int e = __hip_atomic_load(&H->epoch, __ATOMIC_RELAXED, __HIP_MEMORY_SCOPE_SYSTEM);
+        gv = __hip_atomic_load(&pipe->gran[tid], __ATOMIC_RELAXED, __HIP_MEMORY_SCOPE_SYSTEM);
+        const unsigned int e = (unsigned int)(gv >> 32);
+        const bool all = __ballot(e == wait_epoch) == ~0ull;
+        const unsigned int e0 = (unsigned int)__builtin_amdgcn_readfirstlane((int)e);
         if (d == v_no) break;
         if (d == v_pend) { __builtin_amdgcn_s_sleep(8); continue; }
-        if (e == wait_epoch || d == v_go) { go = 1; break; }
-        if (e == end_code) break;
+        if (all) { go = 1; break; }
+        if (e0 == end_code) break;
         const unsigned long long waited = wall_clock64() - t0;
-        if (blockIdx.x == 0 && waited > (unsigned long long)CH_POLL_MS * 100000ull) {
-          __hip_atomic_store(dec, v_pend, __ATOMIC_RELAXED, __HIP_MEMORY_SCOPE_SYSTEM);
+        if (blockIdx.x == 0 && d != v_go && waited > (unsigned long long)CH_POLL_MS * 100000ull) {
+          if (tid == 0) __hip_atomic_store(dec, v_pend, __ATOMIC_RELAXED, __HIP_MEMORY_SCOPE_SYSTEM);
           asm volatile("s_waitcnt vmcnt(0)" ::: "memory");
           for (int nap = 0; nap < 4; nap++) __builtin_amdgcn_s_sleep(127);
-          const unsigned int e2 = __hip_atomic_load(&H->epoch, __ATOMIC_RELAXED, __HIP_MEMORY_SCOPE_SYSTEM);
-          go = e2 == wait_epoch ? 1 : 0;
-          __hip_atomic_store(dec, go ? v_go : v_no, __ATOMIC_RELAXED, __HIP_MEMORY_SCOPE_SYSTEM);
+          gv = __hip_atomic_load(&pipe->gran[tid], __ATOMIC_RELAXED, __HIP_MEMORY_SCOPE_SYSTEM);
+          go = __ballot((unsigned int)(gv >> 32) == wait_epoch) == ~0ull ? 1 : 0;
+          if (tid == 0) __hip_atomic_store(dec, go ? v_go : v_no, __ATOMIC_RELAXED, __HIP_MEMORY_SCOPE_SYSTEM);
           break;
         }
         if (waited > 4ull * (unsigned long long)CH_POLL_MS * 100000ull) break;
         if (look == 0) __builtin_amdgcn_s_sleep(48);
         else __builtin_amdgcn_s_sleep(8);
       }
-      s_go = go;
+      if (go && tid < PH_WORDS) s_head[tid < 36 ? (tid / 12) * 16 + tid % 12 : tid + 12] = (unsigned int)gv;
+      if (tid == 0) s_go = go;
+    } else if (tid < 64 + 12) {
+      const int k = tid - 64;
+      s_head[(k / 4) * 16 + 12 + k % 4] = __float_as_uint(k % 4 == 3 ? 1.f : 0.f);
+    } else if (tid >= 128 && tid < 128 + 16) {
+      s_head[offsetof(ChainHead, prev_RT) / 4 + (tid - 128)] = __float_as_uint(prt.v[tid - 128]);
+    } else if (tid >= 192 && tid < 192 + NW - (int)(offsetof(ChainHead, status) / 4)) {
+      s_head[offsetof(ChainHead, status) / 4 + (tid - 192)] = 0u;
     }
     __syncthreads();
     if (!s_go) return nullptr;
-    if ((int)threadIdx.x < NW)
-      s_head[threadIdx.x] = __hip_atomic_load(reinterpret_cast<const unsigned int*>(H) + threadIdx.x, __ATOMIC_RELAXED, __HIP_MEMORY_SCOPE_SYSTEM);
   } else {
     if ((int)threadIdx.x < NW) s_head[threadIdx.x] = reinterpret_cast<const unsigned int*>(H)[threadIdx.x];
-  }
-  __syncthreads();
+    __syncthreads();
+  }
   const ChainHead* Lh = reinterpret_cast<const ChainHead*>(s_head);
   return Lh->status != 0 ? nullptr : Lh;
 }
@@ -1274,13 +1296,13 @@
                                                    const ChainHead* __restrict__ H, int max_ring, NbrRec* __restrict__ nbr,
                                                    int* __restrict__ wl, int* __restrict__ wl_count,
                                                    unsigned long long* __restrict__ cand_total, int prev_valid, unsigned probe_min, int tail,
-                                                   FuseArgs fa, unsigned int wait_epoch) {
+                                                   FuseArgs fa, unsigned int wait_epoch, const PipeHead* __restrict__ pipe, PrevRT prt) {
   __shared__ __align__(16) uint16_t s_dir[GRID_DIR_MAX];
   {
     const DirRegs dr = grid_dir_fetch(G);
     grid_dir_store(s_dir, dr);
   }
-  const ChainHead* Lh = chain_enter(H, wait_epoch, fa.ch.end_code);
+  const ChainHead* Lh = chain_enter(H, pipe, prt, wait_epoch, fa.ch.end_code);
   if (!Lh) return;
   knn5_pass<L, SLOTS, FUSE, FINE>(G, s_dir, nullptr, scan_sorted, n, Lh->pose, max_ring, nbr, wl, wl_count, cand_total, Lh->prev_RT, prev_valid, probe_min, tail, fa);
 }
@@ -1655,6 +1677,23 @@
   v[13] = 1.f;
 }
 
+__device__ __forceinline__ void publish_counters(int n_wl, unsigned int n_tie, double2* __restrict__ out_granules,
+                                                 unsigned int* __restrict__ ticket, int* __restrict__ wl_count, unsigned long long seq,
+                                                 const TieList& tl) {
+  typedef double v2d_t __attribute__((ext_vector_type(2)));
+  v2d_t g;
+  g.x = (double)n_wl;
+  g.y = __longlong_as_double((long long)seq);
+  double2* o = out_granules + FIT_LIVE;
+  asm volatile("global_store_dwordx4 %0, %1, off sc0 sc1\n\ts_nop 1" :: "v"(o), "v"(g) : "memory");
+  g.x = (double)n_tie;
+  o = out_granules + FIT_LIVE + 1;
+  asm volatile("global_store_dwordx4 %0, %1, off sc0 sc1\n\ts_nop 1" :: "v"(o), "v"(g) : "memory");
+  __hip_atomic_store(ticket + FIT_GROUPS, 0u, __ATOMIC_RELAXED, __HIP_MEMORY_SCOPE_AGENT);
+  __hip_atomic_store(wl_count, 0, __ATOMIC_RELAXED, __HIP_MEMORY_SCOPE_AGENT);
+  if (tl.count_next) __hip_atomic_store(tl.count_next, 0u, __ATOMIC_RELAXED, __HIP_MEMORY_SCOPE_AGENT);
+}
+
 template <int ROWS>
 __device__ __forceinline__ void fit_reduce_publish(const float (&v)[16], bool owns_row, int row, float* sr, double* sa0, double* sa1,
                                                    double* sa2, double* sa3, unsigned int* s_last, const FitIdx& idx,
@@ -1696,9 +1735,10 @@
   __syncthreads();
   TRACE(1, 5);
   if (*s_last) {
-    bool launch_last = false;
-    if (threadIdx.x == 0)
-      launch_last = __hip_atomic_fetch_add(ticket + FIT_GROUPS, 1u, __ATOMIC_RELAXED, __HIP_MEMORY_SCOPE_AGENT) == (unsigned int)FIT_GROUPS - 1u;
+    unsigned int launch_ticket = 0xffffffffu;
+    unsigned int* launch_slot = ticket + FIT_GROUPS;
+    asm volatile("" : "+v"(launch_slot));
+    if (threadIdx.x == 255) launch_ticket = __hip_atomic_fetch_add(launch_slot, 1u, __ATOMIC_RELAXED, __HIP_MEMORY_SCOPE_AGENT);
     const int c2 = (int)threadIdx.x % (FIT_LIVE_PAD / 2), sl = (int)threadIdx.x / (FIT_LIVE_PAD / 2);
     const int per = (nb_g + 4) / 5;
     const int k0 = sl * per, k1 = sl < 5 ? min(nb_g, k0 + per) : 0;
@@ -1707,21 +1747,39 @@
       const double* base = partials + (size_t)group * FIT_LIVE_PAD + 2 * c2;
       const size_t stride = (size_t)FIT_GROUPS * FIT_LIVE_PAD;
       for (int k = k0; k < k1; k += 16) {
+        const double* q[16];
+#pragma unroll
+        for (int u = 0; u < 16; u++) q[u] = base + (size_t)min(k + u, k1 - 1) * stride;
         v2d_t w[16];
-#pragma unroll
-        for (int u = 0; u < 16; u++) {
-          const double* q = base + (size_t)min(k + u, k1 - 1) * stride;
-          asm volatile("global_load_dwordx4 %0, %1, off sc1" : "=v"(w[u]) : "v"(q));
-        }
-        asm volatile("s_waitcnt vmcnt(0)"
-                     : "+v"(w[0]), "+v"(w[1]), "+v"(w[2]), "+v"(w[3]), "+v"(w[4]), "+v"(w[5]), "+v"(w[6]), "+v"(w[7]), "+v"(w[8]), "+v"(w[9]),
-                       "+v"(w[10]), "+v"(w[11]), "+v"(w[12]), "+v"(w[13]), "+v"(w[14]), "+v"(w[15]));
+        asm volatile(
+            "global_load_dwordx4 %0, %16, off sc1\n\tglobal_load_dwordx4 %1, %17, off sc1\n\t"
+            "global_load_dwordx4 %2, %18, off sc1\n\tglobal_load_dwordx4 %3, %19, off sc1\n\t"
+            "global_load_dwordx4 %4, %20, off sc1\n\tglobal_load_dwordx4 %5, %21, off sc1\n\t"
+            "global_load_dwordx4 %6, %22, off sc1\n\tglobal_load_dwordx4 %7, %23, off sc1\n\t"
+            "global_load_dwordx4 %8, %24, off sc1\n\tglobal_load_dwordx4 %9, %25, off sc1\n\t"
+            "global_load_dwordx4 %10, %26, off sc1\n\tglobal_load_dwordx4 %11, %27, off sc1\n\t"
+            "global_load_dwordx4 %12, %28, off sc1\n\tglobal_load_dwordx4 %13, %29, off sc1\n\t"
+            "global_load_dwordx4 %14, %30, off sc1\n\tglobal_load_dwordx4 %15, %31, off sc1\n\t"
+            "s_waitcnt vmcnt(0)"
+            : "=&v"(w[0]), "=&v"(w[1]), "=&v"(w[2]), "=&v"(w[3]), "=&v"(w[4]), "=&v"(w[5]), "=&v"(w[6]), "=&v"(w[7]), "=&v"(w[8]),
+              "=&v"(w[9]), "=&v"(w[10]), "=&v"(w[11]), "=&v"(w[12]), "=&v"(w[13]), "=&v"(w[14]), "=&v"(w[15])
+            : "v"(q[0]), "v"(q[1]), "v"(q[2]), "v"(q[3]), "v"(q[4]), "v"(q[5]), "v"(q[6]), "v"(q[7]), "v"(q[8]), "v"(q[9]), "v"(q[10]),
+              "v"(q[11]), "v"(q[12]), "v"(q[13]), "v"(q[14]), "v"(q[15])
+            : "memory");
 #pragma unroll
         for (int u = 0; u < 16; u += 2) {
           if (k + u < k1) a0 += w[u];
           if (k + u + 1 < k1) a1 += w[u + 1];
         }
       }
+    }
+    asm volatile("" : "+v"(launch_ticket));
+    const bool launch_last = launch_ticket == (unsigned int)FIT_GROUPS - 1u;
+    int n_wl = 0;
+    unsigned int n_tie = 0u;
+    if (launch_last) {
+      n_wl = __hip_atomic_load(wl_count, __ATOMIC_RELAXED, __HIP_MEMORY_SCOPE_AGENT);
+      if (tl.count) n_tie = __hip_atomic_load(tl.count, __ATOMIC_RELAXED, __HIP_MEMORY_SCOPE_AGENT);
     }
     __syncthreads();
     if (sl < 5) {
@@ -1738,22 +1796,10 @@
       double2* o = out_granules + (size_t)group * FIT_LIVE_PAD + threadIdx.x;
       asm volatile("global_store_dwordx4 %0, %1, off sc0 sc1\n\ts_nop 1" :: "v"(o), "v"(g) : "memory");
     }
-    if (threadIdx.x == 0) {
-      __hip_atomic_store(ticket + group, 0u, __ATOMIC_RELAXED, __HIP_MEMORY_SCOPE_AGENT);
-      if (launch_last) {
-        v2d_t g;
-        g.x = (double)__hip_atomic_load(wl_count, __ATOMIC_RELAXED, __HIP_MEMORY_SCOPE_AGENT);
-        g.y = __longlong_as_double((long long)seq);
-        double2* o = out_granules + FIT_LIVE;
-        asm volatile("global_store_dwordx4 %0, %1, off sc0 sc1\n\ts_nop 1" :: "v"(o), "v"(g) : "memory");
-        g.x = tl.count ? (double)__hip_atomic_load(tl.count, __ATOMIC_RELAXED, __HIP_MEMORY_SCOPE_AGENT) : 0.0;
-        o = out_granules + FIT_LIVE + 1;
-        asm volatile("global_store_dwordx4 %0, %1, off sc0 sc1\n\ts_nop 1" :: "v"(o), "v"(g) : "memory");
-        __hip_atomic_store(ticket + FIT_GROUPS, 0u, __ATOMIC_RELAXED, __HIP_MEMORY_SCOPE_AGENT);
-        __hip_atomic_store(wl_count, 0, __ATOMIC_RELAXED, __HIP_MEMORY_SCOPE_AGENT);
-        if (tl.count_next) __hip_atomic_store(tl.count_next, 0u, __ATOMIC_RELAXED, __HIP_MEMORY_SCOPE_AGENT);
-      }
-    }
+    if (threadIdx.x == 0) __hip_atomic_store(ticket + group, 0u, __ATOMIC_RELAXED, __HIP_MEMORY_SCOPE_AGENT);
+    asm volatile("" : "+v"(n_wl), "+v"(n_tie));
+    if (launch_last) publish_counters(n_wl, n_tie, out_granules, ticket, wl_count, seq, tl);
+    if (launch_last) TRACE_LANE(1, 2, 255);
     TRACE(1, 7);
   }
 }
@@ -2477,15 +2523,17 @@
                           int max_ring, void* nbr, int* wl, int* wl_count, unsigned long long* cand, const PrevPass& prev,
                           int tail, hipEvent_t e0, hipEvent_t e1, const FuseArgs* fuse, const TieList* tlp, int after_fine = 0,
                           unsigned long long seq = 0ull, const DeskewArgs* dk = nullptr, const ChainHead* chain = nullptr,
-                          unsigned int wait_epoch = 0u, unsigned int end_code = 0u) {
+                          unsigned int wait_epoch = 0u, unsigned int end_code = 0u, const PipeHead* pipe = nullptr) {
   const int qpb = 256 / L;
+  PrevRT prt;
+  for (int i = 0; i < 16; i++) prt.v[i] = prev.RT[i];
   const int blocks = round_up8((n + qpb - 1) / qpb);
   constexpr int slots = 8;
   if constexpr (L == 2) {
     if (fuse) {
       const int grid = fused_blocks(n) + (fuse->ch.S ? 1 : 0);
-      if (chain)
-        hipExtLaunchKernelGGL((knn5_chain_kernel<2, 8, true>), dim3(grid), dim3(256), 0, st, e0, e1, 0, G, scan_sorted, n, chain, max_ring, (NbrRec*)nbr, wl, wl_count, cand, prev.valid, prev.probe_min, 1, *fuse, wait_epoch);
+      if (chain || pipe)
+        hipExtLaunchKernelGGL((knn5_chain_kernel<2, 8, true>), dim3(grid), dim3(256), 0, st, e0, e1, 0, G, scan_sorted, n, chain, max_ring, (NbrRec*)nbr, wl, wl_count, cand, prev.valid, prev.probe_min, 1, *fuse, wait_epoch, pipe, prt);
       else
       hipExtLaunchKernelGGL((knn5_kernel<2, 8, true>), dim3(grid), dim3(256), 0, st, e0, e1, 0, G, scan_sorted, n, P, max_ring, (NbrRec*)nbr, wl, wl_count, cand, prev, 1, *fuse);
       return;
@@ -2498,8 +2546,8 @@
   if (dk) nofuse.dk = *dk;
   nofuse.ch.end_code = end_code;
   if constexpr (L == 2) {
-    if (chain) {
-      hipExtLaunchKernelGGL((knn5_chain_kernel<2, 8, false>), dim3(blocks), dim3(256), 0, st, e0, e1, 0, G, scan_sorted, n, chain, max_ring, (NbrRec*)nbr, wl, wl_count, cand, prev.valid, prev.probe_min, tail, nofuse, wait_epoch);
+    if (chain || pipe) {
+      hipExtLaunchKernelGGL((knn5_chain_kernel<2, 8, false>), dim3(blocks), dim3(256), 0, st, e0, e1, 0, G, scan_sorted, n, chain, max_ring, (NbrRec*)nbr, wl, wl_count, cand, prev.valid, prev.probe_min, tail, nofuse, wait_epoch, pipe, prt);
       return;
     }
   }
@@ -2509,10 +2557,10 @@
 void launch_knn5(hipStream_t st, int lanes_per_query, const GridView& G, const float4* scan_sorted, int n,
                  const PoseMats& P, int max_ring, void* nbr, int* wl, int* wl_count, unsigned long long* cand,
                  const PrevPass& prev, int tail, hipEvent_t e0, hipEvent_t e1, const FuseArgs* fuse, const TieList* tlp, int after_fine,
-                 unsigned long long seq, const DeskewArgs* dk, const ChainHead* chain, unsigned int wait_epoch, unsigned int end_code) {
+                 unsigned long long seq, const DeskewArgs* dk, const ChainHead* chain) {
   if (n <= 0) return;
   if (max_ring < 2 || max_ring > TAIL_MAX_RING) tail = 0;
-  if (chain) { launch_knn5_L<2>(st, G, scan_sorted, n, P, max_ring, nbr, wl, wl_count, cand, prev, tail, e0, e1, fuse, tlp, after_fine, seq, dk, chain, wait_epoch, end_code); return; }
+  if (chain) { launch_knn5_L<2>(st, G, scan_sorted, n, P, max_ring, nbr, wl, wl_count, cand, prev, tail, e0, e1, fuse, tlp, after_fine, seq, dk, chain); return; }
   (void)lanes_per_query;
   launch_knn5_L<2>(st, G, scan_sorted, n, P, max_ring, nbr, wl, wl_count, cand, prev, tail, e0, e1, fuse, tlp, after_fine, seq, dk);
 }
@@ -2567,11 +2615,9 @@
 int fused_spread(int n) { int sh = 0; while (sh < 3 && ((long long)n << (sh + 1)) <= FUSED_SPREAD_SLOTS) sh++; return sh; }
 int fused_blocks(int n) { return round_up8((int)((((long long)n << fused_spread(n)) + 127) / 128)); }
 void launch_knn5_fine(hipStream_t st, const GridView& Gf, const float4* scan_sorted, int n, const PoseMats& P, void* nbr,
-                      const PrevPass& prev, const int qlo[3], const int qhi[3], const TieList* tlp, unsigned long long seq, const ChainHead* chain,
-                      unsigned int wait_epoch, unsigned int end_code) {
+                      const PrevPass& prev, const int qlo[3], const int qhi[3], const TieList* tlp, unsigned long long seq, const ChainHead* chain) {
   if (n <= 0) return;
   FuseArgs fa{};
-  fa.ch.end_code = end_code;
   fa.fine_mode = 2;
   fa.seq = seq;
   for (int a = 0; a < 3; a++) { fa.qlo[a] = qlo[a]; fa.qhi[a] = qhi[a]; }
@@ -2579,7 +2625,7 @@
   PrevPass pv = prev;
   if (chain) {
     hipLaunchKernelGGL((knn5_chain_kernel<2, 8, false, true>), dim3(round_up8((n + 127) / 128)), dim3(256), 0, st, Gf, scan_sorted, n, chain, 1,
-                       (NbrRec*)nbr, (int*)nullptr, (int*)nullptr, (unsigned long long*)nullptr, pv.valid, pv.probe_min, 0, fa, wait_epoch);
+                       (NbrRec*)nbr, (int*)nullptr, (int*)nullptr, (unsigned long long*)nullptr, pv.valid, pv.probe_min, 0, fa, 0u, (const PipeHead*)nullptr, PrevRT{});
     return;
   }
   hipLaunchKernelGGL((knn5_kernel<2, 8, false, true>), dim3(round_up8((n + 127) / 128)), dim3(256), 0, st, Gf, scan_sorted, n, P, 1,
@@ -2589,8 +2635,9 @@
                         void* nbr, int* wl, int* wl_count, unsigned long long* cand, const PrevPass& prev,
                         const unsigned char* live_idx, double* partials, void* out_granules, unsigned int* ticket,
                         unsigned long long seq, hipEvent_t e0, hipEvent_t e1, const TieList* tlp, int after_fine, const DeskewArgs* dk,
-                        const ChainHead* chain, const ChainCtl* ctl, const BookView* bookp, unsigned int wait_epoch) {
+                        const ChainHead* chain, const ChainCtl* ctl, const BookView* bookp, unsigned int wait_epoch, const PipeHead* pipe) {
   if (n <= 0) return;
+  if ((pipe != nullptr) != (wait_epoch != 0u)) return;
   FuseArgs fa{};
   if (ctl) fa.ch = *ctl;
   if (bookp) fa.book = *bookp;
@@ -2602,7 +2649,7 @@
   for (int i = 0; i < FIT_LIVE_PAD; i++) fa.idx.raw[i] = i < FIT_LIVE ? live_idx[i] : 0;
   fa.partials = partials; fa.granules = (double2*)out_granules; fa.ticket = ticket; fa.seq = seq;
   fa.spread = fused_spread(n);
-  launch_knn5_L<2>(st, G, scan_sorted, n, P, mp.max_ring, nbr, wl, wl_count, cand, prev, 1, e0, e1, &fa, nullptr, 0, 0ull, nullptr, chain, wait_epoch, fa.ch.end_code);
+  launch_knn5_L<2>(st, G, scan_sorted, n, P, mp.max_ring, nbr, wl, wl_count, cand, prev, 1, e0, e1, &fa, nullptr, 0, 0ull, nullptr, chain, wait_epoch, fa.ch.end_code, pipe);
 }
 
 size_t nbr_rec_size() { return sizeof(NbrRec); }
diff --git a/include/flimo_dev.h b/include/flimo_dev.h
--- a/include/flimo_dev.h
+++ b/include/flimo_dev.h
@@ -28,6 +28,7 @@
 int flimo_chain_stats(flimo_ctx* ctx, double out[5], int reset);
 int flimo_map_index_bytes(const flimo_ctx* ctx, uint64_t out[6]);
 int flimo_pass_pipeline_stats(const flimo_ctx* ctx, unsigned long long out[4]);
+int flimo_device_large_bar(int device, int* large_bar);
 
 void flimo_plane_fit5_host(const float xyz[15], float n_out[4]);
 int  flimo_plane_eval5_host(const float n[4], const float xyz[15], float threshold);
```

Result: faster. 8018 scans/s (median of 6 runs) (+2.2%).
